# prannaykaul/lvc

Measured on AMD Instinct MI355X. Metric: img/s COCO 800x1333 R50-FPN inference (GeneralizedRCNN.forward(batched_inputs) -> Instances, 1000 proposals, 100 detections), higher is better.
Workload: dtype f32 (conv/GEMM inner products on the fp16 / bf16 matrix cores through fp32-accurate operand splits: two-way fp16 with main + cross fp32 accumulators for the 3x3 and wide 1x1 / FC layers, three-way bf16 for the rest; final boxes/scores closer to the fp64 evaluation than the reference's fp32 CPU path,; 1 GPU; COCO-detection R50-FPN inference, bs=8 synthetic 3x800x1333 per GPU, 1000 pre/post-NMS proposals per level/image, 80 classes, conditioned random-init weights; batch_per_gpu=8, global_batch=8, parallelism=dp1

## Files before the change

### include/lvc_amd.h

```cpp
#ifndef LVC_AMD_H
#define LVC_AMD_H

#ifdef __cplusplus
extern "C" {
#endif

#define LVC_OK 0
#define LVC_ERR_INVALID 1
#define LVC_ERR_HIP 2

int lvc_abi_version(void);
const char* lvc_last_error(void);
void lvc_set_error(const char* fmt, ...);

long long lvc_conv_workspace_bytes(void);
long long lvc_conv_range_words_offset(void);
void lvc_set_range_slot(int slot);
int lvc_range_slot(void);
int lvc_range_slots(void);
int lvc_conv2d_nhwc_f32(const float* x, const float* w_packed, const float* scale, const float* shift,
                        const float* residual, float* y, int N, int H, int W, int C, int K, int R, int S,
                        int stride, int pad, int Kg, int relu, int res_mode, int ldy, int ldr, int mode,
                        void* workspace, void* stream);

int lvc_conv2d_nhwc_bf16x3(const float* x, const unsigned short* w_split, const float* scale, const float* shift,
                           const float* residual, float* y, int N, int H, int W, int C, int K, int R, int S,
                           int stride, int pad, int Kg, int relu, int res_mode, int ldy, int ldr, void* workspace,
                           void* stream);

int lvc_conv3x3_nhwc_bf16x3(const float* x, const unsigned short* w_split, const float* scale, const float* shift,
                            const float* residual, float* y, int N, int H, int W, int C, int K, int Kg, int relu,
                            int res_mode, int ldy, int ldr, void* workspace, void* stream);

int lvc_conv3x3_nhwc_f16x2(const float* x, const unsigned short* w_split, const float* scale, const float* shift,
                           const float* residual, float* y, int N, int H, int W, int C, int K, int Kg, int relu,
                           int res_mode, int ldy, int ldr, void* workspace, void* stream);
int lvc_conv3x3_nhwc_f16s1(const float* x, const unsigned short* w_split, const float* scale, const float* shift,
                           const float* residual, float* y, int N, int H, int W, int C, int K, int Kg, int relu,
                           int res_mode, int ldy, int ldr, void* workspace, void* stream);
int lvc_conv3x3_nhwc_f16x2_pipe(const float* x, const unsigned short* w_split, const float* scale, const float* shift,
                                const float* residual, float* y, int N, int H, int W, int C, int K, int Kg, int relu,
                                int res_mode, int ldy, int ldr, void* workspace, void* stream);
int lvc_conv3x3_nhwc_f16_levels(int oneacc, const float* const* xs, float* const* ys, const int* Hs, const int* Ws, int L,
                                const unsigned short* w_split, const float* scale, const float* shift, int N, int C, int K, int Kg,
                                int relu, void* workspace, void* stream);
int lvc_conv3x3_nhwc_f16_levels_pred(int oneacc, const float* const* xs, float* const* ys, const int* Hs, const int* Ws, int L,
                                     const unsigned short* w_split, const float* scale, const float* shift, int N, int C, int K, int Kg,
                                     int relu, const unsigned short* pred_w, const float* pred_scale, const float* pred_shift, int pred_K,
                                     int pred_rows, int pred_ld, int pred_slot, void* workspace, void* stream);
int lvc_conv3x3_nhwc_f16_layers(int oneacc, const float* const* xs, float* const* ys, const int* Hs, const int* Ws, int L,
                                const unsigned short* const* ws, const float* const* scales, const float* const* shifts, int N, int C,
                                int K, int Kg, int relu, void* workspace, void* stream);
void lvc_set_wino_streamk(int mode);
void lvc_set_patch_plan(int mode);
int lvc_patch_plan(void);
void lvc_set_nms_reduce_global(int on);
void lvc_set_select_onelaunch(int mode);
int lvc_select_onelaunch(void);
void lvc_set_halo_test_hooks(int ph, int pw, int force);
int lvc_conv3x3_nhwc_wino(const float* x, const unsigned short* u, const float* scale, const float* shift, float* y, int N, int H, int W,
                          int C, int K, int Kpad, int relu, int ldy, void* workspace, void* stream);
int lvc_conv3x3_nhwc_wino_pred(const float* x, const unsigned short* u, const float* scale, const float* shift, float* y, int N, int H,
                               int W, int C, int K, int Kpad, int relu, int ldy, const unsigned short* pred_w, const float* pred_scale,
                               const float* pred_shift, int pred_K, int pred_rows, int pred_slot, void* workspace, void* stream);
int lvc_conv1x1_nhwc_f16x2_pipe(const float* x, const unsigned short* w_split, const float* scale, const float* shift,
                                const float* residual, float* y, int N, int H, int W, int C, int K, int stride, int relu,
                                int res_mode, int ldy, int ldr, void* workspace, void* stream);
int lvc_conv1x1_nhwc_f16s1(const float* x, const unsigned short* w_split, const float* scale, const float* shift,
                           const float* residual, float* y, int N, int H, int W, int C, int K, int stride, int relu,
                           int res_mode, int ldy, int ldr, void* workspace, void* stream);
int lvc_conv3x3_nhwc_f16s1_presplit(const float* x, const unsigned short* w_split, const float* scale, const float* shift, void* y,
                                    int N, int H, int W, int C, int K, int Kg, int next_slot, void* workspace, void* stream);
int lvc_conv1x1_nhwc_f16s1_presplit(const void* x, const unsigned short* w_split, const float* scale, const float* shift,
                                    const float* residual, float* y, int N, int H, int W, int C, int K, int relu,
                                    int res_mode, int ldy, int ldr, void* workspace, void* stream);
int lvc_conv1x1_nhwc_f16s1_w2(const float* x, const unsigned short* w_split, const float* scale, const float* shift,
                              const float* residual, float* y, int N, int H, int W, int C, int K, int Kpad, int stride, int relu,
                              int res_mode, int ldy, int ldr, void* workspace, void* stream);
int lvc_conv1x1_chain_nhwc_f16s1(const float* x, int ldx, const unsigned short* wa, int wa_rows, const float* sa, const float* ta,
                                 const float* residual, int ldr, float* y1, int ldy1, int relu1, const unsigned short* wb,
                                 int wb_rows, const float* sb, const float* tb, float* y2, int ldy2, int relu2, int M, int K1,
                                 int N1, int N2, void* workspace, void* stream);
int lvc_bottleneck_nhwc_f16s1(const float* x, int ldx, float* y, int ldy, int N, int H, int W, int cin, int proj,
                              const unsigned short* w, const float* s1, const float* t1, const float* s2, const float* t2,
                              const float* s3, const float* t3, void* workspace, void* stream);
int lvc_split_weights_rowscaled(const float* wp, int rows, int Kg, void* planes_out, float* row_factor, void* stream);

int lvc_conv2d_nhwc_f16x2(const float* x, const unsigned short* w_split, const float* scale, const float* shift,
                          const float* residual, float* y, int N, int H, int W, int C, int K, int R, int S,
                          int stride, int pad, int Kg, int relu, int res_mode, int ldy, int ldr, void* workspace,
                          void* stream);
int lvc_conv2d_nhwc_f16x2_dma(const float* x, const unsigned short* w_split, const float* scale, const float* shift,
                          const float* residual, float* y, int N, int H, int W, int C, int K, int R, int S,
                          int stride, int pad, int Kg, int relu, int res_mode, int ldy, int ldr, void* workspace,
                          void* stream);

int lvc_stem_conv_pool_nhwc4_f16x2(const float* x, const unsigned short* w_split, const float* scale, const float* shift,
                                   float* y, int N, int H, int W, int Kpad, int relu, int* d_error_word,
                                   float* y2 , int ldy2, void* stream);

int lvc_preprocess_nhwc4(const void* image, int dtype, int h, int w, const float* mean3, const float* std3,
                         float* out, int Hp, int Wp, void* stream);
int lvc_preprocess_batch_nhwc4(const void* const* images, int dtype, const int* hs, const int* ws, int B, const float* mean3,
                               const float* std3, float* out, int Hp, int Wp, void* stream);

int lvc_resize_bilinear_u8(const unsigned char* image, int H, int W, int new_h, int new_w, const int* xb, const int* xk,
                           int kxs, const int* yb, const int* yk, int kys, unsigned char* tmp, unsigned char* out_u8,
                           float* out_nhwc4, int Hp, int Wp, const float* mean3, const float* std3, void* stream);
int lvc_tta_resize_u8(const unsigned char* image, int H, int W, long long sy, long long sx, long long sc, const long long* hjobs,
                      int n_h, const long long* vjobs, int n_v, const float* mean3, const float* std3, void* stream);
long long lvc_tta_merge_workspace_bytes(int B, int Nmax);
int lvc_tta_merge(const float* boxes, const float* scores, const int* classes, const int* counts, int topk_in, const float* params,
                  const int* tab, int B, int Nmax, float score_thresh, double nms_thresh, int topk_out, float* ob, float* osc, int* ocl,
                  int* ocount, void* workspace, long long workspace_bytes, void* stream);
int lvc_train_input_u8(const void* h_blob, const void* d_blob, long long blob_bytes, int B, unsigned char* tmp, long long tmp_bytes,
                       float* out, int n_slots, int Hp, int Wp, const float* mean3, const float* std3, int* launches, void* stream);
int lvc_train_input_tiles_u8(const void* h_blob, const void* d_blob, long long blob_bytes, int B, unsigned char* tmp,
                             long long tmp_bytes, float* out, int n_slots, int Hp, int Wp, const float* mean3, const float* std3,
                             int* launches, void* stream);
int lvc_train_input_lsj_u8(const void* h_blob, const void* d_blob, long long blob_bytes, int B, unsigned char* tmp,
                           long long tmp_bytes, float* out, int n_slots, int Hp, int Wp, const float* mean3, const float* std3,
                           int* launches, void* stream);
int lvc_color_jitter_tiles_u8(const void* h_blob, void* d_blob, long long blob_bytes, int B, unsigned char* out, long long out_bytes,
                              int* launches, void* stream);
int lvc_maxpool2d_nhwc(const float* x, float* y, int N, int H, int W, int C, int k, int stride, int pad,
                       void* stream);

int lvc_crop_resize_nearest(const float* image_chw, int C, int H, int W, const int* d_windows, int K, int out_size,
                            float* out, void* stream);

int lvc_rownorm(const float* x, const float* mu, float* y, int M, int D, int ldx, int ldy, float eps, int mode,
                void* stream);
int lvc_rownorm_backward(const float* x, const float* dy, float* dx, int M, int D, float eps, int accumulate, void* stream);

int lvc_roi_align_forward_nchw(const float* input, const float* rois, float* output, int B, int C, int H, int W,
                               int K, int pooled_h, int pooled_w, float spatial_scale, int sampling_ratio,
                               int aligned, int* d_status, void* stream);
int lvc_roi_align_fpn_nhwc(const float* const* feats, const int* Hs, const int* Ws, const float* scales, int L,
                           int B, int C, const float* rois, const int* levels, const int* d_num_valid, int K,
                           int pooled_h, int pooled_w, int sampling_ratio, int aligned, float* output,
                           int* d_status, void* stream);
int lvc_roi_work_order(const float* rois, const int* levels, const float* scales, int L, int K, int pooled_h, int* d_order,
                       void* stream);
int lvc_roi_work_order_xcd(const float* rois, const int* levels, int K, int B, int* d_order, void* stream);
int lvc_roi_align_fpn_nhwc_ordered(const float* const* feats, const int* Hs, const int* Ws, const float* scales, int L,
                                   int B, int C, const float* rois, const int* levels, const int* d_num_valid, int K,
                                   int pooled_h, int pooled_w, int sampling_ratio, int aligned, float* output,
                                   int* d_status, const int* d_order, void* stream);

int lvc_roi_align_backward_nchw(const float* grad, const float* rois, float* grad_input, int B, int C, int H, int W,
                                int K, int pooled_h, int pooled_w, float spatial_scale, int sampling_ratio,
                                int aligned, int* d_status, void* stream);
int lvc_roi_align_fpn_backward_nhwc(const float* grad, float* const* grad_feats, const int* Hs, const int* Ws,
                                    const float* scales, int L, int B, int C, const float* rois, const int* levels,
                                    const int* d_num_valid, int K, int pooled_h, int pooled_w, int sampling_ratio,
                                    int aligned, int* d_status, void* stream);

long long lvc_batched_nms_workspace_bytes(int B, int Nmax);
int lvc_batched_nms(const float* boxes, const float* scores, const int* idxs, const int* d_counts, int B,
                    int Nmax, double iou_threshold, int max_keep, int* keep, int* d_num_keep, void* workspace,
                    long long workspace_bytes, void* stream);

long long lvc_rpn_proposals_workspace_bytes(int B, int L, int A, const int* Hs, const int* Ws, int pre_nms_topk);
int lvc_rpn_proposals(const float* const* logits, const int* ld_logit, const float* const* deltas,
                      const int* ld_delta, const float* const* cell_anchors, const int* Hs, const int* Ws,
                      const int* strides, int L, int A, int B, const int* d_image_sizes, int pre_nms_topk,
                      int post_nms_topk, double nms_thresh, float min_box_size, float scale_clamp,
                      float* out_boxes, float* out_logits, int* d_out_count, void* workspace,
                      long long workspace_bytes, void* stream);

long long lvc_retinanet_select_workspace_bytes(int B, int L, int A, int K, const int* Hs, const int* Ws, int topk,
                                               int max_survivors);
int lvc_retinanet_select(const float* const* logits, const int* ld_logit, const float* const* deltas, const int* ld_delta,
                         const float* const* cell_anchors, const int* Hs, const int* Ws, const int* strides,
                         float anchor_offset, int L, int A, int K, int B, int topk, float score_thresh, float wx, float wy,
                         float ww, float wh, float scale_clamp, int max_survivors, float* out_boxes, float* out_scores,
                         int* out_classes, int* out_index, int* d_count, int* d_status, void* workspace,
                         long long workspace_bytes, void* stream);

int lvc_gather_detections(const float* boxes, const float* scores, const int* classes, const int* rows, const int* keep,
                          const int* d_num_keep, int B, int Nmax, int topk, const float* d_post, float* out_boxes,
                          float* out_scores, int* out_classes, int* out_rows, int* d_out_count, void* stream);

long long lvc_retinanet_loss_workspace_bytes(int B, int L, int A, int K, const int* Hs, const int* Ws);
int lvc_retinanet_loss(const float* const* logits, const int* ld_logit, const float* const* deltas, const int* ld_delta,
                       const int* Hs, const int* Ws, int L, int A, int K, int B, const float* anchors, const int* matches,
                       const signed char* labels, const float* gt, const long long* gt_classes, const int* gt_off, double alpha,
                       double gamma, double beta, double wx, double wy, double ww, double wh, double momentum,
                       double one_minus_momentum, const double* normalizer_in, double* normalizer_out, float* out_losses,
                       double* out_sums , int* num_pos, void* workspace, long long workspace_bytes, void* stream);
int lvc_retinanet_loss_grad(const float* const* logits, const int* ld_logit, const float* const* deltas, const int* ld_delta,
                            const int* Hs, const int* Ws, int L, int A, int K, int B, const float* anchors, const int* matches,
                            const signed char* labels, const float* gt, const long long* gt_classes, const int* gt_off, double alpha,
                            double gamma, double beta, double wx, double wy, double ww, double wh, const double* normalizer,
                            const float* g_cls, const float* g_box, float* const* dlogits, const int* ld_dlogit,
                            float* const* ddeltas, const int* ld_ddelta, void* stream);

int lvc_assign_levels_rois(const float* boxes, int B, int R, int min_level, int max_level, int canonical_box_size,
                           int canonical_level, int* levels, float* rois, void* stream);

long long lvc_fast_rcnn_inference_workspace_bytes(int B, int max_candidates);
int lvc_fast_rcnn_inference(const float* cls_logits, int ld_cls, const float* deltas, int ld_delta, int K,
                            int cls_agnostic, const float* proposals, const int* d_prop_count, int B, int R,
                            const int* d_image_sizes, float wx, float wy, float ww, float wh, float scale_clamp,
                            float score_thresh, double nms_thresh, int topk, int max_candidates,
                            const float* d_post, float* out_boxes, float* out_scores, int* out_classes,
                            int* out_rows, int* d_out_count, int* d_status, void* workspace,
                            long long workspace_bytes, void* stream);

int lvc_decode_boxes(const float* deltas, int ld, const float* boxes, int M, int R, const int* d_image_sizes,
                     float wx, float wy, float ww, float wh, float scale_clamp, float* out, void* stream);

int lvc_match_boxes(const float* gt, int G, const float* boxes, int N, float t0, float t1, int nthr, int l0, int l1,
                    int l2, int allow_low_quality, long long* matches, signed char* labels, float* matched_vals,
                    unsigned int* d_gt_best, void* stream);
int lvc_match_boxes_batched(const float* gt, const int* gt_off, int Gtot, int B, const float* boxes, long long box_img_stride,
                            const int* nbox, int N, float t0, float t1, int nthr, int l0, int l1, int l2, int allow_low_quality,
                            int* matches, signed char* labels, float* vals, unsigned int* gt_best, void* stream);
long long lvc_subsample_workspace_bytes(int B);
int lvc_subsample_batched(const signed char* labels, const long long* keys , unsigned long long seed,
                          int B, int N, int nbits, int cap_pos, int bs, int* sel, int* counts, void* workspace, void* stream);
int lvc_rpn_gather_sampled(const void* const* fused, const int* ld, const void* const* cell_anchors, const int* H, const int* W,
                           const int* strides, int L, int A, int B, int bs, const int* sel, const int* counts, const int* matches,
                           const float* gt, const int* gt_off, float* logits, float* deltas, float* anchors, float* gt_boxes,
                           signed char* labels, void* stream);
int lvc_roi_build_table(const float* pboxes, const float* plogits, const int* pcount, int B, int P, const float* gt, const int* gt_off,
                        float gt_logit, int Wt, float* boxes, float* logits, int* nrow, void* stream);
int lvc_roi_gather_sampled(const float* boxes, const float* logits, const int* matches, const int* sel, const int* counts,
                           const long long* gt_classes, const int* gt_off, int B, int Wt, int bs, int K, float* s_boxes, float* s_logits,
                           long long* s_cls, long long* s_match, void* stream);
int lvc_fast_rcnn_losses(const float* logits, int ld_cls, const float* deltas, int ld_delta, int K, int cls_agnostic,
                         const float* proposals, const float* gt_boxes, const long long* gt_classes, int R, float wx,
                         float wy, float ww, float wh, float smooth_l1_beta, float* out_losses, float* dlogits,
                         float* ddeltas, double* row_terms , void* stream);
int lvc_rpn_losses(const float* logits, const float* deltas, const float* anchors, const float* gt_boxes,
                   const signed char* labels, int S, float smooth_l1_beta, float normalizer, float* out_losses,
                   void* stream);
int lvc_rpn_losses_grad(const float* logits, const float* deltas, const float* anchors, const float* gt_boxes,
                        const signed char* labels, int S, float smooth_l1_beta, float normalizer, float* out_losses,
                        float* dlogits, float* ddeltas, void* stream);

int lvc_giou_box_loss(const float* deltas, int ld_delta, const float* proposals, const float* gt_boxes,
                      const long long* gt_classes, int R, int K, float wx, float wy, float ww, float wh,
                      float scale_clamp, int iterate, float lambda, float* out_loss, float* ddeltas, void* stream);
int lvc_relu_backward(const float* dy, const float* y, long long n, float* out, void* stream);
int lvc_colsum(const float* x, int M, int N, int ldx, float* out, void* stream);

int lvc_pack_conv_weights(const float* w, const float* scale, float* wp, int K, int C, int R, int S, int rows_pad,
                          int cin_pad, int mode, void* stream);
int lvc_split_weights(const float* wp, long long n, int planes, void* out, int* err_word, void* stream);
int lvc_pack_split_conv_weights(const float* w, const float* scale, float* wp, void* planes_out, int planes, int* err_word,
                                int K, int C, int R, int S, int rows_pad, int cin_pad, int mode, void* stream);
int lvc_pack_group(int njobs, const void* const* ptrs, const int* shapes, int* err_word, void* stream);
int lvc_conv_wgrad_nhwc(const float* x, const float* dy, const float* scale, float* dw, int N, int H, int W, int C,
                        int K, int R, int S, int stride, int pad, int lddy, void* stream);
int lvc_conv_wgrad_nhwc_bf16x3(const float* x, const float* dy, const float* scale, float* dw, int N, int H, int W, int C,
                               int K, int R, int S, int stride, int pad, int lddy, void* stream);
int lvc_conv_wgrad_nhwc_f16x2(const float* x, const float* dy, const float* scale, float* dw, int N, int H, int W, int C,
                              int K, int R, int S, int stride, int pad, int lddy, int* err_word, void* stream);
int lvc_conv_wgrad_group_bf16x3(int njobs, const float* const* x, const float* const* dy, const float* const* scale,
                                float* const* dw, const int* shapes, void* stream);
int lvc_wgrad_finalize_group(int njobs, const float* const* src, float* const* dst, const int* shapes, void* stream);
int lvc_scatter_stride2_nhwc(const float* x, float* y, int N, int H, int W, int C, void* stream);
int lvc_conv3x3_grouped_nhwc(const float* x, const float* wp, const float* scale, const float* shift, const float* residual,
                             float* y, int N, int H, int W, int C, int K, int groups, int stride, int relu, int res_mode, int ldy,
                             int ldr, void* workspace, void* stream);
long long lvc_conv3x3_grouped_packed_floats(int K, int groups);
int lvc_pack_conv3x3_grouped(const float* w, const float* scale, float* wp, int K, int groups, int mode, void* stream);
long long lvc_conv3x3_grouped_wgrad_workspace_bytes(int N, int H, int W, int K, int groups, int stride);
int lvc_conv3x3_grouped_wgrad_nhwc(const float* x, const float* dy, const float* scale, float* dw, int N, int H, int W, int C,
                                   int groups, int stride, int lddy, void* scratch, void* stream);
int lvc_subsample2_nhwc(const float* x, float* y, int N, int H, int W, int C, int ldy, void* stream);
int lvc_downsum2x2_nhwc(const float* x, float* y, int N, int Hs, int Ws, int C, void* stream);
int lvc_avgpool2_nhwc(const float* x, float* y, int N, int H, int W, int C, int ldo, void* stream);
int lvc_avgpool2_bwd_nhwc(const float* dy, float* dx, int N, int H, int W, int C, int ldi, void* stream);
int lvc_colsum_atomic(const float* x, int M, int N, int ldx, float* out, void* stream);

int lvc_colmean(const float* x, float* mu, int M, int D, int ld, void* stream);
int lvc_knn_topk_candidates(const float* sims, int ld, int Q, int S, int idx_base, float* cand_val, int* cand_idx, void* stream);
int lvc_knn_merge_vote(const float* cand_val, const int* cand_idx, int nlists, int Q, const long long* shot_classes,
                       const long long* det_classes, int kvote, long long* top_classes, long long* keep, void* stream);
int lvc_max_f32(const float* x, long long n, float* out, void* stream);
int lvc_knn_topk_vote(const float* sims, int ld, int Q, int S, const long long* shot_classes,
                      const long long* det_classes, int kvote, long long* top_classes, long long* keep,
                      void* stream);
int lvc_rownorm_h(const float* x, const float* mu, float* y, unsigned short* yh, float* den, float* resid, int M, int D, int ldx,
                  float eps, int mode, void* stream);
int lvc_gemm_f16(const unsigned short* a, const unsigned short* b, int ldb, float* y, int M, int N, int C, int ldy,
                 void* stream);
int lvc_knn_verify_topk_vote(const float* approx, int ld, int Q, int S, const float* q, int ldq, const float* mu,
                             const float* den, const float* sn, int D, float margin, const float* margins,
                             const long long* shot_classes, const long long* det_classes, int kvote, long long* top_classes,
                             long long* keep, void* stream);
int lvc_knn_margins(const float* qres, const float* d_sres_max, float acc, float extra, int Q, float* margins, void* stream);
int lvc_gemm_f16_q15(const unsigned short* a, const unsigned short* b, int ldb, short* y, int M, int N, int C, int ldy, void* stream);
int lvc_knn_verify_topk_vote_q15(const short* approx, int ld, int Q, int S, const float* q, int ldq, const float* mu,
                             const float* den, const float* sn, int D, float margin, const float* margins,
// ... 81 lines not shown
```

### lvc_amd/csrc/conv_pw_s1.hip

```cpp
#include "conv_common.h"
#include <type_traits>
#include <stdlib.h>

#define PM 256
#define AROW 64
#define NJ 4
#define NT 512

struct PwArgsS {
  const float* x;
  const unsigned short* w;
  const float* scale;
  const float* shift;
  const float* res;
  float* y;
  float* partials;
  int* flags;
  int H, W, C, K, stride, Ho, Wo, M, relu, res_mode, ldy, ldr;
  int tiles_n, nk, total_units, units_per_worker, nworkers, err_index, ngroup;
  int x_bytes;
  long long w_plane_elems;
  unsigned short* planes;
  int* pl_err;
  long long pl_PS;
  int pl_N, pl_Npad, pl_H;
  float pl_qscale;
};

template <int NI, bool ONEACC, bool PLANES = false, bool PRE = false>
__global__ __launch_bounds__(NT, 2) void conv_pw_s1_kernel(PwArgsS p) {
  constexpr int HN = 64 * NI;
  constexpr int PLANE_A = PM * AROW;
  constexpr int A_BUF = 2 * PLANE_A;
  constexpr int A_BYTES = 3 * A_BUF;
  constexpr int PLANE_B = HN * 64;
  constexpr int B_BUF = 2 * PLANE_B;
  constexpr int RING_BYTES = A_BYTES + 3 * B_BUF;
  constexpr int CS_STRIDE = HN + 4;
  constexpr int CS_BYTES = PM * CS_STRIDE * 4;
  constexpr int SMEM_BYTES = RING_BYTES > CS_BYTES ? RING_BYTES : CS_BYTES;
  constexpr int RBLK = HN / 16;
  __shared__ __attribute__((aligned(1024))) unsigned char smem_raw[SMEM_BYTES];
  unsigned char* sA = smem_raw;
  unsigned char* sB = smem_raw + A_BYTES;

  const int tid = threadIdx.x;
  const int lane = tid & 63;
  const int wave = __builtin_amdgcn_readfirstlane(tid >> 6);
  const int wm = wave >> 1, wn = wave & 1;
  const int fi = lane & 31, fh = lane >> 5;
  const int q = PRE ? ((tid >> 4) & 1) * 4 + (tid & 3) : tid & 7;
  const int arid = PRE ? (tid >> 5) * 4 + ((tid >> 2) & 3) : tid >> 3;
  const int hrow = arid;

  const int lw = lvc_xcd_remap(blockIdx.x, p.nworkers);
  const int wq = p.ngroup > 1 ? lw / p.ngroup : lw;
  const int wsel = p.ngroup > 1 ? lw - wq * p.ngroup : 0;
  int u = wq * p.units_per_worker;
  const int u_end = min(u + p.units_per_worker, p.total_units);

  const unsigned long long xbase = (unsigned long long)p.x;
  const u32x4 xres = {(unsigned)__builtin_amdgcn_readfirstlane((unsigned)xbase), (unsigned)__builtin_amdgcn_readfirstlane((unsigned)(xbase >> 32) & 0xffffu),
                      (unsigned)p.x_bytes, 0x00020000u};
  const int fx3 = (fi >> 2) & 3;
  const int a_row[2] = {(wm * 64 + fi) * AROW, (wm * 64 + 32 + fi) * AROW};
  const int b_row = (wn * 32 * NI + fi) * 64;
  const int b_g[2] = {((0 + fh) ^ fx3) * 16, ((2 + fh) ^ fx3) * 16};
  int a_lds[NJ];
#pragma unroll
  for (int j = 0; j < NJ; ++j) {
    const int row = hrow + 64 * j;
    a_lds[j] = row * AROW + (((q >> 1) ^ ((row >> 2) & 3)) << 4) + (q & 1) * 8;
  }
  float big = 0.f;
  int a_pre[NJ];
#pragma unroll
  for (int j = 0; j < NJ; ++j) {
    const int row = hrow + 64 * j;
    a_pre[j] = (q >> 2) * (PM * AROW) + row * AROW + (((q & 3) ^ ((row >> 2) & 3)) << 4);
  }
#ifdef PW_TIMELINE
  unsigned long long tl_pro = 0, tl_loop = 0, tl_hand = 0, tl_cs = 0, tl_rows = 0, tl_t0 = __builtin_readcyclecounter();
  unsigned long long tl_wa = 0, tl_wv = 0, tl_wb = 0;
  unsigned tl_tiles = 0, tl_chunks = 0;
#endif

  while (u < u_end) {
#ifdef PW_TIMELINE
    const unsigned long long tl_a = __builtin_readcyclecounter();
#endif
    const int tile = u / p.nk;
    const int cc0 = u - tile * p.nk;
    const int cc1 = min(p.nk, cc0 + (u_end - u));
    const int tile_n = p.ngroup > 1 ? wsel : tile % p.tiles_n;
    const int tile_m = p.ngroup > 1 ? tile : tile / p.tiles_n;
    const int m0 = tile_m * PM;
    const int n0 = tile_n * HN;

    unsigned a_off[NJ];
#pragma unroll
    for (int j = 0; j < NJ; ++j) {
      const int m = m0 + hrow + 64 * j;
      const int n = m / (p.Ho * p.Wo);
      const int rem = m - n * (p.Ho * p.Wo);
      const int ho = rem / p.Wo, wo = rem - ho * p.Wo;
      a_off[j] = m < p.M ? (unsigned)(((n * p.H + ho * p.stride) * p.W + wo * p.stride) * p.C + q * 4) * 4u : 0x80000000u;
    }
    const unsigned short* bsrc[NI];
    int bdst[NI];
#pragma unroll
    for (int j = 0; j < NI; ++j) {
      const int idx = wave * NI + j;
      const int pl = idx / RBLK, rb = idx - pl * RBLK;
      const int row = rb * 16 + (lane >> 2);
      const int G = (lane & 3) ^ ((row >> 2) & 3);
      bsrc[j] = p.w + (size_t)pl * p.w_plane_elems + (size_t)(n0 + row) * p.C + G * 8;
      bdst[j] = pl * PLANE_B + rb * 16 * 64;
    }
    auto dma_B = [&](int cc, int buf) {
#pragma unroll
      for (int j = 0; j < NI; ++j) glds16(bsrc[j] + cc * 32, sB + buf * B_BUF + bdst[j]);
    };
    f32x4 ar[3][NJ];
    auto load_A = [&](int set, int cc) {
#pragma unroll
      for (int j = 0; j < NJ; ++j) ar[set][j] = load_untracked(xres, a_off[j], (unsigned)cc * 128u);
    };
    auto store_A = [&](int set, unsigned char* dstA) {
      if (PRE) {
#pragma unroll
        for (int j = 0; j < NJ; ++j) {
          *reinterpret_cast<f32x4*>(dstA + a_pre[j]) = ar[set][j];
        }
        return;
      }
#pragma unroll
      for (int j = 0; j < NJ; ++j) {
        f16x4 h, m;
#pragma unroll
        for (int e = 0; e < 4; ++e) {
          const float a = ONEACC ? ar[set][j][e] * LVC_ACT_SCALE : ar[set][j][e];
          const f16 hh = (f16)a;
          h[e] = hh;
          m[e] = ONEACC ? (f16)(a - (float)hh) : (f16)((a - (float)hh) * 2048.f);
          big = fmaxf(big, fabsf(ar[set][j][e]));
        }
        *reinterpret_cast<f16x4*>(dstA + a_lds[j]) = h;
        *reinterpret_cast<f16x4*>(dstA + PLANE_A + a_lds[j]) = m;
      }
    };

    f32x16 acc[2][NI], accx[ONEACC ? 1 : 2][ONEACC ? 1 : NI];
#pragma unroll
    for (int a = 0; a < 2; ++a)
#pragma unroll
      for (int b = 0; b < NI; ++b)
#pragma unroll
        for (int e = 0; e < 16; ++e) {
          acc[a][b][e] = 0.f;
          if (!ONEACC) accx[ONEACC ? 0 : a][ONEACC ? 0 : b][e] = 0.f;
        }

    f16x8 ahi[2], alo[2], bhi[NI], blo[NI];
    auto rdA = [&](const unsigned char* A, int pl, int mi, int s2) {
      return *reinterpret_cast<const f16x8*>(A + pl * PLANE_A + a_row[mi] + b_g[s2]);
    };
    auto rdB = [&](const unsigned char* B, int pl, int ni, int s2) {
      return *reinterpret_cast<const f16x8*>(B + pl * PLANE_B + b_row + ni * 32 * 64 + b_g[s2]);
    };
    auto step_body = [&](const unsigned char* A, int s2, const unsigned char* B, const unsigned char* An, int s2n, const unsigned char* Bn) {
#ifndef PW_DIAG_SKIP_LATE_READS
      alo[0] = rdA(A, 1, 0, s2);
      bhi[0] = rdB(B, 0, 0, s2);
      alo[1] = rdA(A, 1, 1, s2);
      if (NI == 2) bhi[NI - 1] = rdB(B, 0, NI - 1, s2);
#endif
#pragma unroll
      for (int mi = 0; mi < 2; ++mi)
#pragma unroll
        for (int ni = 0; ni < NI; ++ni) {
          f32x16& c = ONEACC ? acc[mi][ni] : accx[ONEACC ? 0 : mi][ONEACC ? 0 : ni];
          c = __builtin_amdgcn_mfma_f32_32x32x16_f16(ahi[mi], blo[ni], c, 0, 0, 0);
        }
      f16x8 blo_n[NI], ahi_n[2];
#pragma unroll
      for (int ni = 0; ni < NI; ++ni) blo_n[ni] = rdB(Bn, 1, ni, s2n);
#pragma unroll
      for (int ni = 0; ni < NI; ++ni)
#pragma unroll
        for (int mi = 0; mi < 2; ++mi) {
          f32x16& c = ONEACC ? acc[mi][ni] : accx[ONEACC ? 0 : mi][ONEACC ? 0 : ni];
#ifndef PW_DIAG_DROP_CROSS
          c = __builtin_amdgcn_mfma_f32_32x32x16_f16(alo[mi], bhi[ni], c, 0, 0, 0);
#endif
        }
#pragma unroll
      for (int mi = 0; mi < 2; ++mi) ahi_n[mi] = rdA(An, 0, mi, s2n);
#pragma unroll
      for (int mi = 0; mi < 2; ++mi)
#pragma unroll
        for (int ni = 0; ni < NI; ++ni)
          acc[mi][ni] = __builtin_amdgcn_mfma_f32_32x32x16_f16(ahi[mi], bhi[ni], acc[mi][ni], 0, 0, 0);
#pragma unroll
      for (int mi = 0; mi < 2; ++mi) ahi[mi] = ahi_n[mi];
#pragma unroll
      for (int ni = 0; ni < NI; ++ni) blo[ni] = blo_n[ni];
    };

    const int last = cc1 - 1;
    load_A(0, cc0);
    load_A(1, min(cc0 + 1, last));
    load_A(2, min(cc0 + 2, last));
    dma_B(cc0, 0);
    dma_B(min(cc0 + 1, last), 1);
    wait_tied<2 * NJ + 2 * NI>(ar[0][0], ar[0][1], ar[0][2], ar[0][3]);
    store_A(0, sA);
    wait_vm<0>();
    __syncthreads();
#pragma unroll
    for (int mi = 0; mi < 2; ++mi) ahi[mi] = rdA(sA, 0, mi, 0);
#pragma unroll
    for (int ni = 0; ni < NI; ++ni) blo[ni] = rdB(sB, 1, ni, 0);
#ifdef PW_DIAG_SKIP_LATE_READS
#pragma unroll
    for (int mi = 0; mi < 2; ++mi) alo[mi] = rdA(sA, 1, mi, 0);
#pragma unroll
    for (int ni = 0; ni < NI; ++ni) bhi[ni] = rdB(sB, 0, ni, 0);
#endif
#ifdef PW_TIMELINE
    const unsigned long long tl_b = __builtin_readcyclecounter();
    tl_pro += tl_b - tl_a;
#endif
    auto chunk = [&](int i, int k) {
      const int cc = cc0 + i;
      const int kn = (k + 1) % 3;
      const unsigned char* Acur = sA + k * A_BUF;
      unsigned char* Anext = sA + kn * A_BUF;
      const unsigned char* Bcur = sB + k * B_BUF;
      const unsigned char* Bnext = sB + kn * B_BUF;
#ifdef PW_TIMELINE
      const unsigned long long tl_1 = __builtin_readcyclecounter();
#endif
      wait_tied<NJ + NI>(ar[kn][0], ar[kn][1], ar[kn][2], ar[kn][3]);
#ifdef PW_TIMELINE
      tl_wa += __builtin_readcyclecounter() - tl_1;
#endif
      step_body(Acur, 0, Bcur, Acur, 1, Bcur);
      store_A(kn, Anext);
      __builtin_amdgcn_sched_barrier(0);
#ifdef PW_TIMELINE
      const unsigned long long tl_2 = __builtin_readcyclecounter();
      wait_vm<NJ>();
      const unsigned long long tl_3 = __builtin_readcyclecounter();
      __builtin_amdgcn_s_barrier();
      tl_wv += tl_3 - tl_2; tl_wb += __builtin_readcyclecounter() - tl_3;
#else
      wait_vm<NJ>();
      __builtin_amdgcn_s_barrier();
#endif
      __builtin_amdgcn_sched_barrier(0);
      dma_B(min(cc + 2, last), (k + 2) % 3);
      load_A(k, min(cc + 3, last));
      step_body(Acur, 1, Bcur, Anext, 0, Bnext);
      __builtin_amdgcn_sched_barrier(0);
    };
    const int nchunks = cc1 - cc0;
#pragma unroll 1
    for (int i = 0; i < nchunks; i += 3) {
      chunk(i, 0);
      if (i + 1 < nchunks) chunk(i + 1, 1);
      if (i + 2 < nchunks) chunk(i + 2, 2);
    }
    wait_vm<0>();
    __syncthreads();
#ifdef PW_TIMELINE
    const unsigned long long tl_c = __builtin_readcyclecounter();
    tl_loop += tl_c - tl_b; tl_chunks += nchunks; ++tl_tiles;
#endif
    u += nchunks;
// ... 152 lines not shown
        using A0 = std::integral_constant<int, 0>; using A1 = std::integral_constant<int, 1>; using A2 = std::integral_constant<int, 2>;
        if constexpr (PLANES) {
          const int hd = p.pl_H * 64;
          const int which = col / hd, hh = (col - which * hd) >> 6, d = col & 63;
          const float f = which == 0 ? p.pl_qscale : 1.f;
          unsigned short* const ph = p.planes + (size_t)(2 * which) * p.pl_PS + d;
          float bigp = 0.f;
#pragma unroll 1
          for (int g = 0; g < NIT; ++g) {
            const int m = m0 + g * RPI + rsub;
            if (m < p.M) {
              const f32x4 v = *reinterpret_cast<const f32x4*>(cs + g * RPI * CS_STRIDE);
              f32x4 o = v * sc + sh;
              o *= f;
              const int b = m / p.pl_N, n = m - b * p.pl_N;
              f16x4 hi, lo;
#pragma unroll
              for (int e = 0; e < 4; ++e) {
                float a = o[e];
                asm volatile("" : "+v"(a));
                bigp = fmaxf(bigp, fabsf(a));
                if (a != a) bigp = INFINITY;
                hi[e] = (f16)a;
                lo[e] = (f16)(a - (float)hi[e]);
              }
              unsigned short* dst = ph + ((size_t)(b * p.pl_H + hh) * p.pl_Npad + n) * 64;
              *reinterpret_cast<f16x4*>(dst) = hi;
              *reinterpret_cast<f16x4*>(dst + p.pl_PS) = lo;
            }
          }
          if (p.pl_err && !(bigp <= LVC_F16_MAX)) atomicOr(p.pl_err, 2);
        } else if (has_res) {
          if (p.relu == 1) rows(std::true_type{}, A1{}); else if (p.relu == 2) rows(std::true_type{}, A2{}); else rows(std::true_type{}, A0{});
        } else {
          if (p.relu == 1) rows(std::false_type{}, A1{}); else if (p.relu == 2) rows(std::false_type{}, A2{}); else rows(std::false_type{}, A0{});
        }
      }
    } else {
      constexpr int C4 = HN / 4;
      constexpr int RPI = NT / C4;
      constexpr int NIT = PM / RPI;
      constexpr int NG = 4;
      const int c4 = tid % C4, rsub = tid / C4;
      const int col = n0 + c4 * 4;
      const bool col_ok = col < p.K;
      const bool has_res = p.res_mode != 0 && col_ok;
      auto res_load = [&](int it) {
        const int m = m0 + it * RPI + rsub;
        f32x4 v = {0.f, 0.f, 0.f, 0.f};
        if (m < p.M) {
          size_t ro = (size_t)m;
          if (p.res_mode == 2) {
            const int n = m / (p.Ho * p.Wo);
            const int rem = m - n * (p.Ho * p.Wo);
            const int ho = rem / p.Wo, wo = rem - ho * p.Wo;
            ro = ((size_t)(n * (p.Ho >> 1) + (ho >> 1)) * (p.Wo >> 1) + (wo >> 1));
          }
          v = *reinterpret_cast<const f32x4*>(p.res + ro * p.ldr + col);
        }
        return v;
      };
      f32x4 rv[NG];
#pragma unroll
      for (int i = 0; i < NG; ++i) rv[i] = f32x4{0.f, 0.f, 0.f, 0.f};
      if (has_res) {
#pragma unroll
        for (int i = 0; i < NG; ++i) rv[i] = res_load(i);
      }
      float* Cs = reinterpret_cast<float*>(smem_raw);
#pragma unroll
      for (int mi = 0; mi < 2; ++mi)
#pragma unroll
        for (int ni = 0; ni < NI; ++ni)
#pragma unroll
          for (int e = 0; e < 16; ++e) {
            const int row = wm * 64 + mi * 32 + (e & 3) + 8 * (e >> 2) + 4 * fh;
            const int colc = wn * 32 * NI + ni * 32 + fi;
            Cs[row * CS_STRIDE + colc] = acc[mi][ni][e];
          }
      __syncthreads();
#ifdef PW_TIMELINE
      tl_e = __builtin_readcyclecounter();
      tl_cs += tl_e - tl_d;
#endif
      if (col_ok) {
        f32x4 sc = {1.f, 1.f, 1.f, 1.f}, sh = {0.f, 0.f, 0.f, 0.f};
        if (p.scale) sc = *reinterpret_cast<const f32x4*>(p.scale + col);
        if (p.shift) sh = *reinterpret_cast<const f32x4*>(p.shift + col);
        const float* cs = Cs + rsub * CS_STRIDE + c4 * 4;
        float* const yb = p.y + (size_t)(m0 + rsub) * p.ldy + col;
        auto rows = [&](auto res_tag, auto act_tag) {
          constexpr bool RES = decltype(res_tag)::value;
          constexpr int ACT = decltype(act_tag)::value;
#pragma unroll 1
          for (int g = 0; g < NIT; g += NG) {
            f32x4 rn[NG];
            if (RES) {
#pragma unroll
              for (int i = 0; i < NG; ++i) rn[i] = f32x4{0.f, 0.f, 0.f, 0.f};
              if (g + NG < NIT) {
#pragma unroll
                for (int i = 0; i < NG; ++i) rn[i] = res_load(g + NG + i);
              }
            }
            f32x4 v[NG];
#pragma unroll
            for (int i = 0; i < NG; ++i) v[i] = *reinterpret_cast<const f32x4*>(cs + (g + i) * RPI * CS_STRIDE);
#pragma unroll
            for (int i = 0; i < NG; ++i) {
              const int m = m0 + (g + i) * RPI + rsub;
              if (m < p.M) {
                f32x4 o = v[i] * sc + sh;
                if (RES) o += rv[i];
                if (ACT == 1) {
                  o[0] = o[0] > 0.f ? o[0] : 0.f; o[1] = o[1] > 0.f ? o[1] : 0.f;
                  o[2] = o[2] > 0.f ? o[2] : 0.f; o[3] = o[3] > 0.f ? o[3] : 0.f;
                } else if (ACT == 2) {
#pragma unroll
                  for (int e = 0; e < 4; ++e) o[e] = o[e] * 0.5f * (1.f + erff(o[e] * 0.70710678118654752440f));
                }
                *reinterpret_cast<f32x4*>(yb + (size_t)((g + i) * RPI) * p.ldy) = o;
              }
            }
            if (RES) {
#pragma unroll
              for (int i = 0; i < NG; ++i) rv[i] = rn[i];
            }
          }
        };
        using A0 = std::integral_constant<int, 0>; using A1 = std::integral_constant<int, 1>; using A2 = std::integral_constant<int, 2>;
        if (has_res) {
          if (p.relu == 1) rows(std::true_type{}, A1{}); else if (p.relu == 2) rows(std::true_type{}, A2{}); else rows(std::true_type{}, A0{});
        } else {
          if (p.relu == 1) rows(std::false_type{}, A1{}); else if (p.relu == 2) rows(std::false_type{}, A2{}); else rows(std::false_type{}, A0{});
        }
      }
    }
    __syncthreads();
#ifdef PW_TIMELINE
    tl_rows += __builtin_readcyclecounter() - tl_e;
#endif
  }
#ifdef PW_TIMELINE
  if (lane == 0 && (blockIdx.x & 15) == 0) {
    unsigned long long* d = reinterpret_cast<unsigned long long*>(reinterpret_cast<char*>(p.partials) + LVC_WS_DIAG_OFFSET) + ((blockIdx.x >> 4) * 8 + wave) * 16;
    d[0] = tl_pro; d[1] = tl_loop; d[2] = tl_hand; d[3] = tl_cs; d[4] = tl_rows; d[5] = tl_tiles; d[6] = tl_chunks; d[7] = __builtin_readcyclecounter() - tl_t0; d[8] = 1; d[9] = tl_wa; d[10] = tl_wv; d[11] = tl_wb;
  }
#endif
  if (PRE) return;
  lvc_report_range(p.flags, p.err_index, big, ONEACC ? LVC_ACT_MAX : LVC_F16_MAX);
}

struct PwPlanes { unsigned short* planes; int* err; long long PS; int N, Npad, H; float qscale; };

static int pw_s1_launch(bool oneacc, const float* x, const unsigned short* w_split, const float* scale, const float* shift,
                        const float* residual, float* y, int N, int H, int W, int C, int K, int stride, int relu, int res_mode,
                        int ldy, int ldr, void* workspace, void* stream, const PwPlanes* pl = nullptr, bool pre = false) {
  LVC_CHECK_ARG(x && w_split && y && workspace, "null pointer");
  LVC_CHECK_ARG(!oneacc || scale, "the single-accumulator form needs the row factors in `scale`");
  LVC_CHECK_ARG(N > 0 && H > 0 && W > 0 && C > 0 && K > 0 && stride >= 1, "non-positive dimension");
  LVC_CHECK_ARG(C % 32 == 0, "needs C % 32 == 0");
  LVC_CHECK_ARG(relu >= 0 && relu <= 2, "relu: 0 none, 1 ReLU, 2 GELU");
  LVC_CHECK_ARG(res_mode >= 0 && res_mode <= 2 && (res_mode == 0 || residual), "bad residual");
  const int Ho = (H - 1) / stride + 1, Wo = (W - 1) / stride + 1;
  if (res_mode == 2) LVC_CHECK_ARG(Ho % 2 == 0 && Wo % 2 == 0, "upsample-add needs even output size");
  PwArgsS a;
  a.x = x; a.w = w_split; a.scale = scale; a.shift = shift; a.res = residual; a.y = y;
  a.H = H; a.W = W; a.C = C; a.K = K; a.stride = stride; a.Ho = Ho; a.Wo = Wo;
  const long long Mll = (long long)N * Ho * Wo;
  LVC_CHECK_ARG(Mll < (1ll << 31), "too many output pixels");
  a.M = (int)Mll; a.relu = relu; a.res_mode = res_mode;
  a.ldy = ldy > 0 ? ldy : K; a.ldr = ldr > 0 ? ldr : K;
  LVC_CHECK_ARG((K & 3) == 0 && (a.ldy & 3) == 0 && (res_mode == 0 || (a.ldr & 3) == 0), "K, ldy, ldr must be multiples of 4");
  LVC_CHECK_ARG(((uintptr_t)x & 15) == 0 && ((uintptr_t)w_split & 15) == 0 && ((uintptr_t)y & 15) == 0 && ((uintptr_t)workspace & 15) == 0 &&
                    ((uintptr_t)scale & 15) == 0 && ((uintptr_t)shift & 15) == 0 && ((uintptr_t)residual & 15) == 0,
                "pointers must be 16-byte aligned");
  const long long xb = (long long)N * H * W * C * 4;
  LVC_CHECK_ARG(xb < (1ll << 31), "input tensor must be smaller than 2 GiB");
  a.x_bytes = (int)xb;
  const int ni = K <= 64 ? 1 : 2;
  const int HN = 64 * ni;
  a.tiles_n = lvc_cdiv(K, HN);
  a.nk = C / 32;
  const int tiles_m = lvc_cdiv(a.M, PM);
  long long units = (long long)tiles_m * a.tiles_n * a.nk;
  LVC_CHECK_ARG(units < (1ll << 31), "iteration space too large");
  a.total_units = (int)units;
  a.w_plane_elems = (long long)(lvc_cdiv(K, 128) * 128) * C;
  int cap = lvc_cu_count();
  if (cap > LVC_MAX_WORKERS) cap = LVC_MAX_WORKERS;
  a.ngroup = 1;
  if ((a.tiles_n == 2 || a.tiles_n == 4 || a.tiles_n == 8 || a.tiles_n == 16) && cap % a.tiles_n == 0 && units / a.tiles_n >= (long long)(cap / a.tiles_n) * 4) {
    a.ngroup = a.tiles_n;
    units /= a.tiles_n;
    cap /= a.tiles_n;
    a.total_units = (int)units;
  }
  const int min_units = 4;
  lvc_plan_workers(units, cap, min_units, &a.units_per_worker, &a.nworkers);
  a.nworkers *= a.ngroup;
  a.partials = (float*)workspace;
  a.flags = lvc_ws_flags(workspace);
  a.err_index = lvc_ws_range_index(lvc_range_slot());
  hipStream_t st = (hipStream_t)stream;
  a.planes = nullptr; a.pl_err = nullptr; a.pl_PS = 0; a.pl_N = a.pl_Npad = a.pl_H = 0; a.pl_qscale = 1.f;
  if (pl) {
    LVC_CHECK_ARG(oneacc && ni == 2 && res_mode == 0 && relu == 0, "the planes epilogue exists for the single-accumulator 128-column tile");
    a.planes = pl->planes; a.pl_err = pl->err; a.pl_PS = pl->PS; a.pl_N = pl->N; a.pl_Npad = pl->Npad; a.pl_H = pl->H; a.pl_qscale = pl->qscale;
    hipLaunchKernelGGL((conv_pw_s1_kernel<2, true, true>), dim3(a.nworkers), dim3(NT), 0, st, a);
    LVC_CHECK_LAUNCH();
    return LVC_OK;
  }
  if (pre) {
    LVC_CHECK_ARG(oneacc && ni == 2 && stride == 1, "pre-split input: the single-accumulator 128-column tile, stride 1");
    hipLaunchKernelGGL((conv_pw_s1_kernel<2, true, false, true>), dim3(a.nworkers), dim3(NT), 0, st, a);
    LVC_CHECK_LAUNCH();
    return LVC_OK;
  }
  if (oneacc) {
    if (ni == 1) hipLaunchKernelGGL((conv_pw_s1_kernel<1, true>), dim3(a.nworkers), dim3(NT), 0, st, a);
    else hipLaunchKernelGGL((conv_pw_s1_kernel<2, true>), dim3(a.nworkers), dim3(NT), 0, st, a);
  } else {
    if (ni == 1) hipLaunchKernelGGL((conv_pw_s1_kernel<1, false>), dim3(a.nworkers), dim3(NT), 0, st, a);
    else hipLaunchKernelGGL((conv_pw_s1_kernel<2, false>), dim3(a.nworkers), dim3(NT), 0, st, a);
  }
  LVC_CHECK_LAUNCH();
  return LVC_OK;
}

extern "C" int lvc_conv1x1_nhwc_f16x2_pipe(const float* x, const unsigned short* w_split, const float* scale, const float* shift,
                                            const float* residual, float* y, int N, int H, int W, int C, int K, int stride, int relu,
                                            int res_mode, int ldy, int ldr, void* workspace, void* stream) {
  return pw_s1_launch(false, x, w_split, scale, shift, residual, y, N, H, W, C, K, stride, relu, res_mode, ldy, ldr, workspace, stream);
}

extern "C" int lvc_conv1x1_nhwc_f16s1(const float* x, const unsigned short* w_split, const float* scale, const float* shift,
                                       const float* residual, float* y, int N, int H, int W, int C, int K, int stride, int relu,
                                       int res_mode, int ldy, int ldr, void* workspace, void* stream) {
  return pw_s1_launch(true, x, w_split, scale, shift, residual, y, N, H, W, C, K, stride, relu, res_mode, ldy, ldr, workspace, stream);
}

extern "C" int lvc_conv1x1_nhwc_f16s1_presplit(const void* x, const unsigned short* w_split, const float* scale, const float* shift,
                                                const float* residual, float* y, int N, int H, int W, int C, int K, int relu,
                                                int res_mode, int ldy, int ldr, void* workspace, void* stream) {
  return pw_s1_launch(true, (const float*)x, w_split, scale, shift, residual, y, N, H, W, C, K, 1, relu, res_mode, ldy, ldr, workspace, stream, nullptr, true);
}

extern "C" int lvc_conv1x1_qkv_planes_f16s1(const float* x, const unsigned short* w_split, const float* scale, const float* shift, void* planes,
                                            int B, int N, int C, int H, float softmax_scale, int* err_word, void* workspace, void* stream) {
  LVC_CHECK_ARG(planes && B > 0 && N > 0 && H > 0, "bad arguments");
  const int Npad = (N + 127) / 128 * 128;
  PwPlanes pl;
  pl.planes = (unsigned short*)planes; pl.err = err_word; pl.N = N; pl.Npad = Npad; pl.H = H; pl.qscale = softmax_scale * 1.44269504088896340736f;
  pl.PS = (long long)B * H * Npad * 64;
  return pw_s1_launch(true, x, w_split, scale, shift, nullptr, (float*)planes, B * N, 1, 1, C, 3 * H * 64, 1, 0, 0, 0, 0, workspace, stream, &pl);
}
```

### lvc_amd/csrc/roi_align.hip

```cpp
#include "common.h"
#include <stdlib.h>
#include <type_traits>

#define LVC_MAX_LEVELS 8

struct RoiAlignArgs {
  const float* feat[LVC_MAX_LEVELS];
  int H[LVC_MAX_LEVELS], W[LVC_MAX_LEVELS];
  float scale[LVC_MAX_LEVELS];
  long long sb[LVC_MAX_LEVELS];
  long long sc, sh_mul_w;
  int nhwc;
  int C;
  const float* rois;
  const int* levels;
  const int* num_valid;
  int K, ph, pw, sampling_ratio, aligned;
  float* out;
  long long so_k, so_c, so_h, so_w;
  int* status;
  const int* order;
};

__global__ __launch_bounds__(256) void roi_align_fwd_kernel(RoiAlignArgs p) {
// ... 532 lines not shown
        for (int ix = 0; ix < gw; ++ix) {
          const float xx = roi_start_w + pw * bin_w + (float)(ix + .5f) * bin_w / (float)gw;
          float x = xx, y = yy;
          if (y < -1.0f || y > (float)H || x < -1.0f || x > (float)W) continue;
          if (y <= 0) y = 0;
          if (x <= 0) x = 0;
          int y_low = (int)y, x_low = (int)x, y_high, x_high;
          if (y_low >= H - 1) { y_high = y_low = H - 1; y = (float)y_low; } else y_high = y_low + 1;
          if (x_low >= W - 1) { x_high = x_low = W - 1; x = (float)x_low; } else x_high = x_low + 1;
          const float ly = y - y_low, lx = x - x_low;
          const float hy = 1.f - ly, hx = 1.f - lx;
          if (c_ok) {
            unsafeAtomicAdd(gin + (long long)(y_low * W + x_low) * p.C, g * (hy * hx) / count);
            unsafeAtomicAdd(gin + (long long)(y_low * W + x_high) * p.C, g * (hy * lx) / count);
            unsafeAtomicAdd(gin + (long long)(y_high * W + x_low) * p.C, g * (ly * hx) / count);
            unsafeAtomicAdd(gin + (long long)(y_high * W + x_high) * p.C, g * (ly * lx) / count);
          }
        }
      }
    }
  }
}

extern "C" int lvc_roi_align_backward_nchw(const float* grad, const float* rois, float* grad_input, int B, int C,
                                           int H, int W, int K, int pooled_h, int pooled_w, float spatial_scale,
                                           int sampling_ratio, int aligned, int* d_status, void* stream) {
  LVC_CHECK_ARG(grad_input && (K == 0 || (grad && rois)), "null pointer");
  LVC_CHECK_ARG(B > 0 && C > 0 && H > 0 && W > 0 && pooled_h > 0 && pooled_w > 0 && K >= 0, "bad shape");
  if (hipMemsetAsync(grad_input, 0, (size_t)B * C * H * W * sizeof(float), (hipStream_t)stream) != hipSuccess) {
    lvc_set_error("%s: hipMemsetAsync failed", __func__);
    return LVC_ERR_HIP;
  }
  if (K == 0) return LVC_OK;
  RoiAlignArgs a;
  memset(&a, 0, sizeof a);
  a.feat[0] = grad_input; a.H[0] = H; a.W[0] = W; a.scale[0] = spatial_scale;
  a.sb[0] = (long long)C * H * W;
  a.nhwc = 0; a.C = C; a.rois = rois; a.levels = nullptr; a.num_valid = nullptr;
  a.K = K; a.ph = pooled_h; a.pw = pooled_w; a.sampling_ratio = sampling_ratio; a.aligned = aligned;
  a.out = const_cast<float*>(grad);
  a.so_k = (long long)C * pooled_h * pooled_w; a.so_c = (long long)pooled_h * pooled_w;
  a.so_h = pooled_w; a.so_w = 1;
  a.status = d_status;
  hipLaunchKernelGGL(roi_align_bwd_kernel, dim3(K, lvc_cdiv(C, 256)), dim3(256), 0, (hipStream_t)stream, a);
  LVC_CHECK_LAUNCH();
  return LVC_OK;
}

extern "C" int lvc_roi_align_fpn_backward_nhwc(const float* grad, float* const* grad_feats, const int* Hs,
                                               const int* Ws, const float* scales, int L, int B, int C,
                                               const float* rois, const int* levels, const int* d_num_valid, int K,
                                               int pooled_h, int pooled_w, int sampling_ratio, int aligned,
                                               int* d_status, void* stream) {
  LVC_CHECK_ARG(L >= 1 && L <= LVC_MAX_LEVELS, "1..8 levels");
  LVC_CHECK_ARG(grad_feats && Hs && Ws && scales && (K == 0 || (grad && rois)), "null pointer");
  LVC_CHECK_ARG(B > 0 && C > 0 && pooled_h > 0 && pooled_w > 0 && K >= 0, "bad shape");
  LVC_CHECK_ARG(L == 1 || levels, "levels required when L > 1");
  RoiAlignArgs a;
  memset(&a, 0, sizeof a);
  for (int l = 0; l < L; ++l) {
    LVC_CHECK_ARG(grad_feats[l] && Hs[l] > 0 && Ws[l] > 0, "bad level");
    if (hipMemsetAsync(grad_feats[l], 0, (size_t)B * Hs[l] * Ws[l] * C * sizeof(float), (hipStream_t)stream) != hipSuccess) {
      lvc_set_error("%s: hipMemsetAsync failed", __func__);
      return LVC_ERR_HIP;
    }
    a.feat[l] = grad_feats[l]; a.H[l] = Hs[l]; a.W[l] = Ws[l]; a.scale[l] = scales[l];
    a.sb[l] = (long long)C * Hs[l] * Ws[l];
  }
  if (K == 0) return LVC_OK;
  a.nhwc = 1; a.C = C; a.rois = rois; a.levels = levels; a.num_valid = d_num_valid;
  a.K = K; a.ph = pooled_h; a.pw = pooled_w; a.sampling_ratio = sampling_ratio; a.aligned = aligned;
  a.out = const_cast<float*>(grad);
  a.so_k = (long long)C * pooled_h * pooled_w; a.so_c = 1;
  a.so_h = (long long)pooled_w * C; a.so_w = C;
  a.status = d_status;
  if (pooled_h == 7 && pooled_w == 7)
    hipLaunchKernelGGL((roi_align_bwd_rows_kernel<7, 7>), dim3(K, lvc_cdiv(C, 256)), dim3(256), 0, (hipStream_t)stream, a);
  else
    hipLaunchKernelGGL(roi_align_bwd_kernel, dim3(K, lvc_cdiv(C, 256)), dim3(256), 0, (hipStream_t)stream, a);
  LVC_CHECK_LAUNCH();
  return LVC_OK;
}

extern "C" int lvc_roi_align_forward_nchw(const float* input, const float* rois, float* output, int B,
                                          int C, int H, int W, int K, int pooled_h, int pooled_w,
                                          float spatial_scale, int sampling_ratio, int aligned,
                                          int* d_status, void* stream) {
  LVC_CHECK_ARG(K == 0 || (input && rois && output), "null pointer");
  LVC_CHECK_ARG(B > 0 && C > 0 && H > 0 && W > 0 && pooled_h > 0 && pooled_w > 0 && K >= 0, "bad shape");
  RoiAlignArgs a;
  memset(&a, 0, sizeof a);
  a.feat[0] = input; a.H[0] = H; a.W[0] = W; a.scale[0] = spatial_scale;
  a.sb[0] = (long long)C * H * W;
  a.nhwc = 0; a.C = C; a.rois = rois; a.levels = nullptr; a.num_valid = nullptr;
  a.K = K; a.ph = pooled_h; a.pw = pooled_w; a.sampling_ratio = sampling_ratio; a.aligned = aligned;
  a.out = output;
  a.so_k = (long long)C * pooled_h * pooled_w; a.so_c = (long long)pooled_h * pooled_w;
  a.so_h = pooled_w; a.so_w = 1;
  a.status = d_status;
  return launch(a, stream);
}

struct RoiOrderArgs {
  const float* rois;
  const int* levels;
  float scale[LVC_MAX_LEVELS];
  int K, ph;
  int* order;
};
__global__ __launch_bounds__(1024) void roi_work_order_kernel(RoiOrderArgs p) {
  __shared__ int hist[64];
  const int tid = threadIdx.x;
  if (tid < 64) hist[tid] = 0;
  __syncthreads();
  auto bucket = [&](int k) {
    const float* r = p.rois + (long long)k * 5;
    const float sc = p.scale[p.levels ? p.levels[k] : 0];
    const float w = fmaxf((r[3] - r[1]) * sc, 0.f) + 2.f, h = fmaxf((r[4] - r[2]) * sc, 0.f) + 2.f * (float)p.ph;
    const float a = w * h;
    int b = a == a ? (int)(2.f * log2f(fminf(fmaxf(a, 1.f), 1e9f))) : 0;
    b = b < 0 ? 0 : b > 63 ? 63 : b;
    return 63 - b;
  };
  for (int k = tid; k < p.K; k += 1024) atomicAdd(&hist[bucket(k)], 1);
  __syncthreads();
  if (tid == 0) {
    int run = 0;
    for (int i = 0; i < 64; ++i) { const int n = hist[i]; hist[i] = run; run += n; }
  }
  __syncthreads();
  for (int k = tid; k < p.K; k += 1024) p.order[atomicAdd(&hist[bucket(k)], 1)] = k;
}

extern "C" int lvc_roi_work_order(const float* rois, const int* levels, const float* scales, int L, int K, int pooled_h,
                                  int* d_order, void* stream) {
  LVC_CHECK_ARG(L >= 1 && L <= LVC_MAX_LEVELS && K >= 0 && pooled_h > 0, "bad shape");
  if (K == 0) return LVC_OK;
  LVC_CHECK_ARG(rois && scales && d_order && (L == 1 || levels), "null pointer");
  RoiOrderArgs a;
  memset(&a, 0, sizeof a);
  a.rois = rois; a.levels = levels; a.K = K; a.ph = pooled_h; a.order = d_order;
  for (int l = 0; l < L; ++l) a.scale[l] = scales[l];
  hipLaunchKernelGGL(roi_work_order_kernel, dim3(1), dim3(1024), 0, (hipStream_t)stream, a);
  LVC_CHECK_LAUNCH();
  return LVC_OK;
}

#define ROI_XCD_MAX_B 16
struct RoiOrderXcdArgs {
  const float* rois;
  const int* levels;
  int K, B;
  int* order;
};
__global__ __launch_bounds__(1024) void roi_work_order_xcd_kernel(RoiOrderXcdArgs p) {
  __shared__ int hist[ROI_XCD_MAX_B][256];
  __shared__ int cnt[ROI_XCD_MAX_B], tail0[ROI_XCD_MAX_B], s_min;
  const int tid = threadIdx.x;
  for (int i = tid; i < ROI_XCD_MAX_B * 256; i += 1024) (&hist[0][0])[i] = 0;
  __syncthreads();
  auto key = [&](int k, int& b) {
    const float* r = p.rois + (long long)k * 5;
    const float bf = r[0];
    b = bf >= 0.f && bf < (float)p.B ? (int)bf : 0;
    const int lv = p.levels ? (p.levels[k] & 3) : 0;
    const float yc = (r[2] + r[4]) * 0.5f;
    int band = yc == yc ? (int)(fminf(fmaxf(yc, 0.f), 1e6f) * (1.f / 16.f)) : 0;
    band = band > 63 ? 63 : band;
    return lv * 64 + band;
  };
  for (int k = tid; k < p.K; k += 1024) { int b; const int ky = key(k, b); atomicAdd(&hist[b][ky], 1); }
  __syncthreads();
  if (tid < p.B) {
    int run = 0;
    for (int i = 0; i < 256; ++i) { const int n = hist[tid][i]; hist[tid][i] = run; run += n; }
    cnt[tid] = run;
  }
  __syncthreads();
  if (tid == 0) {
    int m = cnt[0];
    for (int b = 1; b < p.B; ++b) m = cnt[b] < m ? cnt[b] : m;
    s_min = m;
    int run = 0;
    for (int b = 0; b < p.B; ++b) { tail0[b] = run; run += cnt[b] - m; }
  }
  __syncthreads();
  const int m = s_min;
  for (int k = tid; k < p.K; k += 1024) {
    int b;
    const int ky = key(k, b);
    const int r = atomicAdd(&hist[b][ky], 1);
    p.order[r < m ? r * p.B + b : m * p.B + tail0[b] + (r - m)] = k;
  }
}

extern "C" int lvc_roi_work_order_xcd(const float* rois, const int* levels, int K, int B, int* d_order, void* stream) {
  LVC_CHECK_ARG(K >= 0 && B >= 1 && B <= ROI_XCD_MAX_B, "1..16 images");
  if (K == 0) return LVC_OK;
  LVC_CHECK_ARG(rois && d_order, "null pointer");
  RoiOrderXcdArgs a;
  a.rois = rois; a.levels = levels; a.K = K; a.B = B; a.order = d_order;
  hipLaunchKernelGGL(roi_work_order_xcd_kernel, dim3(1), dim3(1024), 0, (hipStream_t)stream, a);
  LVC_CHECK_LAUNCH();
  return LVC_OK;
}

static int roi_align_fpn_nhwc_impl(const float* const* feats, const int* Hs, const int* Ws,
                                      const float* scales, int L, int B, int C, const float* rois,
                                      const int* levels, const int* d_num_valid, int K, int pooled_h,
                                      int pooled_w, int sampling_ratio, int aligned, float* output,
                                      int* d_status, const int* d_order, void* stream) {
  LVC_CHECK_ARG(L >= 1 && L <= LVC_MAX_LEVELS, "1..8 levels");
  LVC_CHECK_ARG(K == 0 || (feats && Hs && Ws && scales && rois && output), "null pointer");
  LVC_CHECK_ARG(B > 0 && C > 0 && pooled_h > 0 && pooled_w > 0 && K >= 0, "bad shape");
  LVC_CHECK_ARG(L == 1 || levels, "levels required when L > 1");
  RoiAlignArgs a;
  memset(&a, 0, sizeof a);
  for (int l = 0; l < L; ++l) {
    a.feat[l] = feats[l]; a.H[l] = Hs[l]; a.W[l] = Ws[l]; a.scale[l] = scales[l];
    a.sb[l] = (long long)C * Hs[l] * Ws[l];
  }
  a.nhwc = 1; a.C = C; a.rois = rois; a.levels = levels; a.num_valid = d_num_valid;
  a.K = K; a.ph = pooled_h; a.pw = pooled_w; a.sampling_ratio = sampling_ratio; a.aligned = aligned;
  a.out = output;
  a.so_k = (long long)C * pooled_h * pooled_w; a.so_c = 1;
  a.so_h = (long long)pooled_w * C; a.so_w = C;
  a.status = d_status;
  a.order = d_order;
  return launch(a, stream);
}

extern "C" int lvc_roi_align_fpn_nhwc(const float* const* feats, const int* Hs, const int* Ws,
                                      const float* scales, int L, int B, int C, const float* rois,
                                      const int* levels, const int* d_num_valid, int K, int pooled_h,
                                      int pooled_w, int sampling_ratio, int aligned, float* output,
                                      int* d_status, void* stream) {
  return roi_align_fpn_nhwc_impl(feats, Hs, Ws, scales, L, B, C, rois, levels, d_num_valid, K, pooled_h, pooled_w, sampling_ratio, aligned,
                                 output, d_status, nullptr, stream);
}

extern "C" int lvc_roi_align_fpn_nhwc_ordered(const float* const* feats, const int* Hs, const int* Ws,
                                      const float* scales, int L, int B, int C, const float* rois,
                                      const int* levels, const int* d_num_valid, int K, int pooled_h,
                                      int pooled_w, int sampling_ratio, int aligned, float* output,
                                      int* d_status, const int* d_order, void* stream) {
  return roi_align_fpn_nhwc_impl(feats, Hs, Ws, scales, L, B, C, rois, levels, d_num_valid, K, pooled_h, pooled_w, sampling_ratio, aligned,
                                 output, d_status, d_order, stream);
}
```

### lvc_amd/csrc/stem_pool_h2.hip

```cpp
#include "conv_common.h"
#include <stdlib.h>

#define SP_PH 3
#define SP_PW 17
#define SP_CH (2 * SP_PH + 1)
#define SP_CW (2 * SP_PW + 1)
#define SP_M (SP_CH * SP_CW)
#define SP_IH (2 * SP_CH + 5)
#define SP_IW (2 * SP_CW + 6)
#define SP_IROW (SP_IW * 4)
#define SP_PLANE_IN (SP_IH * SP_IROW)
#define SP_LROW 40
#define SP_PLANE_B (64 * SP_LROW)
#define SP_CS 68
#define SP_NT 512
#define SP_NLD 3

struct StemArgsH {
  const float* x;
  const unsigned short* w;
  int* err;
  const float* scale;
  const float* shift;
  float* y;
  float* y2;
  int ldy2;
  int N, H, W, Ho, Wo, Hp, Wp, relu;
  int tiles_x, tiles_y, ntiles, nworkers;
  int x_bytes, w_plane_bytes;
};

__device__ __forceinline__ void split2s(float a, f16& h, f16& m) {
  h = (f16)a;
  m = (f16)((a - (float)h) * 2048.f);
}

__global__ __launch_bounds__(SP_NT, 4) void stem_pool_h2_kernel(StemArgsH p) {
  constexpr int IN_ELEMS = 2 * SP_PLANE_IN;
  constexpr int B_ELEMS = 2 * SP_PLANE_B;
  constexpr int CS_OFF = 0;
  constexpr int RING_BYTES = (IN_ELEMS + 2 * B_ELEMS) * 2;
  constexpr int CS_BYTES = SP_M * SP_CS * 4;
  constexpr int SMEM_BYTES = RING_BYTES > CS_BYTES ? RING_BYTES : CS_BYTES;
  __shared__ __attribute__((aligned(16))) unsigned char smem_raw[SMEM_BYTES];
  f16* sIn = reinterpret_cast<f16*>(smem_raw);
  f16* sB = sIn + IN_ELEMS;
  float* Cs = reinterpret_cast<float*>(smem_raw + CS_OFF);

  const int tid = threadIdx.x;
  const int lane = tid & 63;
  const int wave = tid >> 6;
  const int wm = wave >> 1, wn = wave & 1;
  const int fi = lane & 31, fh = lane >> 5;
  const int brid = (tid & 255) >> 2;
  const int b_row = (brid & 1) * 4 + ((brid >> 1) & 3) + (brid >> 3) * 8;
  const int b_q4 = tid & 3;
  const int b_pl0 = tid >> 8;
  const unsigned b_off = (unsigned)(b_row * 224 + b_q4 * 8) * 2u;

  const __amdgpu_buffer_rsrc_t xres = __builtin_amdgcn_make_buffer_rsrc((void*)p.x, 0, p.x_bytes, 0x00020000);
  const __amdgpu_buffer_rsrc_t wres = __builtin_amdgcn_make_buffer_rsrc((void*)p.w, 0, 2 * p.w_plane_bytes, 0x00020000);

  int a_frag[2];
#pragma unroll
  for (int mi = 0; mi < 2; ++mi) {
    const int m = wm * 64 + mi * 32 + fi;
    const int mm = m < SP_M ? m : 0;
    const int cyl = mm / SP_CW, cxl = mm - cyl * SP_CW;
    a_frag[mi] = 2 * cyl * SP_IROW + 8 * cxl + fh * 8;
  }
  const int b_frag = (wn * 32 + fi) * SP_LROW + fh * 8;

  const int ocol = wn * 32 + fi;
  const float sc = p.scale ? p.scale[ocol] : 1.f;
  const float sh = p.shift ? p.shift[ocol] : 0.f;

  int range_err = 0;
  f32x4 wreg[SP_NLD];
  u32x4 breg[1], breg2;
  auto window_offsets = [&](int tile, unsigned* off) {
    const int tx = tile % p.tiles_x;
    const int t2 = tile / p.tiles_x;
    const int ty = t2 % p.tiles_y;
    const int img = t2 / p.tiles_y;
    const int iy0 = 2 * (2 * ty * SP_PH - 1) - 3, ix0 = 2 * (2 * tx * SP_PW - 1) - 3;
#pragma unroll
    for (int j = 0; j < SP_NLD; ++j) {
      const int idx = tid + SP_NT * j;
      const int iy = idx / SP_IW, ix = idx - iy * SP_IW;
      const int yy = iy0 + iy, xx = ix0 + ix;
      const bool ok = idx < SP_IH * SP_IW && yy >= 0 && yy < p.H && xx >= 0 && xx < p.W;
      off[j] = ok ? (unsigned)(((img * p.H + yy) * p.W + xx) * 4) * 4u : 0x80000000u;
    }
  };
  auto load_window = [&](int tile) {
    unsigned off[SP_NLD];
    window_offsets(tile, off);
#pragma unroll
    for (int j = 0; j < SP_NLD; ++j)
      wreg[j] = __builtin_bit_cast(f32x4, __builtin_amdgcn_raw_buffer_load_b128(xres, off[j], 0, 0));
  };
  auto store_window = [&]() {
#pragma unroll
    for (int j = 0; j < SP_NLD; ++j) {
      const int idx = tid + SP_NT * j;
      if (idx < SP_IH * SP_IW) {
        f16x4 h, m;
        float big = 0.f;
#pragma unroll
        for (int e = 0; e < 4; ++e) {
          f16 hh, mm;
          split2s(wreg[j][e], hh, mm);
          h[e] = hh; m[e] = mm;
          big = fmaxf(big, fabsf(wreg[j][e]));
        }
        if (!(big <= LVC_F16_MAX)) range_err = 1;
        const int o = idx * 4;
        *reinterpret_cast<f16x4*>(sIn + o) = h;
        *reinterpret_cast<f16x4*>(sIn + SP_PLANE_IN + o) = m;
      }
    }
  };
  int ld_r = 0;
  auto load_B = [&]() {
    breg[0] = __builtin_bit_cast(u32x4, __builtin_amdgcn_raw_buffer_load_b128(
                                            wres, b_off + (unsigned)(b_pl0 * p.w_plane_bytes), ld_r * 64, 0));
    ld_r = ld_r == 6 ? 0 : ld_r + 1;
  };
  auto load_B2 = [&]() {
    breg2 = __builtin_bit_cast(u32x4, __builtin_amdgcn_raw_buffer_load_b128(
                                          wres, b_off + (unsigned)(b_pl0 * p.w_plane_bytes), ld_r * 64, 0));
    ld_r = ld_r == 6 ? 0 : ld_r + 1;
  };
  auto store_B = [&](int buf) {
    f16* sb = sB + buf * B_ELEMS;
    *reinterpret_cast<u32x4*>(sb + b_pl0 * SP_PLANE_B + b_row * SP_LROW + b_q4 * 8) = breg[0];
  };

  int tile = lvc_xcd_remap(blockIdx.x, p.nworkers);
  if (tile >= p.ntiles) return;
  load_window(tile);
  load_B();
  store_window();
  store_B(0);
  load_B();
  if (tile + p.nworkers < p.ntiles) load_window(tile + p.nworkers);
  __syncthreads();
  int cur = 0;

  for (; tile < p.ntiles; tile += p.nworkers) {
    f32x16 acc[2], accx[2];
#pragma unroll
    for (int a = 0; a < 2; ++a)
#pragma unroll
      for (int e = 0; e < 16; ++e) { acc[a][e] = 0.f; accx[a][e] = 0.f; }

    f16x8 fa[2][2], fb[2];
    auto read_frags = [&](int row_off, const f16* sb, int s2) {
#pragma unroll
      for (int mi = 0; mi < 2; ++mi)
#pragma unroll
        for (int pl = 0; pl < 2; ++pl)
          fa[mi][pl] = *reinterpret_cast<const f16x8*>(sIn + pl * SP_PLANE_IN + a_frag[mi] + row_off + s2 * 16);
#pragma unroll
      for (int pl = 0; pl < 2; ++pl)
        fb[pl] = *reinterpret_cast<const f16x8*>(sb + pl * SP_PLANE_B + b_frag + s2 * 16);
    };
    auto mfma_group = [&]() {
#pragma unroll
      for (int mi = 0; mi < 2; ++mi) accx[mi] = __builtin_amdgcn_mfma_f32_32x32x16_f16(fa[mi][0], fb[1], accx[mi], 0, 0, 0);
#pragma unroll
      for (int mi = 0; mi < 2; ++mi) acc[mi] = __builtin_amdgcn_mfma_f32_32x32x16_f16(fa[mi][0], fb[0], acc[mi], 0, 0, 0);
#pragma unroll
      for (int mi = 0; mi < 2; ++mi) accx[mi] = __builtin_amdgcn_mfma_f32_32x32x16_f16(fa[mi][1], fb[0], accx[mi], 0, 0, 0);
    };
    for (int r = 0; r < 7; ++r) {
      const f16* sb = sB + cur * B_ELEMS;
      read_frags(r * SP_IROW, sb, 0);
      if (r < 6) store_B(cur ^ 1);
      mfma_group();
      __builtin_amdgcn_sched_barrier(0);
      read_frags(r * SP_IROW, sb, 1);
      if (r < 6) load_B(); else load_B2();
      mfma_group();
      __builtin_amdgcn_sched_barrier(0);
      __syncthreads();
      cur ^= 1;
    }

    const int tx = tile % p.tiles_x;
    const int t2 = tile / p.tiles_x;
    const int ty = t2 % p.tiles_y;
    const int img = t2 / p.tiles_y;
#pragma unroll
    for (int mi = 0; mi < 2; ++mi)
#pragma unroll
      for (int e = 0; e < 16; ++e) {
        const int row = wm * 64 + mi * 32 + (e & 3) + 8 * (e >> 2) + 4 * fh;
        if (row < SP_M) {
          float v = (acc[mi][e] + accx[mi][e] * (1.f / 2048.f)) * sc + sh;
          if (p.relu) v = v > 0.f ? v : 0.f;
          Cs[row * SP_CS + ocol] = v;
        }
      }
    const bool more = tile + p.nworkers < p.ntiles;
    __syncthreads();
    const int cy0 = 2 * ty * SP_PH - 1, cx0 = 2 * tx * SP_PW - 1;
    for (int o = tid; o < SP_PH * SP_PW * 16; o += SP_NT) {
      const int c4 = o & 15, pp = o >> 4;
      const int pi = pp / SP_PW, pj = pp - pi * SP_PW;
      const int py = ty * SP_PH + pi, px = tx * SP_PW + pj;
      if (py < p.Hp && px < p.Wp) {
        f32x4 best = {-INFINITY, -INFINITY, -INFINITY, -INFINITY};
#pragma unroll
        for (int dy = 0; dy < 3; ++dy) {
          const int cyl = 2 * pi + dy;
          const int cy = cy0 + cyl;
          if (cy < 0 || cy >= p.Ho) continue;
#pragma unroll
          for (int dx = 0; dx < 3; ++dx) {
            const int cxl = 2 * pj + dx;
            const int cx = cx0 + cxl;
            if (cx < 0 || cx >= p.Wo) continue;
            const f32x4 v = *reinterpret_cast<const f32x4*>(Cs + (cyl * SP_CW + cxl) * SP_CS + c4 * 4);
            best[0] = v[0] > best[0] ? v[0] : best[0];
            best[1] = v[1] > best[1] ? v[1] : best[1];
            best[2] = v[2] > best[2] ? v[2] : best[2];
            best[3] = v[3] > best[3] ? v[3] : best[3];
          }
        }
        *reinterpret_cast<f32x4*>(p.y + ((size_t)(img * p.Hp + py) * p.Wp + px) * 64 + c4 * 4) = best;
        if (p.y2) *reinterpret_cast<f32x4*>(p.y2 + ((size_t)(img * p.Hp + py) * p.Wp + px) * p.ldy2 + c4 * 4) = best;
      }
    }
    __syncthreads();
    if (more) store_window();
    store_B(cur);
    breg[0] = breg2;
    if (tile + 2 * p.nworkers < p.ntiles) load_window(tile + 2 * p.nworkers);
    __syncthreads();
  }
  if (range_err && p.err) atomicOr(p.err, 2);
}

extern "C" int lvc_stem_conv_pool_nhwc4_f16x2(const float* x, const unsigned short* w_split, const float* scale,
                                              const float* shift, float* y, int N, int H, int W, int Kpad, int relu,
                                              int* d_error_word, float* y2, int ldy2, void* stream) {
  LVC_CHECK_ARG(x && w_split && y, "null pointer");
  LVC_CHECK_ARG(!y2 || (ldy2 >= 64 && ldy2 % 4 == 0 && ((uintptr_t)y2 & 15) == 0), "bad second output");
  LVC_CHECK_ARG(N > 0 && H > 0 && W > 0 && Kpad >= 64, "bad shape");
  LVC_CHECK_ARG(((uintptr_t)x & 15) == 0 && ((uintptr_t)w_split & 15) == 0 && ((uintptr_t)y & 15) == 0,
                "pointers must be 16-byte aligned");
  StemArgsH a;
  a.x = x; a.w = w_split; a.scale = scale; a.shift = shift; a.y = y; a.y2 = y2; a.ldy2 = ldy2;
  a.N = N; a.H = H; a.W = W; a.relu = relu; a.err = d_error_word;
  a.Ho = (H + 6 - 7) / 2 + 1; a.Wo = (W + 6 - 7) / 2 + 1;
  a.Hp = (a.Ho + 2 - 3) / 2 + 1; a.Wp = (a.Wo + 2 - 3) / 2 + 1;
  a.tiles_x = lvc_cdiv(a.Wp, SP_PW); a.tiles_y = lvc_cdiv(a.Hp, SP_PH);
  const long long nt = (long long)N * a.tiles_x * a.tiles_y;
  const long long xb = (long long)N * H * W * 16, wb = (long long)Kpad * 224 * 2;
  LVC_CHECK_ARG(nt < (1ll << 31) && xb < (1ll << 31), "input too large");
  a.ntiles = (int)nt; a.x_bytes = (int)xb; a.w_plane_bytes = (int)wb;
  a.nworkers = a.ntiles < 2 * lvc_cu_count() ? a.ntiles : 2 * lvc_cu_count();
  hipLaunchKernelGGL(stem_pool_h2_kernel, dim3(a.nworkers), dim3(SP_NT), 0, (hipStream_t)stream, a);
  LVC_CHECK_LAUNCH();
  return LVC_OK;
}
```

### lvc_amd/kernels.py

```python
import collections
import ctypes

import torch

from . import _lib
from ._lib import LvcNativeError, c_double, c_float, c_int, c_longlong, c_void_p, check, ptr

BK = 32
BN = 128


def _stream(t):
    return c_void_p(torch.cuda.current_stream(t.device).cuda_stream)


def _req_cuda(*ts):
    for t in ts:
        if t is not None and not t.is_cuda:
            raise RuntimeError("lvc_amd kernels need device tensors (got a CPU tensor); there is no CPU path")


def _float3(v):
    return (c_float * 3)(*[float(x) for x in v])

# ... 518 lines not shown
            and pc.K % 4 == 0 and ldo % 4 == 0 and (ldr or 0) % 4 == 0):
        return ConvRoute("f32", "lvc_conv2d_nhwc_f32", False, False)
    if halo:
        if not (f16 and halo_tiles(N, H * W, pc.K) >= _HALO_H2_MIN_TILES):
            return ConvRoute("bf16x3_halo", "lvc_conv3x3_nhwc_bf16x3", False, False)
        if configured and HALO_S1 == 2:
            if (tier == 0 and (not pc.two_acc or WINO_RPN) and not has_res and out_contiguous and ldo == pc.K
                    and wino_sized(N, H, W, pc.K)):
                return ConvRoute("f16x2_wino", "lvc_conv3x3_nhwc_wino", True, True)
            if not two_acc:
                return ConvRoute("f16x2_halo", "lvc_conv3x3_nhwc_f16s1", True, True)
        if configured and HALO_S1 >= 1:
            return ConvRoute("f16x2_halo", "lvc_conv3x3_nhwc_f16x2_pipe", False, True)
        return ConvRoute("f16x2_halo", "lvc_conv3x3_nhwc_f16x2", False, configured)
    if f16 and pw and pc.C >= _H2_PW_MIN_C and rows >= 2048:
        if configured and PW_S1 and pc.C >= _PW_S1_MIN_C and pc.K >= 64 and (not has_res or _PW_S1_RES) and out_numel < (1 << 29):
            one = PW_S1 == 2 and not two_acc and pc.C >= _PW_S1_ONE_MIN_C
            if one and PW_W2 and pc.C >= _PW_W2_MIN_C and pc.K >= 256 and pc.K % 256 == 0 and rows >= _PW_W2_MIN_ROWS:
                return ConvRoute("f16x2_pws1", "lvc_conv1x1_nhwc_f16s1_w2", True, True)
            return ConvRoute("f16x2_pws1", "lvc_conv1x1_nhwc_f16s1" if one else "lvc_conv1x1_nhwc_f16x2_pipe", one, True)
        dma_ok = out_numel < (1 << 29) and (not has_res or (res_numel < (1 << 29) and pc.K % 32 == 0))
        return ConvRoute("f16x2_pw", "lvc_conv2d_nhwc_f16x2_dma" if dma_ok else "lvc_conv2d_nhwc_f16x2", False, configured)
    return ConvRoute("bf16x3", "lvc_conv2d_nhwc_bf16x3", False, False)


_TAIL_GENERIC = lambda pc, wts: (pc.R, pc.S, pc.stride, pc.pad, pc.Kg)
_TAIL_3X3 = lambda pc, wts: (pc.Kg,)
_TAIL_1X1 = lambda pc, wts: (pc.stride,)
_NO_LAST = lambda pc: ()
_CONV_ARGS = {
    "lvc_conv2d_nhwc_f32": ("w", _TAIL_GENERIC, lambda pc: (pc.mode,)),
    "lvc_conv2d_nhwc_bf16x3": ("3", _TAIL_GENERIC, _NO_LAST),
    "lvc_conv2d_nhwc_f16x2": ("h", _TAIL_GENERIC, _NO_LAST),
    "lvc_conv2d_nhwc_f16x2_dma": ("h", _TAIL_GENERIC, _NO_LAST),
    "lvc_conv3x3_nhwc_bf16x3": ("3", _TAIL_3X3, _NO_LAST),
    "lvc_conv3x3_nhwc_f16x2": ("h", _TAIL_3X3, _NO_LAST),
    "lvc_conv3x3_nhwc_f16x2_pipe": ("h", _TAIL_3X3, _NO_LAST),
    "lvc_conv3x3_nhwc_f16s1": ("s", _TAIL_3X3, _NO_LAST),
    "lvc_conv1x1_nhwc_f16x2_pipe": ("h", _TAIL_1X1, _NO_LAST),
    "lvc_conv1x1_nhwc_f16s1": ("s", _TAIL_1X1, _NO_LAST),
    "lvc_conv1x1_nhwc_f16s1_w2": ("s", lambda pc, wts: (wts.shape[1], pc.stride), _NO_LAST),
    "lvc_conv3x3_grouped_nhwc": ("w", lambda pc, wts: (pc.groups, pc.stride), _NO_LAST),
}
_GELU_EPILOGUE = ("lvc_conv1x1_nhwc_f16x2_pipe", "lvc_conv1x1_nhwc_f16s1", "lvc_conv1x1_nhwc_f16s1_w2", "lvc_conv2d_nhwc_f16x2_dma")


def presplit_pair_ok(x, pc2, pc3, residual=None):
    if not (PRESPLIT and pc3.C == pc2.K and pc2.K % 32 == 0):
        return False
    N, H, W, C = x.shape
    rows = N * H * W
    if not (C == pc2.C and 2048 <= rows and max(x.numel(), rows * pc2.K, rows * pc3.K) < (1 << 29) and pc3.K > 64
            and _out_hw(pc3, H, W) == (H, W)):
        return False
    r2 = conv_route(pc2, N, H, W)
    r3 = conv_route(pc3, N, H, W, ldr=None if residual is None else residual.shape[-1],
                    res_numel=0 if residual is None else residual.numel())
    return r2.entry == "lvc_conv3x3_nhwc_f16s1" and r3.entry == "lvc_conv1x1_nhwc_f16s1"


def conv3x3_conv1x1_presplit(x, pc2, pc3, residual=None, relu=True):
    _req_cuda(x, residual)
    assert x.dim() == 4 and x.is_contiguous() and x.dtype == torch.float32
    N, H, W, C = x.shape
    mid = torch.empty(N, H, W, pc2.K, device=x.device, dtype=torch.float32)
    out = torch.empty(N, H, W, pc3.K, device=x.device, dtype=torch.float32)
    if residual is not None:
        assert residual.is_contiguous() and residual.dtype == torch.float32 and residual.shape[:3] == out.shape[:3]
    ldr = residual.shape[-1] if residual is not None else 0
    ws = ptr(conv_workspace(x.device))
    planes2, scale2 = pc2.split2s()
    planes3, scale3 = pc3.split2s()
    rows = N * H * W
    pc2.last_one = True
    pc3.last_one = True
    _launch("f16x2_halo", 2.0 * rows * pc2.K * C * 9, 4.0 * (rows * C + rows * pc2.K + pc2.K * C * 9), pc2.slot,
            "lvc_conv3x3_nhwc_f16s1_presplit", lambda: _lib.lib().lvc_conv3x3_nhwc_f16s1_presplit(
                ptr(x), ptr(planes2), ptr(scale2), ptr(pc2.shift), ptr(mid), c_int(N), c_int(H), c_int(W), c_int(C), c_int(pc2.K),
                c_int(pc2.Kg), c_int(pc3.slot), ws, _stream(x)))
    _launch("f16x2_pws1", 2.0 * rows * pc3.K * pc3.C,
            4.0 * (rows * pc3.C + rows * pc3.K + (residual.numel() if residual is not None else 0) + pc3.K * pc3.C), pc3.slot,
            "lvc_conv1x1_nhwc_f16s1_presplit", lambda: _lib.lib().lvc_conv1x1_nhwc_f16s1_presplit(
                ptr(mid), ptr(planes3), ptr(scale3), ptr(pc3.shift), ptr(residual), ptr(out), c_int(N), c_int(H), c_int(W), c_int(pc3.C),
                c_int(pc3.K), c_int(1 if relu else 0), c_int(1 if residual is not None else 0), c_int(pc3.K), c_int(ldr), ws, _stream(x)))
    return out


def conv2d_nhwc(x, pc, relu=False, residual=None, res_mode=0, out=None, split=None, act=None):
    _req_cuda(x, residual)
    assert x.dim() == 4 and x.is_contiguous() and x.dtype == torch.float32
    N, H, W, C = x.shape
    assert C == pc.C, "channel mismatch: tensor {} vs packed {}".format(C, pc.C)
    Ho, Wo = _out_hw(pc, H, W)
    if out is None:
        out = torch.empty(N, Ho, Wo, pc.K, device=x.device, dtype=torch.float32)
    grouped = getattr(pc, "groups", 1) != 1
    if grouped and out.numel() == 0:
        return out
    if residual is not None:
        assert residual.is_contiguous() and residual.dtype == torch.float32
        if res_mode == 0:
            res_mode = 1
    res_numel = residual.numel() if residual is not None else 0
    big = max(x.numel(), out.numel(), res_numel)
    if big >= (1 << 29) and N > 1 and out.is_contiguous() and out.shape[-1] == pc.K:
        per_image = (big + N - 1) // N
        nb = max(1, ((1 << 29) - 1) // per_image)
        _log_once("conv_batch_split", "conv/GEMM layer with %d elements in one tensor (batch %d): run in groups of %d images to stay "
                  "inside the kernels' 2 GiB buffer descriptors", big, N, nb)
        for n0 in range(0, N, nb):
            n1 = min(N, n0 + nb)
            conv2d_nhwc(x[n0:n1], pc, relu=relu, residual=residual[n0:n1] if residual is not None else None, res_mode=res_mode,
                        out=out[n0:n1], split=split, act=act)
        return out
    ldo = out.shape[-1]
    ldr = residual.shape[-1] if residual is not None else 0
    route = conv_route(pc, N, H, W, ldo, out.is_contiguous(), out.numel(), None if residual is None else ldr, res_numel, split)
    entry = route.entry
    if route.slotted:
        pc.last_one = route.one
    if entry == "lvc_conv3x3_nhwc_wino":
        def call():
            return _wino_launch(x, pc, relu, out)
    else:
        if entry == "lvc_conv2d_nhwc_f16x2" and route.engine == "f16x2_pw":
            _log_once("pw_dma_fallback", "pointwise layer %dx%d->%d (%d output elements, residual %s) is outside the LDS-DMA "
                      "kernel's range; it runs on the register-staged fp16x2 kernel", N * H * W, C, pc.K, out.numel(),
                      "yes" if residual is not None else "no")
        code = 1 if relu else 0
        if act == "gelu" and not relu and entry in _GELU_EPILOGUE:
            code, act = 2, None
        operand, tail, last = _CONV_ARGS[entry]

        def call():
            wts, scale = (pc.split2s() if operand == "s" else
                          ((pc.split2h() if operand == "h" else pc.split3() if operand == "3" else pc.w), pc.scale))
            ints = (N, H, W, C, pc.K) + tail(pc, wts) + (code, res_mode, ldo, ldr) + last(pc)
            return getattr(_lib.lib(), entry)(ptr(x), ptr(wts), ptr(scale), ptr(pc.shift), ptr(residual), ptr(out),
                                              *[c_int(v) for v in ints], ptr(conv_workspace(x.device)), _stream(x))
    c_real = 3 if pc.mode == 1 else C
    nbytes = 4.0 * (N * (Ho * Wo if (pc.R == 1 and pc.S == 1) else H * W) * c_real + N * Ho * Wo * pc.K + res_numel
                    + pc.K * c_real * pc.R * pc.S)
    if grouped:
        c_real = C // pc.groups
        nbytes = 4.0 * (N * H * W * C + N * Ho * Wo * pc.K + res_numel + pc.K * c_real * 9)
    _launch(route.engine, 2.0 * N * Ho * Wo * pc.K * c_real * pc.R * pc.S, nbytes, pc.slot if route.slotted else None, entry, call)
    if act == "gelu":
        check(_lib.lib().lvc_gelu(ptr(out), ptr(out), c_longlong(out.numel()), _stream(out)), "lvc_gelu")
    elif act is not None:
        raise ValueError("unknown activation {!r}".format(act))
    return out


class PackedChain:

    __slots__ = ("wa", "sa", "ta", "wb", "sb", "tb", "K1", "N1", "N2", "slot", "state", "__weakref__")


_PERM16 = (0, 1, 2, 3, 8, 9, 10, 11, 4, 5, 6, 7, 12, 13, 14, 15)
CHAIN_SHAPES = {(64, 256, 64), (128, 256, 64), (128, 512, 128)}


def _chain_planes(pc):
    assert pc.R == 1 and pc.S == 1 and pc.mode == 0 and pc.stride == 1 and pc.pad == 0
    rows, Kg = pc.w.shape
    idx = torch.arange(Kg, device=pc.w.device).view(-1, 16)[:, list(_PERM16)].reshape(-1)
    wperm = pc.w[:, idx].contiguous()
    planes = torch.empty((2, rows, Kg), device=pc.w.device, dtype=torch.float16)
    fac = torch.empty(rows, device=pc.w.device, dtype=torch.float32)
    check(_lib.lib().lvc_split_weights_rowscaled(ptr(wperm), c_int(rows), c_int(Kg), ptr(planes), ptr(fac), _stream(pc.w)),
          "lvc_split_weights_rowscaled")
    fac = fac[: pc.K]
    return planes, (fac * pc.scale if pc.scale is not None else fac).contiguous()


CONV_WINO = _os.environ.get("LVC_CONV_WINO", "1") != "0"
WINO_STREAMK = int(_os.environ.get("LVC_WINO_STREAMK", "0"))


def set_wino_streamk(mode):
    global WINO_STREAMK
    WINO_STREAMK = int(mode)
    _lib.lib().lvc_set_wino_streamk(c_int(int(mode)))
WINO_RPN = False
_WINO_MIN_TILES = 512


def pack_wino(pc):
    cached = pc.state.get("_wino")
    if cached is not None and cached[0] is pc.w:
        return cached[1], cached[2]
    assert pc.R == 3 and pc.S == 3 and pc.mode == 0 and pc.C % 32 == 0
    K, C = pc.K, pc.C
    w = pc.w[:K].view(K, C // 32, 3, 3, 32).permute(0, 1, 4, 2, 3).reshape(K, C, 3, 3).double()
    g0, g1, g2 = w[..., 0], w[..., 1], w[..., 2]
    U = torch.stack([g0, (g0 + g1 + g2) / 2, (g0 - g1 + g2) / 2, g2], dim=-1).float()
    Kpad = (K + 127) // 128 * 128
    flat = torch.zeros(Kpad, C * 12, device=pc.w.device)
    flat[:K] = U.reshape(K, C * 12)
    planes = torch.empty(2, Kpad, C * 12, dtype=torch.int16, device=pc.w.device)
    fac = torch.empty(Kpad, device=pc.w.device)
    check(_lib.lib().lvc_split_weights_rowscaled(ptr(flat), c_int(Kpad), c_int(C * 12), ptr(planes), ptr(fac), _stream(flat)), "lvc_split_weights_rowscaled")
    u = planes.view(2, Kpad, C // 16, 16, 3, 4).permute(4, 2, 5, 0, 1, 3).contiguous()
    scale = (fac[:K] * pc.scale if pc.scale is not None else fac[:K]).contiguous()
    pc.state["_wino"] = (pc.w, u, scale)
    return u, scale


def _wino_launch(x, pc, relu, out):
    _req_cuda(x)
    N, H, W, C = x.shape
    u, scale = pack_wino(pc)
    return _lib.lib().lvc_conv3x3_nhwc_wino(ptr(x), ptr(u), ptr(scale), ptr(pc.shift), ptr(out), c_int(N), c_int(H), c_int(W), c_int(C), c_int(pc.K),
                                            c_int(u.shape[4]), c_int(1 if relu else 0), c_int(out.stride(2)), ptr(conv_workspace(x.device)), _stream(x))


def conv3x3_wino(x, pc, relu=False, out=None):
    if out is None:
        out = torch.empty(x.shape[0], x.shape[1], x.shape[2], pc.K, device=x.device, dtype=torch.float32)
    check(_wino_launch(x, pc, relu, out), "lvc_conv3x3_nhwc_wino")
    return out


def wino_tiles(N, H, W, K):
    return N * ((H + 7) // 8) * ((W + 31) // 32) * ((K + 127) // 128)


def _direct_f16_3x3(pc, C):
    return (CONV_ENGINE == "bf16x3" and CONV_SPLIT == "f16x2" and CONV_HALO and HALO_S1 >= 1 and pc.state["tier"] < 2 and pc.mode == 0
            and pc.R == 3 and pc.S == 3 and pc.stride == 1 and pc.pad == 1 and pc.C == C and C % 32 == 0)


def _level_maps_ok(xs, N, C, K):
    return (all(x.dim() == 4 and x.is_contiguous() and x.dtype == torch.float32 and x.shape[0] == N and x.shape[3] == C
                and x.numel() < (1 << 29) for x in xs)
            and halo_tiles(N, max(x.shape[1] * x.shape[2] for x in xs), K) >= _HALO_H2_MIN_TILES)


def _wino_levels(xs, K):
    big = [i for i, x in enumerate(xs) if wino_sized(x.shape[0], x.shape[1], x.shape[2], K)]
    return big, [i for i in range(len(xs)) if i not in big]


_GROUP_SLOTS = {}


def _group_slot(pcs):
    key = tuple(id(pc.state) for pc in pcs)
    ent = _GROUP_SLOTS.get(key)
    if ent is None or any(r() is None for r in ent[1]):
        import weakref

        slot = _new_range_slot(pcs[0])
        for pc in pcs[1:]:
            _SLOT_OWNERS[slot].append(weakref.ref(pc))
        if len(_GROUP_SLOTS) > 64:
            _GROUP_SLOTS.clear()
        ent = _GROUP_SLOTS[key] = (slot, [weakref.ref(pc) for pc in pcs])
    else:
        import weakref

        live = [r for r in _SLOT_OWNERS.get(ent[0], []) if r() is not None and all(r() is not pc for pc in pcs)]
        _SLOT_OWNERS[ent[0]] = live + [weakref.ref(pc) for pc in pcs]
    return ent[0]


def conv3x3_levels(xs, pc, relu=False, outs=None):
    _req_cuda(*xs)
    pcs = list(pc) if isinstance(pc, (list, tuple)) else [pc] * len(xs)
    shared = not isinstance(pc, (list, tuple))
    p0 = pcs[0]
    N, C = xs[0].shape[0], xs[0].shape[3]
    if outs is None:
        outs = [torch.empty(x.shape[0], x.shape[1], x.shape[2], q.K, device=x.device, dtype=torch.float32) for x, q in zip(xs, pcs)]
    forms = {(q.two_acc or q.state["tier"] >= 1) for q in pcs}
    ok = (len(xs) > 1 and len(xs) <= 6 and len(pcs) == len(xs) and len(forms) == 1
          and all(_direct_f16_3x3(q, C) and q.K == p0.K and q.Kg == p0.Kg for q in pcs) and p0.K >= 64 and p0.K % 4 == 0
          and _level_maps_ok(xs, N, C, p0.K)
          and all(o.is_contiguous() and o.shape == (x.shape[0], x.shape[1], x.shape[2], p0.K) for o, x in zip(outs, xs)))
    if not ok:
        for x, q, o in zip(xs, pcs, outs):
            conv2d_nhwc(x, q, relu=relu, out=o)
        return outs
    one = HALO_S1 == 2 and not (True in forms)
    if CONV_WINO and HALO_S1 == 2 and all(q.state["tier"] == 0 and (not q.two_acc or WINO_RPN) for q in pcs):
        big, rest = _wino_levels(xs, p0.K)
        if big:
            for i in big:
                conv2d_nhwc(xs[i], pcs[i], relu=relu, out=outs[i])
            if rest:
                conv3x3_levels([xs[i] for i in rest], pc if shared else [pcs[i] for i in rest], relu=relu, outs=[outs[i] for i in rest])
            return outs
    L = len(xs)
    XP, IP = c_void_p * L, c_int * L
    xp, yp = XP(*[x.data_ptr() for x in xs]), XP(*[o.data_ptr() for o in outs])
    hs, ws = IP(*[x.shape[1] for x in xs]), IP(*[x.shape[2] for x in xs])
    for q in pcs:
        q.last_one = one
    ops = [q.split2s() if one else (q.split2h(), q.scale) for q in (pcs[:1] if shared else pcs)]
    if shared:
        weights = (ptr(ops[0][0]), ptr(ops[0][1]), ptr(p0.shift))
    else:
        weights = [XP(*[0 if t is None else t.data_ptr() for t in ts]) for ts in ([o[0] for o in ops], [o[1] for o in ops], [q.shift for q in pcs])]
    entry = "lvc_conv3x3_nhwc_f16_levels" if shared else "lvc_conv3x3_nhwc_f16_layers"
    px = sum(x.shape[0] * x.shape[1] * x.shape[2] for x in xs)
    _launch("f16x2_halo", 2.0 * px * p0.K * C * 9, 4.0 * (px * C + px * p0.K + (1 if shared else L) * p0.K * C * 9),
# ... 56 lines not shown
                c_int(0), xp, yp, hs, ws, c_int(L), ptr(planes), ptr(pc.scale), ptr(pc.shift), c_int(N),
                c_int(C), c_int(pc.K), c_int(pc.Kg), c_int(1 if relu else 0), ptr(pplanes),
                ptr(pred.scale), ptr(pred.shift), c_int(pred.K), c_int(pred.w.shape[0]),
                c_int(pred.K), c_int(pred.slot), ptr(conv_workspace(xs[0].device)), _stream(xs[0])))
    return outs


def pack_chain(pc_a, pc_b, state=None):
    assert pc_b.C == pc_a.K
    ch = PackedChain()
    ch.slot = _new_range_slot(ch)
    ch.state = state if state is not None else {"off": False}
    ch.wa, ch.sa = _chain_planes(pc_a)
    ch.wb, ch.sb = _chain_planes(pc_b)
    ch.ta, ch.tb = pc_a.shift, pc_b.shift
    ch.K1, ch.N1, ch.N2 = pc_a.C, pc_a.K, pc_b.K
    return ch


def conv1x1_chain(x, ch, residual=None, relu1=True, relu2=True, out1=None, out2=None):
    _req_cuda(x, residual)
    assert x.dtype == torch.float32 and x.is_contiguous() and x.shape[-1] >= ch.K1
    M = x.numel() // x.shape[-1]
    lead = tuple(x.shape[:-1])
    if out1 is None:
        out1 = torch.empty(lead + (ch.N1,), device=x.device, dtype=torch.float32)
    if out2 is None:
        out2 = torch.empty(lead + (ch.N2,), device=x.device, dtype=torch.float32)
    if residual is not None:
        assert residual.is_contiguous() and residual.dtype == torch.float32 and residual.numel() // residual.shape[-1] == M
    nbytes = 4.0 * (M * (ch.K1 + ch.N1 + ch.N2 + (ch.N1 if residual is not None else 0)) + ch.K1 * ch.N1 + ch.N1 * ch.N2)
    _launch("f16s1_chain", 2.0 * M * (ch.K1 * ch.N1 + ch.N1 * ch.N2), nbytes, ch.slot, "lvc_conv1x1_chain_nhwc_f16s1",
            lambda: _lib.lib().lvc_conv1x1_chain_nhwc_f16s1(
                ptr(x), c_int(x.shape[-1]), ptr(ch.wa), c_int(ch.wa.shape[1]), ptr(ch.sa), ptr(ch.ta), ptr(residual),
                c_int(residual.shape[-1] if residual is not None else 0), ptr(out1), c_int(out1.shape[-1]), c_int(1 if relu1 else 0),
                ptr(ch.wb), c_int(ch.wb.shape[1]), ptr(ch.sb), ptr(ch.tb), ptr(out2), c_int(out2.shape[-1]), c_int(1 if relu2 else 0),
                c_int(M), c_int(ch.K1), c_int(ch.N1), c_int(ch.N2), ptr(conv_workspace(x.device)), _stream(x)))
    return out1, out2


class PackedBneck:

    __slots__ = ("w", "s1", "t1", "s2", "t2", "s3", "t3", "cin", "proj", "slot", "state", "__weakref__")


BNECK = _os.environ.get("LVC_BNECK", "1") != "0"
BNECK_SHAPES = {(256, 64, 256, False), (64, 64, 256, True)}
_BNECK_IDX = {}


def _bneck_index(cin, proj, device):
    key = (cin, proj, str(device))
    if key in _BNECK_IDX:
        return _BNECK_IDX[key]
    import numpy as np

    lane = np.arange(64)
    rowl = (lane % 32)[:, None].repeat(8, 1)
    kpos = np.asarray(_PERM16)[(lane // 32)[:, None] * 8 + np.arange(8)[None]]

    def frags(specs):
        pl = np.stack([np.full((64, 8), s[0]) for s in specs])
        rows = np.stack([s[1] + rowl for s in specs])
        cols = np.stack([np.asarray(s[2])[kpos] for s in specs])
        return pl, rows, cols

    a16 = np.arange(16)
    p1 = [(pl, 32 * cb, 32 * c + 16 * sp + a16) for c in range(cin // 32) for sp in range(2) for cb in range(2) for pl in range(2)]

    def col2(ch, r, s_):
        return (ch // 32) * 288 + (r * 3 + s_) * 32 + ch % 32

    p2 = [(pl, 32 * cb, col2(16 * (u // 9) + a16, (u % 9) // 3, (u % 9) % 3)) for u in range(36) for cb in range(2) for pl in range(2)]
    p3 = [(pl, 32 * j, 64 * half + 16 * s + a16) for j in range(8) for half in range(2 if proj else 1) for s in range(4)
          for pl in range(2)]
    out = tuple(tuple(torch.from_numpy(np.ascontiguousarray(a)).to(device) for a in frags(sp)) for sp in (p1, p2, p3))
    _BNECK_IDX[key] = out
    return out


def pack_bottleneck(pc1, pc2, pc3, proj, state=None):
    assert pc1.R == 1 and pc2.R == 3 and pc2.S == 3 and pc2.pad == 1 and pc2.stride == 1 and pc3.R == 1 and pc1.stride == 1
    cin = pc1.C
    assert (cin, pc1.K, pc3.K, bool(proj)) in BNECK_SHAPES and pc2.C == 64 and pc2.K == 64 and pc3.C == (128 if proj else 64)
    dev = pc1.w.device
    bk = PackedBneck()
    bk.slot = _new_range_slot(bk)
    bk.state = state if state is not None else {"off": False}
    bk.cin, bk.proj = cin, bool(proj)
    parts = []
    affine = []
    for pc, (pl, rows, cols) in zip((pc1, pc2, pc3), _bneck_index(cin, bool(proj), dev)):
        nrows, Kg = pc.w.shape
        planes = torch.empty((2, nrows, Kg), device=dev, dtype=torch.float16)
        fac = torch.empty(nrows, device=dev, dtype=torch.float32)
        check(_lib.lib().lvc_split_weights_rowscaled(ptr(pc.w), c_int(nrows), c_int(Kg), ptr(planes), ptr(fac), _stream(pc.w)),
              "lvc_split_weights_rowscaled")
        parts.append(planes[pl, rows, cols].reshape(-1))
        fac = fac[: pc.K]
        affine.append(((fac * pc.scale) if pc.scale is not None else fac).contiguous())
        affine.append(pc.shift.contiguous() if pc.shift is not None else torch.zeros(pc.K, device=dev, dtype=torch.float32))
    bk.w = torch.cat(parts).contiguous()
    bk.s1, bk.t1, bk.s2, bk.t2, bk.s3, bk.t3 = affine
    return bk


def bottleneck_fused(x, bk, out=None):
    _req_cuda(x)
    assert x.dtype == torch.float32 and x.is_contiguous() and x.dim() == 4 and x.shape[-1] >= bk.cin
    N, H, W, ldx = x.shape
    if out is None:
        out = torch.empty(N, H, W, 256, device=x.device, dtype=torch.float32)
    M = N * H * W
    kk = bk.cin * 64 + 64 * 64 * 9 + 64 * 256 + (bk.cin * 256 if bk.proj else 0)
    _launch("f16s1_bneck", 2.0 * M * kk, 4.0 * (M * (bk.cin + 256) + kk), bk.slot, "lvc_bottleneck_nhwc_f16s1",
            lambda: _lib.lib().lvc_bottleneck_nhwc_f16s1(
                ptr(x), c_int(ldx), ptr(out), c_int(out.shape[-1]), c_int(N), c_int(H), c_int(W),
                c_int(bk.cin), c_int(1 if bk.proj else 0), ptr(bk.w), ptr(bk.s1), ptr(bk.t1), ptr(bk.s2),
                ptr(bk.t2), ptr(bk.s3), ptr(bk.t3), ptr(conv_workspace(x.device)), _stream(x)))
    return out


def split_planes_f16x2(w):
    _req_cuda(w)
    w = w.detach().float().contiguous()
    out = torch.empty((2,) + tuple(w.shape), device=w.device, dtype=torch.float16)
    check(_lib.lib().lvc_split_weights(ptr(w), c_longlong(w.numel()), c_int(2), ptr(out), ptr(_conv_error_view(w.device)), _stream(w)),
          "lvc_split_weights")
    return out


def stem_conv_pool(x4, pc, relu=True, second=None):
    _req_cuda(x4)
    assert x4.dim() == 4 and x4.shape[3] == 4 and x4.is_contiguous() and x4.dtype == torch.float32
    assert pc.mode == 1 and pc.K == 64 and pc.R == 7 and pc.stride == 2 and pc.pad == 3
    N, H, W, _ = x4.shape
    Ho, Wo = (H - 1) // 2 + 1, (W - 1) // 2 + 1
    Hp, Wp = (Ho - 1) // 2 + 1, (Wo - 1) // 2 + 1
    out = torch.empty(N, Hp, Wp, 64, device=x4.device, dtype=torch.float32)
    y2 = second(out.shape) if second is not None else None
    if y2 is not None:
        assert y2.shape == out.shape and y2.stride(3) == 1 and y2.stride(1) == Wp * y2.stride(2) and y2.stride(0) == Hp * y2.stride(1)
    if CONV_SPLIT == "f16x2":
        err = _conv_error_view(x4.device)
        st = _lib.lib().lvc_stem_conv_pool_nhwc4_f16x2(ptr(x4), ptr(pc.split2h()), ptr(pc.scale), ptr(pc.shift), ptr(out),
                                                       c_int(N), c_int(H), c_int(W), c_int(pc.w.shape[0]),
                                                       c_int(1 if relu else 0), ptr(err), ptr(y2),
                                                       c_int(y2.stride(2) if y2 is not None else 0), _stream(x4))
        check(st, "lvc_stem_conv_pool_nhwc4_f16x2")
        return out
    raise RuntimeError("the fused stem exists for the fp16 split only; BasicStem runs conv + max-pool as two launches otherwise")


def linear(x, pc, relu=False, split=None):
    M, Kin = x.shape
    y = conv2d_nhwc(x.view(M, 1, 1, Kin), pc, relu=relu, split=split)
    return y.view(M, pc.K)


def new_status(device):
    return torch.zeros(1, dtype=torch.int32, device=device)


ROI_NEGATIVE_SIZE = 1
DET_OVERFLOW = 2
RETINA_OVERFLOW = 4
MASK_BAD_CLASS = 8
KEYPOINT_BAD_TARGET = 16


def roi_align_forward(input, rois, spatial_scale, pooled_h, pooled_w, sampling_ratio, aligned, status=None):
    _req_cuda(input, rois)
    input = input.contiguous().float()
    rois = rois.contiguous().float()
    B, C, H, W = input.shape
    K = rois.shape[0]
    out = torch.empty(K, C, pooled_h, pooled_w, device=input.device, dtype=torch.float32)
    st = _lib.lib().lvc_roi_align_forward_nchw(
        ptr(input), ptr(rois), ptr(out), c_int(B), c_int(C), c_int(H), c_int(W), c_int(K),
        c_int(pooled_h), c_int(pooled_w), c_float(spatial_scale), c_int(sampling_ratio),
        c_int(1 if aligned else 0), ptr(status), _stream(input))
    check(st, "lvc_roi_align_forward_nchw")
    return out


ROI_ORDER_MIN = 1024


def roi_align_fpn_nhwc(feats, scales, rois, levels, pooled_h, pooled_w, sampling_ratio, aligned,
                       num_valid=None, status=None, order=None):
    _req_cuda(rois, *feats)
    L = len(feats)
    B, _, _, C = feats[0].shape
    K = rois.shape[0]
    rois = rois.contiguous().float()
    out = torch.empty(K, pooled_h, pooled_w, C, device=rois.device, dtype=torch.float32)
    FP = c_void_p * L
    IP = c_int * L
    FL = c_float * L
    fp = FP(*[f.data_ptr() for f in feats])
    hs = IP(*[f.shape[1] for f in feats])
    ws = IP(*[f.shape[2] for f in feats])
    sc = FL(*[float(s) for s in scales])
    for f in feats:
        assert f.is_contiguous() and f.dtype == torch.float32 and f.shape[0] == B and f.shape[3] == C
    if levels is not None:
        assert levels.dtype == torch.int32 and levels.is_contiguous()
    if order is not None:
        assert order.dtype == torch.int32 and order.is_contiguous() and order.numel() == K
    elif K >= ROI_ORDER_MIN:
        order = torch.empty(K, device=rois.device, dtype=torch.int32)
        if B <= 16:
            check(_lib.lib().lvc_roi_work_order_xcd(ptr(rois), ptr(levels), c_int(K), c_int(B), ptr(order), _stream(rois)), "lvc_roi_work_order_xcd")
        else:
            check(_lib.lib().lvc_roi_work_order(ptr(rois), ptr(levels), sc, c_int(L), c_int(K), c_int(pooled_h), ptr(order), _stream(rois)),
                  "lvc_roi_work_order")
    st = _lib.lib().lvc_roi_align_fpn_nhwc_ordered(
        fp, hs, ws, sc, c_int(L), c_int(B), c_int(C), ptr(rois), ptr(levels), ptr(num_valid), c_int(K),
        c_int(pooled_h), c_int(pooled_w), c_int(sampling_ratio), c_int(1 if aligned else 0), ptr(out),
        ptr(status), ptr(order), _stream(rois))
    check(st, "lvc_roi_align_fpn_nhwc")
    return out


def roi_align_backward(grad, rois, spatial_scale, pooled_h, pooled_w, batch_size, channels, height, width,
                       sampling_ratio, aligned, status=None):
    _req_cuda(grad, rois)
    grad = grad.contiguous().float()
    rois = rois.contiguous().float()
    K = rois.shape[0]
    assert grad.shape == (K, channels, pooled_h, pooled_w)
    gin = torch.empty(batch_size, channels, height, width, device=grad.device, dtype=torch.float32)
    st = _lib.lib().lvc_roi_align_backward_nchw(
        ptr(grad), ptr(rois), ptr(gin), c_int(batch_size), c_int(channels), c_int(height), c_int(width), c_int(K),
        c_int(pooled_h), c_int(pooled_w), c_float(spatial_scale), c_int(sampling_ratio),
        c_int(1 if aligned else 0), ptr(status), _stream(grad))
    check(st, "lvc_roi_align_backward_nchw")
    return gin


def roi_align_fpn_backward_nhwc(grad, shapes, scales, rois, levels, sampling_ratio, aligned, num_valid=None,
                                status=None):
    _req_cuda(grad, rois)
    grad = grad.contiguous().float()
    rois = rois.contiguous().float()
    K, ph, pw, C = grad.shape
    L = len(shapes)
    B = shapes[0][0]
    outs = [torch.empty(*sh, device=grad.device, dtype=torch.float32) for sh in shapes]
    FP = c_void_p * L
    IP = c_int * L
    FL = c_float * L
    if levels is not None:
        assert levels.dtype == torch.int32 and levels.is_contiguous()
    st = _lib.lib().lvc_roi_align_fpn_backward_nhwc(
        ptr(grad), FP(*[o.data_ptr() for o in outs]), IP(*[sh[1] for sh in shapes]), IP(*[sh[2] for sh in shapes]),
        FL(*[float(s) for s in scales]), c_int(L), c_int(B), c_int(C), ptr(rois), ptr(levels), ptr(num_valid),
        c_int(K), c_int(ph), c_int(pw), c_int(sampling_ratio), c_int(1 if aligned else 0), ptr(status),
        _stream(grad))
    check(st, "lvc_roi_align_fpn_backward_nhwc")
    return outs


SELECT_ONELAUNCH = int(_os.environ.get("LVC_SELECT_ONELAUNCH", "3"))


def set_select_onelaunch(mode):
    global SELECT_ONELAUNCH
    SELECT_ONELAUNCH = int(mode)
    _lib.lib().lvc_set_select_onelaunch(c_int(int(mode)))


def batched_nms_batch(boxes, scores, idxs, counts, iou_threshold, max_keep=0):
    _req_cuda(boxes, scores, idxs, counts)
    B, Nmax = scores.shape
    boxes = boxes.contiguous().float()
    scores = scores.contiguous().float()
    if idxs is not None:
        idxs = idxs.contiguous()
        assert idxs.dtype == torch.int32
    keep = torch.empty(B, Nmax, dtype=torch.int32, device=boxes.device)
    num_keep = torch.empty(B, dtype=torch.int32, device=boxes.device)
    wsb = _lib.size_query("lvc_batched_nms_workspace_bytes", c_int(B), c_int(Nmax))
    ws = torch.empty(wsb, dtype=torch.uint8, device=boxes.device)
    st = _lib.lib().lvc_batched_nms(
        ptr(boxes), ptr(scores), ptr(idxs), ptr(counts), c_int(B), c_int(Nmax), c_double(iou_threshold),
        c_int(max_keep), ptr(keep), ptr(num_keep), ptr(ws), c_longlong(wsb), _stream(boxes))
    check(st, "lvc_batched_nms")
    return keep, num_keep


def batched_nms(boxes, scores, idxs, iou_threshold):
    n = boxes.shape[0]
    if n == 0:
        return torch.empty(0, dtype=torch.int64, device=boxes.device)
    idx32 = idxs.to(torch.int32)[None] if idxs is not None else None
    keep, nk = batched_nms_batch(boxes[None], scores[None], idx32, None, iou_threshold)
    return keep[0, : int(nk.item())].to(torch.int64)


def nms(boxes, scores, iou_threshold):
    return batched_nms(boxes, scores, None, iou_threshold)


SCALE_CLAMP = 4.135166556742356


def _arr(ctype, vals):
    return (ctype * len(vals))(*vals)


def rpn_proposals(logits, deltas, cell_anchors, strides, image_sizes, pre_nms_topk, post_nms_topk,
                  nms_thresh, min_box_size=0.0):
    L = len(logits)
    B, A = logits[0].shape[0], cell_anchors[0].shape[0]
    dev = logits[0].device
    _req_cuda(*logits, *deltas, *cell_anchors, image_sizes)
    for t in list(logits) + list(deltas):
        assert t.dtype == torch.float32 and t.stride(-1) == 1 and t.dim() == 4
        assert t.stride(2) == t.stride(3) * 0 + t.stride(2)
    Hs = [t.shape[1] for t in logits]
    Ws = [t.shape[2] for t in logits]
    for t, h, w in zip(list(logits) + list(deltas), Hs * 2, Ws * 2):
        assert t.stride(1) == w * t.stride(2) and t.stride(0) == h * w * t.stride(2), "need an NHWC channel slice"
    VP, IP = c_void_p * L, c_int * L
    lp = VP(*[t.data_ptr() for t in logits])
    dp = VP(*[t.data_ptr() for t in deltas])
    ap = VP(*[t.contiguous().data_ptr() for t in cell_anchors])
    ldl = IP(*[t.stride(2) for t in logits])
    ldd = IP(*[t.stride(2) for t in deltas])
    hs, ws_, st = IP(*Hs), IP(*Ws), IP(*strides)
    lib = _lib.lib()
    nbytes = _lib.size_query("lvc_rpn_proposals_workspace_bytes", c_int(B), c_int(L), c_int(A), hs, ws_, c_int(pre_nms_topk))
    ws = torch.empty(nbytes, dtype=torch.uint8, device=dev)
    boxes = torch.empty(B, post_nms_topk, 4, device=dev, dtype=torch.float32)
    olog = torch.empty(B, post_nms_topk, device=dev, dtype=torch.float32)
    count = torch.empty(B, dtype=torch.int32, device=dev)
    assert image_sizes.dtype == torch.int32 and image_sizes.is_contiguous()
    rc = lib.lvc_rpn_proposals(lp, ldl, dp, ldd, ap, hs, ws_, st, c_int(L), c_int(A), c_int(B), ptr(image_sizes),
                               c_int(pre_nms_topk), c_int(post_nms_topk), c_double(nms_thresh),
                               c_float(min_box_size), c_float(SCALE_CLAMP), ptr(boxes), ptr(olog), ptr(count),
                               ptr(ws), c_longlong(nbytes), _stream(boxes))
    check(rc, "lvc_rpn_proposals")
    return boxes, olog, count


def assign_levels_rois(boxes, min_level, max_level, canonical_box_size=224, canonical_level=4):
    _req_cuda(boxes)
    B, R, _ = boxes.shape
    boxes = boxes.contiguous()
    levels = torch.empty(B * R, dtype=torch.int32, device=boxes.device)
    rois = torch.empty(B * R, 5, dtype=torch.float32, device=boxes.device)
    rc = _lib.lib().lvc_assign_levels_rois(ptr(boxes), c_int(B), c_int(R), c_int(min_level), c_int(max_level),
                                           c_int(canonical_box_size), c_int(canonical_level), ptr(levels), ptr(rois),
                                           _stream(boxes))
    check(rc, "lvc_assign_levels_rois")
    return levels, rois


def fast_rcnn_inference(cls_logits, deltas, proposals, prop_count, image_sizes, num_classes, box_weights,
                        score_thresh, nms_thresh, topk, post=None, status=None, max_candidates=16384):
    _req_cuda(cls_logits, deltas, proposals, prop_count, image_sizes, post)
    B, R, _ = proposals.shape
    K = num_classes
    dev = proposals.device
    assert cls_logits.stride(1) == 1 and deltas.stride(1) == 1
    cls_agnostic = 1 if deltas.shape[1] == 4 else 0
    if status is None:
        status = new_status(dev)
    lib = _lib.lib()
    max_candidates = max(1, R * K) if max_candidates is None else min(max_candidates, max(1, R * K))
    nbytes = _lib.size_query("lvc_fast_rcnn_inference_workspace_bytes", c_int(B), c_int(max_candidates))
    ws = torch.empty(nbytes, dtype=torch.uint8, device=dev)
    ob = torch.empty(B, topk, 4, device=dev, dtype=torch.float32)
    osc = torch.empty(B, topk, device=dev, dtype=torch.float32)
    ocl = torch.empty(B, topk, device=dev, dtype=torch.int32)
    orow = torch.empty(B, topk, device=dev, dtype=torch.int32)
    cnt = torch.empty(B, device=dev, dtype=torch.int32)
    wx, wy, ww, wh = box_weights
    rc = lib.lvc_fast_rcnn_inference(
        ptr(cls_logits), c_int(cls_logits.stride(0)), ptr(deltas), c_int(deltas.stride(0)), c_int(K),
        c_int(cls_agnostic), ptr(proposals.contiguous()), ptr(prop_count), c_int(B), c_int(R), ptr(image_sizes),
        c_float(wx), c_float(wy), c_float(ww), c_float(wh), c_float(SCALE_CLAMP), c_float(score_thresh),
        c_double(nms_thresh), c_int(topk), c_int(max_candidates), ptr(post), ptr(ob), ptr(osc), ptr(ocl), ptr(orow),
        ptr(cnt), ptr(status), ptr(ws), c_longlong(nbytes), _stream(proposals))
    check(rc, "lvc_fast_rcnn_inference")
    return ob, osc, ocl, orow, cnt


RETINANET_MAX_SURVIVORS = 1 << 16
RETINANET_OVERFLOW = 4


def retinanet_select(logits, deltas, cell_anchors, strides, anchor_offset, num_classes, topk, score_thresh,
                     box_weights=(1.0, 1.0, 1.0, 1.0), max_survivors=RETINANET_MAX_SURVIVORS, status=None):
    L = len(logits)
    if not (L == len(deltas) == len(cell_anchors) == len(strides) and 1 <= L <= 8):
        raise ValueError("retinanet_select: 1..8 levels with logits, deltas, cell anchors and a stride each")
    _req_cuda(*logits, *deltas, *cell_anchors, status)
    B, A, K = logits[0].shape[0], cell_anchors[0].shape[0], int(num_classes)
    dev = logits[0].device
    if not (0 < topk <= 2048):
        raise ValueError("retinanet_select: topk must be in 1..2048 (got {})".format(topk))
    if any(c.shape != (A, 4) for c in cell_anchors):
        raise NotImplementedError("retinanet_select: a different number of anchors per level is not built")
    Hs = [t.shape[1] for t in logits]
    Ws = [t.shape[2] for t in logits]
    for t, d, h, w in zip(logits, deltas, Hs, Ws):
        for u, need in ((t, A * K), (d, 4 * A)):
            if not (u.dtype == torch.float32 and u.dim() == 4 and u.shape[:3] == (B, h, w) and u.shape[3] >= need and u.stride(3) == 1
                    and u.stride(1) == w * u.stride(2) and u.stride(0) == h * w * u.stride(2)):
                raise ValueError("retinanet_select: need fp32 NHWC channel slices [B,H,W,>=A*K] / [B,H,W,>=4A] of dense pixel rows")
        if h * w * A * K >= (1 << 31) or h * w * t.stride(2) >= (1 << 31):
            raise ValueError("retinanet_select: a level with 2^31 entries per image")
    full = max(h * w * A * K for h, w in zip(Hs, Ws))
    max_survivors = full if max_survivors is None else max(1, min(int(max_survivors), full))
    if status is None:
        status = new_status(dev)
    VP, IP = c_void_p * L, c_int * L
    lp = VP(*[t.data_ptr() for t in logits])
    dp = VP(*[t.data_ptr() for t in deltas])
    anchors = [t.contiguous().float() for t in cell_anchors]
    ap = VP(*[t.data_ptr() for t in anchors])
    ldl = IP(*[t.stride(2) for t in logits])
    ldd = IP(*[t.stride(2) for t in deltas])
    hs, ws_, st = IP(*Hs), IP(*Ws), IP(*[int(s) for s in strides])
    lib = _lib.lib()
    try:
        nbytes = _lib.size_query("lvc_retinanet_select_workspace_bytes", c_int(B), c_int(L), c_int(A), c_int(K), hs, ws_, c_int(topk), c_int(max_survivors))
    except _lib.LvcNativeError:
        raise ValueError("retinanet_select: shapes outside the kernel's range") from None
    ws = torch.empty(nbytes, dtype=torch.uint8, device=dev)
    rows = L * topk
    boxes = torch.empty(B, rows, 4, device=dev, dtype=torch.float32)
    scores = torch.empty(B, rows, device=dev, dtype=torch.float32)
    classes = torch.empty(B, rows, device=dev, dtype=torch.int32)
    index = torch.empty(B, rows, device=dev, dtype=torch.int32)
    count = torch.empty(B, device=dev, dtype=torch.int32)
    wx, wy, ww, wh = [float(v) for v in box_weights]
    rc = lib.lvc_retinanet_select(lp, ldl, dp, ldd, ap, hs, ws_, st, c_float(anchor_offset), c_int(L), c_int(A), c_int(K), c_int(B),
                                  c_int(topk), c_float(score_thresh), c_float(wx), c_float(wy), c_float(ww), c_float(wh),
                                  c_float(SCALE_CLAMP), c_int(max_survivors), ptr(boxes), ptr(scores), ptr(classes), ptr(index),
                                  ptr(count), ptr(status), ptr(ws), c_longlong(nbytes), _stream(boxes))
    check(rc, "lvc_retinanet_select")
    return boxes, scores, classes, index, count, status


def retinanet_select_checked(*args, max_survivors=RETINANET_MAX_SURVIVORS, **kw):
    out = retinanet_select(*args, max_survivors=max_survivors, **kw)
    if max_survivors is not None and int(out[5].item()) & RETINANET_OVERFLOW:
        _log_once("retinanet_overflow", "more than %d entries above the score threshold on one (image, level): the selection is "
                  "repeated with the list sized for H*W*A*K", max_survivors)
        kw.pop("status", None)
        out = retinanet_select(*args, max_survivors=None, **kw)
    return out


class RetinaNetLossArgs:

    def __init__(self, logits, deltas, num_anchors, num_classes, anchors, matches, labels, gt, gt_classes, gt_off,
                 alpha=0.25, gamma=2.0, beta=0.1, box_weights=(1.0, 1.0, 1.0, 1.0)):
        L = len(logits)
        if not (L == len(deltas) and 1 <= L <= 8):
            raise ValueError("retinanet_loss: 1..8 levels with logits and deltas each")
        if 0.0 < float(gamma) < 1.0 or float(gamma) < 0.0:
            raise NotImplementedError("MODEL.RETINANET.FOCAL_LOSS_GAMMA = {}: an exponent in (0, 1) has an unbounded derivative at "
                                      "saturation (and a negative one is no focal loss); 0 or >= 1 are built".format(gamma))
        _req_cuda(*logits, *deltas, anchors, matches, labels, gt_off, gt_classes)
        A, Kc = int(num_anchors), int(num_classes)
        B = logits[0].shape[0]
        self.Hs = [t.shape[1] for t in logits]
        self.Ws = [t.shape[2] for t in logits]
        for t, d, h, w in zip(logits, deltas, self.Hs, self.Ws):
            for u, need in ((t, A * Kc), (d, 4 * A)):
                if not (u.dtype == torch.float32 and u.dim() == 4 and u.shape[:3] == (B, h, w) and u.shape[3] >= need and u.stride(3) == 1
                        and u.stride(1) == w * u.stride(2) and u.stride(0) == h * w * u.stride(2)):
                    raise ValueError("retinanet_loss: need fp32 NHWC channel slices [B,H,W,>=A*K] / [B,H,W,>=4A] of dense pixel rows")
        R = sum(h * w for h, w in zip(self.Hs, self.Ws)) * A
        G = gt.shape[0]
        if not (anchors.shape == (R, 4) and anchors.dtype == torch.float32 and anchors.is_contiguous()):
            raise ValueError("retinanet_loss: anchors must be a contiguous fp32 [R,4], R = sum_l H_l W_l A = {}".format(R))
        if not (matches.shape == (B, R) and matches.dtype == torch.int32 and matches.is_contiguous()
                and labels.shape == (B, R) and labels.dtype == torch.int8 and labels.is_contiguous()):
            raise ValueError("retinanet_loss: matches int32 [B,R] and labels int8 [B,R] (match_boxes_batched)")
        if not (gt_off.dtype == torch.int32 and gt_off.numel() == B + 1 and gt.dtype == torch.float32 and gt.shape == (G, 4)
                and gt.is_contiguous() and gt_classes.dtype == torch.int64 and gt_classes.numel() == G and gt_classes.is_contiguous()):
            raise ValueError("retinanet_loss: gt fp32 [G,4], gt_classes int64 [G], gt_off int32 [B+1]")
        self.logits, self.deltas = list(logits), list(deltas)
        self.L, self.A, self.K, self.B, self.R = L, A, Kc, B, R
        self.tensors = (anchors, matches, labels, gt, gt_classes, gt_off)
        self.scalars = (float(alpha), float(gamma), float(beta)) + tuple(float(v) for v in box_weights)
        self.dev = logits[0].device

    def _levels(self, ts):
        VP, IP = c_void_p * self.L, c_int * self.L
        return VP(*[t.data_ptr() for t in ts]), IP(*[t.stride(2) for t in ts])

    def common(self):
        lp, ldl = self._levels(self.logits)
        dp, ldd = self._levels(self.deltas)
        IP = c_int * self.L
        return ([lp, ldl, dp, ldd, IP(*self.Hs), IP(*self.Ws), c_int(self.L), c_int(self.A), c_int(self.K), c_int(self.B)]
                + [ptr(t) for t in self.tensors] + [c_double(v) for v in self.scalars])


def retinanet_loss(args, normalizer_in, normalizer_out, momentum=0.9, one_minus_momentum=1 - 0.9, return_sums=False):
    _req_cuda(normalizer_in, normalizer_out)
    if not (normalizer_in.dtype == normalizer_out.dtype == torch.float64 and normalizer_in.numel() == normalizer_out.numel() == 1
            and normalizer_in.data_ptr() != normalizer_out.data_ptr()):
        raise ValueError("retinanet_loss: normalizer_in / normalizer_out must be two different float64 [1] device tensors")
# ... 1861 lines not shown
```

### lvc_amd/modeling/backbone/resnet.py

```python
import torch
import torch.nn.functional as F
from torch import nn

from ... import kernels as K
from ...layers import Conv2d, ShapeSpec, get_norm
from ...layers.layout import require_device, to_nchw_view, to_nhwc
from ...utils import weight_init
from .backbone import BACKBONE_REGISTRY, Backbone


class CNNBlockBase(nn.Module):

    def __init__(self, in_channels, out_channels, stride):
        super().__init__()
        self.in_channels, self.out_channels, self.stride = in_channels, out_channels, stride

    def freeze(self):
        for p in self.parameters():
            p.requires_grad = False
        return self


FUSE_STRIDED_PROJECTION = True


class BottleneckBlock(CNNBlockBase):
    def __init__(self, in_channels, out_channels, *, bottleneck_channels, stride=1, num_groups=1, norm="BN",
                 stride_in_1x1=False, dilation=1):
        super().__init__(in_channels, out_channels, stride)
        if dilation != 1:
            raise NotImplementedError("dilated bottlenecks (MODEL.RESNETS.RES5_DILATION != 1) are not built")
        if in_channels != out_channels:
            self.shortcut = Conv2d(in_channels, out_channels, kernel_size=1, stride=stride, bias=False,
                                   norm=get_norm(norm, out_channels))
        else:
            self.shortcut = None
        stride_1x1, stride_3x3 = (stride, 1) if stride_in_1x1 else (1, stride)
        self.conv1 = Conv2d(in_channels, bottleneck_channels, kernel_size=1, stride=stride_1x1, bias=False,
                            norm=get_norm(norm, bottleneck_channels), activation=F.relu_)
        self.conv2 = Conv2d(bottleneck_channels, bottleneck_channels, kernel_size=3, stride=stride_3x3, padding=1,
                            bias=False, norm=get_norm(norm, bottleneck_channels), activation=F.relu_, groups=num_groups)
        self.conv3 = Conv2d(bottleneck_channels, out_channels, kernel_size=1, bias=False,
                            norm=get_norm(norm, out_channels))
        for layer in [self.conv1, self.conv2, self.conv3, self.shortcut]:
            if layer is not None:
                weight_init.c2_msra_fill(layer)

    def can_fuse_projection(self, *inputs):
        grad_free = self._grad_free(*inputs)
        strided = self.shortcut is not None and self.shortcut.stride == 2 and self.conv1.stride == 2
        return (K.FUSE_PROJECTION and K.CONV_ENGINE == "bf16x3" and grad_free and self.shortcut is not None
                and (self.shortcut.stride == 1 or (strided and FUSE_STRIDED_PROJECTION)) and self.conv2.stride == 1
                and (self.conv2.out_channels + self.in_channels) % 32 == 0 and self.conv2.out_channels % 4 == 0)

    def _fused_projection(self):
        a3, asc = self.conv3._affine(), self.shortcut._affine()

        def build():
            w3, ws = self.conv3.weight.detach().float(), self.shortcut.weight.detach().float()
            if a3[0] is not None:
                w3 = w3 * a3[0].view(-1, 1, 1, 1)
            if asc[0] is not None:
                ws = ws * asc[0].view(-1, 1, 1, 1)
            shifts = [t for t in (a3[1], asc[1]) if t is not None]
            shift = None if not shifts else shifts[0] if len(shifts) == 1 else shifts[0] + shifts[1]
            return K.pack_conv(torch.cat([w3, ws], 1).contiguous(), affine=(None, shift))

        if not hasattr(self, "_cache_fused"):
            from ...layers.wrappers import _PackedCache
            self._cache_fused = _PackedCache()
        return self._cache_fused.get([self.conv3.weight, self.shortcut.weight, a3[0], a3[1], asc[0], asc[1]], build)

    def _grad_free(self, *inputs):
        if not torch.is_grad_enabled():
            return True
        if any(t is not None and t.requires_grad for t in inputs):
            return False
        return not any(p.requires_grad for p in self.parameters())

    def chain_to(self, nxt, fused_projection, *inputs):
        if nxt is not None and nxt.fused_eligible():
            return None
        if not (K.CHAIN and K.CONV_ENGINE == "bf16x3" and K.CONV_SPLIT == "f16x2" and K.PW_S1 == 2 and nxt is not None
                and self._grad_free(*inputs) and nxt._grad_free() and nxt.conv1.stride == 1 and self.conv2.stride == 1
                and not getattr(self.conv3, "two_acc", False) and not getattr(nxt.conv1, "two_acc", False)):
            return None
        k1 = self.conv2.out_channels + (self.in_channels if fused_projection else 0)
        if (k1, self.out_channels, nxt.conv1.out_channels) not in K.CHAIN_SHAPES:
            return None
        if not hasattr(self, "_cache_chain"):
            from ...layers.wrappers import _PackedCache
            self._cache_chain = _PackedCache()
            self._chain_state = {"off": False}
        if self._chain_state["off"] or self.conv3._range_state["tier"] or nxt.conv1._range_state["tier"]:
            return None
        pa = self._fused_projection() if fused_projection else self.conv3.packed()
        pb = nxt.conv1.packed()
        return self._cache_chain.get([pa.w, pa.scale, pa.shift, pb.w, pb.scale, pb.shift], lambda: K.pack_chain(pa, pb, self._chain_state))

    def fused_eligible(self, *inputs):
        if not (K.BNECK and K.CONV_ENGINE == "bf16x3" and K.CONV_SPLIT == "f16x2" and self.conv1.stride == 1 and self.conv2.stride == 1
                and self.conv2.out_channels == 64 and self.conv2.groups == 1):
            return False
        proj = self.shortcut is not None
        if (self.in_channels, self.conv2.in_channels, self.out_channels, proj) not in K.BNECK_SHAPES:
            return False
        if getattr(self, "_bneck_state", None) is not None and self._bneck_state["off"]:
            return False
        if not self._grad_free(*inputs):
            return False
        if proj and (self.shortcut.stride != 1 or not self.can_fuse_projection(*inputs)):
            return False
        layers = (self.conv1, self.conv2, self.conv3, self.shortcut) if proj else (self.conv1, self.conv2, self.conv3)
        return not any(not l._folds_norm() or getattr(l, "two_acc", False) or l._range_state["tier"] for l in layers)

    def fused(self, *inputs):
        if not self.fused_eligible(*inputs):
            return None
        proj = self.shortcut is not None
        if not hasattr(self, "_cache_bneck"):
            from ...layers.wrappers import _PackedCache
            self._cache_bneck = _PackedCache()
            self._bneck_state = {"off": False}
        p1, p2 = self.conv1.packed(), self.conv2.packed()
        p3 = self._fused_projection() if proj else self.conv3.packed()
        return self._cache_bneck.get([p1.w, p1.scale, p1.shift, p2.w, p2.scale, p2.shift, p3.w, p3.scale, p3.shift],
                                     lambda: K.pack_bottleneck(p1, p2, p3, proj, self._bneck_state))

    def forward_chained(self, x, t, nxt, concat=None):
        if t is None and concat is None:
            bk = self.fused(x)
            if bk is not None and x.shape[0] * x.shape[1] * x.shape[2] * max(x.shape[3], 256) * 4 < 0xFFF00000:
                return K.bottleneck_fused(x, bk), None
        if t is None:
            t = self.conv1.forward_nhwc(x)
        if (concat is None and self.shortcut is not None and self.shortcut.stride == 2 and self.can_fuse_projection(x, t)
                and self.chain_to(nxt, False, x, t) is None):
            cb = self.conv2.out_channels
            concat = torch.empty(t.shape[0], t.shape[1], t.shape[2], cb + self.in_channels, device=t.device, dtype=torch.float32)
            K.subsample2_into(x, concat[..., cb:])
        if concat is not None:
            K.conv2d_nhwc(t, self.conv2.packed(), relu=True, out=concat)
            ch = self.chain_to(nxt, True, x, t)
            if ch is not None and concat.numel() < (1 << 29):
                return K.conv1x1_chain(concat, ch)
            return K.conv2d_nhwc(concat, self._fused_projection(), relu=True), None
        ch = self.chain_to(nxt, False, x, t)
        if ch is None and self.conv2.activation is not None and self._grad_free(x, t):
            p2, p3 = self.conv2.packed(), self.conv3.packed()
            shortcut = self.shortcut.forward_nhwc(x) if self.shortcut is not None else x
            if K.presplit_pair_ok(t, p2, p3, shortcut):
                return K.conv3x3_conv1x1_presplit(t, p2, p3, residual=shortcut, relu=True), None
            z = self.conv2.forward_nhwc(t)
            return self.conv3.forward_nhwc(z, residual=shortcut, res_mode=1, relu=True), None
        z = self.conv2.forward_nhwc(t)
        shortcut = self.shortcut.forward_nhwc(x) if self.shortcut is not None else x
        if ch is not None and shortcut.numel() < (1 << 29):
            return K.conv1x1_chain(z, ch, residual=shortcut)
        return self.conv3.forward_nhwc(z, residual=shortcut, res_mode=1, relu=True), None

    def forward_nhwc(self, x, concat=None):
        return self.forward_chained(x, None, None, concat=concat)[0]

    def forward(self, x):
        return to_nchw_view(self.forward_nhwc(to_nhwc(x)))


FUSE_POOLED_PROJECTION = True


class BottleneckBlockCLIP(CNNBlockBase):

    def __init__(self, in_channels, out_channels, *, bottleneck_channels, stride=1, num_groups=1, norm="BN",
                 stride_in_1x1=False, dilation=1):
        super().__init__(in_channels, out_channels, stride)
        if dilation != 1:
            raise NotImplementedError("dilated bottlenecks (MODEL.RESNETS.RES5_DILATION != 1) are not built")
        if num_groups != 1:
            raise NotImplementedError("MODEL.RESNETS.D with MODEL.RESNETS.NUM_GROUPS > 1 is not built")
        if stride not in (1, 2):
            raise NotImplementedError("BottleneckBlockCLIP: the average pool is built for stride 1 and 2 (got {})".format(stride))
        if in_channels != out_channels or stride > 1:
            self.shortcut = Conv2d(in_channels, out_channels, kernel_size=1, stride=1, bias=False, norm=get_norm(norm, out_channels))
        else:
            self.shortcut = None
        self.conv1 = Conv2d(in_channels, bottleneck_channels, kernel_size=1, bias=False,
                            norm=get_norm(norm, bottleneck_channels), activation=F.relu_)
        self.conv2 = Conv2d(bottleneck_channels, bottleneck_channels, kernel_size=3, padding=1, bias=False,
                            norm=get_norm(norm, bottleneck_channels), activation=F.relu_)
        self.conv3 = Conv2d(bottleneck_channels, out_channels, kernel_size=1, bias=False, norm=get_norm(norm, out_channels))
        for layer in [self.conv1, self.conv2, self.conv3, self.shortcut]:
            if layer is not None:
                weight_init.c2_msra_fill(layer)

    _grad_free = BottleneckBlock._grad_free
    _fused_projection = BottleneckBlock._fused_projection

    def _pool(self, x):
        return K.avgpool2_nhwc(x) if self.stride == 2 else x

    def can_fuse_projection(self, x=None):
        if x is not None and torch.is_grad_enabled() and x.requires_grad:
            return False
        return (FUSE_POOLED_PROJECTION and K.FUSE_PROJECTION and K.CONV_ENGINE == "bf16x3" and self._grad_free() and self.stride == 2
                and (self.conv2.out_channels + self.in_channels) % 32 == 0 and self.conv2.out_channels % 4 == 0 and self.in_channels % 4 == 0)

    def fused_eligible(self):
        return False

    def fused(self):
        return None

    def chain_to(self, nxt, fused_projection):
        return None

    def forward_nhwc(self, x):
        t = self.conv2.forward_nhwc(self.conv1.forward_nhwc(x))
        if self.can_fuse_projection(x):
            N, H, W, _ = x.shape
            cb = self.conv2.out_channels
            concat = torch.empty(N, H // 2, W // 2, cb + self.in_channels, device=x.device, dtype=torch.float32)
            K.avgpool2_into(t, concat[..., :cb])
            K.avgpool2_into(x, concat[..., cb:])
            return K.conv2d_nhwc(concat, self._fused_projection(), relu=True)
        shortcut = self.shortcut.forward_nhwc(self._pool(x)) if self.shortcut is not None else x
        return self.conv3.forward_nhwc(self._pool(t), residual=shortcut, res_mode=1, relu=True)

    def forward(self, x):
        return to_nchw_view(self.forward_nhwc(to_nhwc(x)))


class BasicStem(CNNBlockBase):
    def __init__(self, in_channels=3, out_channels=64, norm="BN"):
        super().__init__(in_channels, out_channels, 4)
        self.in_channels = in_channels
        self.conv1 = Conv2d(in_channels, out_channels, kernel_size=7, stride=2, padding=3, bias=False,
                            norm=get_norm(norm, out_channels), activation=F.relu_)
        weight_init.c2_msra_fill(self.conv1)

    def forward_nhwc(self, x4, second=None):
        if (K.CONV_ENGINE == "bf16x3" and K.CONV_SPLIT == "f16x2" and K.STEM_FUSED and self.conv1.out_channels == 64
                and self.conv1._folds_norm()):
            return K.stem_conv_pool(x4, self.conv1.packed(), relu=True, second=second)
        y = self.conv1.forward_nhwc(x4)
        y = K.maxpool2d_nhwc(y, 3, 2, 1)
        if second is not None:
            second(y.shape).copy_(y)
        return y

    def forward(self, x):
        return to_nchw_view(self.forward_nhwc(_as_nhwc4(x)))


class DeepStem(CNNBlockBase):

    def __init__(self, in_channels=3, out_channels=64, norm="BN"):
        super().__init__(in_channels, out_channels, 4)
        self.in_channels = in_channels
        mid = out_channels // 2
        if in_channels != 3 or mid % 32:
            raise NotImplementedError("DeepStem: 3 input channels and MODEL.RESNETS.STEM_OUT_CHANNELS a multiple of 64 (got {} -> {})".format(
                in_channels, out_channels))
        self.conv1 = Conv2d(in_channels, mid, kernel_size=3, stride=2, padding=1, bias=False, norm=get_norm(norm, mid), activation=F.relu_)
        self.conv2 = Conv2d(mid, mid, kernel_size=3, stride=1, padding=1, bias=False, norm=get_norm(norm, mid), activation=F.relu_)
        self.conv3 = Conv2d(mid, out_channels, kernel_size=3, stride=1, padding=1, bias=False, norm=get_norm(norm, out_channels),
                            activation=F.relu_)
        weight_init.c2_msra_fill(self.conv1)

    def forward_nhwc(self, x4):
        y = self.conv3.forward_nhwc(self.conv2.forward_nhwc(self.conv1.forward_nhwc(x4)))
        return K.maxpool2d_nhwc(y, 3, 2, 1)

    def forward(self, x):
        return to_nchw_view(self.forward_nhwc(_as_nhwc4(x)))


def _as_nhwc4(x):
    N, C, H, W = x.shape
    assert C == 3
    s = x.stride()
    if s == (H * W * 4, 1, W * 4, 4) and x.storage_offset() % 4 == 0:
        return x.as_strided((N, H, W, 4), (H * W * 4, W * 4, 4, 1), x.storage_offset())
    return F.pad(x.permute(0, 2, 3, 1), (0, 1)).contiguous()


class ResNet(Backbone):
    def __init__(self, stem, stages, num_classes=None, out_features=None):
        super().__init__()
        if num_classes is not None:
            raise NotImplementedError("classification head is not on the detection path")
        self.stem = stem
        current_stride = self.stem.stride
        self._out_feature_strides = {"stem": current_stride}
        self._out_feature_channels = {"stem": self.stem.out_channels}
        self.stages_and_names = []
        for i, blocks in enumerate(stages):
            assert len(blocks) > 0, len(blocks)
            for block in blocks:
                assert isinstance(block, CNNBlockBase), block
            name = "res" + str(i + 2)
            stage = nn.Sequential(*blocks)
            self.add_module(name, stage)
            self.stages_and_names.append((stage, name))
            current_stride = int(current_stride * _prod([k.stride for k in blocks]))
            self._out_feature_strides[name] = current_stride
            self._out_feature_channels[name] = blocks[-1].out_channels
        if out_features is None:
            out_features = [name]
        self._out_features = out_features
        assert len(self._out_features)
        children = [x[0] for x in self.named_children()]
        for f in self._out_features:
            assert f in children, "Available children: {}".format(", ".join(children))

    def forward_nhwc(self, x4):
        outputs = {}
        first = self.stages_and_names[0][0][0] if self.stages_and_names else None
        concat = []
        if (isinstance(first, BottleneckBlock) and first.shortcut is not None and first.shortcut.stride == 1 and first.can_fuse_projection(x4)
                and not first.fused_eligible(x4)):
            def second(shape):
                n, h, w, c = shape
                concat.append(torch.empty(n, h, w, first.conv2.out_channels + c, device=x4.device, dtype=torch.float32))
                return concat[0][..., first.conv2.out_channels:]
            x = self.stem.forward_nhwc(x4, second=second)
        else:
            x = self.stem.forward_nhwc(x4)
        if "stem" in self._out_features:
            outputs["stem"] = x
        for stage, name in self.stages_and_names:
            blocks = list(stage)
            t = None
            for i, blk in enumerate(blocks):
                nxt = blocks[i + 1] if i + 1 < len(blocks) else None
                if isinstance(blk, BottleneckBlock):
                    x, t = blk.forward_chained(x, t, nxt if isinstance(nxt, BottleneckBlock) else None,
                                               concat=concat[0] if (blk is first and concat) else None)
                else:
                    x, t = blk.forward_nhwc(x), None
            if name in self._out_features:
                outputs[name] = x
        return outputs

    def forward(self, x):
        require_device(x, "ResNet")
        return {k: to_nchw_view(v) for k, v in self.forward_nhwc(_as_nhwc4(x)).items()}

    def output_shape(self):
        return {name: ShapeSpec(channels=self._out_feature_channels[name], stride=self._out_feature_strides[name])
                for name in self._out_features}

    def freeze(self, freeze_at=0):
        if freeze_at >= 1:
            self.stem.freeze()
        for idx, (stage, _) in enumerate(self.stages_and_names, start=2):
            if freeze_at >= idx:
                for block in stage.children():
                    block.freeze()
        return self

    @staticmethod
    def make_stage(block_class, num_blocks, first_stride=None, *, in_channels, out_channels, **kwargs):
        if first_stride is not None:
            assert "stride" not in kwargs and "stride_per_block" not in kwargs
            kwargs["stride_per_block"] = [first_stride] + [1] * (num_blocks - 1)
        blocks = []
        for i in range(num_blocks):
            curr = {}
            for k, v in kwargs.items():
                if k.endswith("_per_block"):
                    assert len(v) == num_blocks
                    curr[k[: -len("_per_block")]] = v[i]
                else:
                    curr[k] = v
            blocks.append(block_class(in_channels=in_channels, out_channels=out_channels, **curr))
            in_channels = out_channels
        return blocks


def _prod(xs):
    p = 1
    for x in xs:
        p *= x
    return p


@BACKBONE_REGISTRY.register()
def build_resnet_backbone(cfg, input_shape):
    R = cfg.MODEL.RESNETS
    norm = R.NORM
    unsupported = []
    resnet_d = bool(R.get("D", False))
    if resnet_d and R.NUM_GROUPS > 1:
        unsupported.append("RESNETS.D with RESNETS.NUM_GROUPS = {} (grouped CLIP blocks)".format(R.NUM_GROUPS))
    if resnet_d and R.DEPTH in (18, 34):
        unsupported.append("RESNETS.D with RESNETS.DEPTH = {}".format(R.DEPTH))
# ... 35 lines not shown
```

### lvc_amd/modeling/meta_arch/rcnn.py

```python
import torch
from torch import nn

from ... import kernels as K
from ...structures import Boxes, ImageList, Instances
from ..backbone import build_backbone
from ..postprocessing import detector_postprocess
from ..proposal_generator import RPN, build_proposal_generator
from ..roi_heads import StandardROIHeads, build_roi_heads
from ..roi_heads.roi_heads import check_status, instances_from_batched, run_with_fallbacks
from .build import META_ARCH_REGISTRY


def _freeze(module):
    for p in module.parameters():
        p.requires_grad = False


class _RCNNBase(nn.Module):
    def _dev_const(self, values, dtype):
        cache = self.__dict__.setdefault("_const_cache", {})
        key = (dtype, tuple(tuple(v) for v in values))
        t = cache.get(key)
        if t is None or t.device.type != torch.device(self.device).type:
            if len(cache) > 256:
                cache.clear()
            t = torch.tensor([list(v) for v in values], dtype=dtype, device=self.device)
            cache[key] = t
        return t

    def _init_common(self, cfg):
        self.device = torch.device(cfg.MODEL.DEVICE)
        assert len(cfg.MODEL.PIXEL_MEAN) == len(cfg.MODEL.PIXEL_STD)
        self.pixel_mean = [float(v) for v in cfg.MODEL.PIXEL_MEAN]
        self.pixel_std = [float(v) for v in cfg.MODEL.PIXEL_STD]
        assert len(self.pixel_mean) == 3, "the stem kernel is built for 3-channel images"
        self._input_cfg = cfg

    def _prepack_trainable(self):
        if not K.PREPACK or not torch.is_grad_enabled():
            return
        lst = self.__dict__.get("_trainable_convs")
        if lst is None or lst[0] != sum(1 for p in self.parameters() if p.requires_grad):
            from ...layers import Conv2d

            convs = [m for m in self.modules() if isinstance(m, Conv2d) and m.weight.requires_grad]
            lst = self.__dict__["_trainable_convs"] = (sum(1 for p in self.parameters() if p.requires_grad), convs)
        if lst[1]:
            from ...layers import Conv2d

            Conv2d.prepack(lst[1], holder=self.__dict__.setdefault("_prepack_plan", {}))

    def _mean_std(self):
        return self.__dict__.get("_norm") or (self.pixel_mean, self.pixel_std)

    def preprocess_image(self, batched_inputs):
        if "prepared" in batched_inputs[0] and "image" not in batched_inputs[0]:
            return batched_inputs[0]["prepared"].image_list(self.device)
        if "image" not in batched_inputs[0] and "raw" in batched_inputs[0]:
            return self._preprocess_raw(batched_inputs)
        images = [x["image"].to(self.device, non_blocking=True) for x in batched_inputs]
        sizes = [(int(im.shape[-2]), int(im.shape[-1])) for im in images]
        Hp, Wp = ImageList.padded_size(sizes, self.backbone.size_divisibility)
        buf = torch.empty(len(images), Hp, Wp, 4, device=self.device, dtype=torch.float32)
        if len({im.dtype for im in images}) == 1 and images[0].dtype in (torch.float32, torch.uint8):
            K.preprocess_batch_into(images, buf, *self._mean_std())
        else:
            for i, im in enumerate(images):
                K.preprocess_into(im, buf[i], *self._mean_std())
        return ImageList(buf.permute(0, 3, 1, 2)[:, :3], sizes)

    def preprocess_nhwc(self, batched_inputs):
        images = self.preprocess_image(batched_inputs)
        N, _, Hp, Wp = images.tensor.shape
        x4 = images.tensor.as_strided((N, Hp, Wp, 4), (Hp * Wp * 4, Wp * 4, 4, 1), images.tensor.storage_offset())
        return x4, images.image_sizes

    @staticmethod
    def post_rows(batched_inputs, sizes):
        post_rows, out_sizes = [], []
        for inp, (h, w) in zip(batched_inputs, sizes):
            dh, dw = (int(inp["raw"].shape[0]), int(inp["raw"].shape[1])) if "image" not in inp else (h, w)
            oh, ow = inp.get("height", dh), inp.get("width", dw)
            post_rows.append([ow / w, oh / h, float(oh), float(ow)])
            out_sizes.append((oh, ow))
        return post_rows, out_sizes

    def _preprocess_raw(self, batched_inputs):
        from ...data import ResizeShortestEdge

        aug = self.__dict__.get("_test_resize")
        if aug is None:
            aug = self.__dict__["_test_resize"] = ResizeShortestEdge.from_config(self._input_cfg, is_train=False)
        raws = [x["raw"].to(self.device, non_blocking=True) for x in batched_inputs]
        tfms = [aug.get_transform(r) for r in raws]
        sizes = [(t.new_h, t.new_w) if t is not None else (int(r.shape[0]), int(r.shape[1])) for t, r in zip(tfms, raws)]
        Hp, Wp = ImageList.padded_size(sizes, self.backbone.size_divisibility)
        buf = torch.empty(len(raws), Hp, Wp, 4, device=self.device, dtype=torch.float32)
        for i, (r, t) in enumerate(zip(raws, tfms)):
            if t is None:
                K.preprocess_into(r.permute(2, 0, 1), buf[i], *self._mean_std())
            else:
                t.apply_image(r, out_slot=buf[i], mean=self._mean_std()[0], std=self._mean_std()[1])
        return ImageList(buf.permute(0, 3, 1, 2)[:, :3], sizes)


@META_ARCH_REGISTRY.register()
class GeneralizedRCNN(_RCNNBase):
    def __init__(self, cfg):
        super().__init__()
        self._init_common(cfg)
        self.backbone = build_backbone(cfg)
        self.proposal_generator = build_proposal_generator(cfg, self.backbone.output_shape())
        self.roi_heads = build_roi_heads(cfg, self.backbone.output_shape())
        self.to(self.device)
        M = cfg.MODEL
        if M.BACKBONE.FREEZE:
            _freeze(self.backbone)
        if M.BACKBONE.FREEZE_BOTTOM_UP:
            _freeze(self.backbone.bottom_up)
        if M.PROPOSAL_GENERATOR.FREEZE and self.proposal_generator:
            _freeze(self.proposal_generator)
        if M.ROI_HEADS.FREEZE_FEAT:
            _freeze(self.roi_heads.box_head)
            if M.ROI_BOX_HEAD.CLS_AGNOSTIC_BBOX_REG:
                for n, p in self.roi_heads.box_predictor.named_parameters():
                    if "bbox_pred" in n:
                        p.requires_grad = False
        if M.ROI_HEADS.FREEZE_BBOX_PRED:
            for n, p in self.roi_heads.box_predictor.named_parameters():
                if "bbox_pred" in n:
                    p.requires_grad = False
        if M.PROPOSAL_GENERATOR.UNFREEZE_FIN:
            for p in self.proposal_generator.rpn_head.objectness_logits.parameters():
                p.requires_grad = True
            for p in self.proposal_generator.rpn_head.anchor_deltas.parameters():
                p.requires_grad = True
        assert not M.IMAGES_ONLY
        self.roi_heads_name = M.ROI_HEADS.NAME
        self.output_layer = M.ROI_HEADS.OUTPUT_LAYER

    def forward(self, batched_inputs):
        if not self.training:
            return self.inference(batched_inputs)
        if self._mask_on() and not self.__dict__.get("_mask_train_enabled", False):
            raise NotImplementedError("training the mask branch (MODEL.MASK_ON: mask_rcnn_loss, gt_masks) is not built")
        if self._keypoint_on() and not self.__dict__.get("_keypoint_train_enabled", False):
            from ..roi_heads.keypoint_head import TRAIN_REFUSAL

            raise NotImplementedError(TRAIN_REFUSAL)

        def once():
            self.__dict__["_range_checked"] = False
            self._prepack_trainable()
            losses = self._forward_train(batched_inputs)
            if not self.__dict__["_range_checked"]:
                K.check_conv_error_word(self.device)
            return losses

        return run_with_fallbacks(self, once)

    def _forward_train(self, batched_inputs):
        images = self.preprocess_image(batched_inputs)
        if "instances" in batched_inputs[0]:
            gt_instances = [x["instances"].to(self.device) for x in batched_inputs]
        elif "targets" in batched_inputs[0]:
            gt_instances = [x["targets"].to(self.device) for x in batched_inputs]
        else:
            gt_instances = None
        with torch.set_grad_enabled(torch.is_grad_enabled() and any(p.requires_grad for p in self.backbone.parameters())):
            features = self.backbone(images.tensor)
        from ..proposal_generator.rbg import RBG

        if isinstance(self.proposal_generator, RBG):
            proposals = [x["proposals"].to(self.device) for x in batched_inputs]
            proposal_losses = {}
            from ..roi_heads.cascade_rcnn import CascadeROIHeads

            if (isinstance(self.roi_heads, CascadeROIHeads) and self.roi_heads.can_batch_train(gt_instances)
                    and self.proposal_generator.can_batch(proposals, gt_instances)):
                gt, gt_off, _n = K.cat_ground_truth(gt_instances)
                table, keep = self.proposal_generator.forward_batched(proposals, gt_instances, gt, gt_off)
                return self.roi_heads.forward_train_batched(features, table, keep, gt, gt_off, gt_instances,
                                                            [x.image_size for x in gt_instances])
            proposals, _ = self.proposal_generator(proposals, gt_instances)
        elif (self.deferred_reads and isinstance(self.proposal_generator, RPN) and isinstance(self.roi_heads, StandardROIHeads)
              and self.proposal_generator.can_batch_targets(gt_instances) and self.roi_heads.can_batch_train(gt_instances)):
            return self._forward_train_deferred(images, features, gt_instances)
        elif self.proposal_generator:
            proposals, proposal_losses = self.proposal_generator(images, features, gt_instances)
        else:
            assert "proposals" in batched_inputs[0]
            proposals = [x["proposals"].to(self.device) for x in batched_inputs]
            proposal_losses = {}
        _, detector_losses = self.roi_heads(images, features, proposals, gt_instances)
        losses = {}
        losses.update(detector_losses)
        losses.update(proposal_losses)
        return losses

    deferred_reads = True

    def _forward_train_deferred(self, images, features, gt_instances):
        from ...utils.events import get_event_storage

        rpn, heads = self.proposal_generator, self.roi_heads
        boxes, logits, count, proposal_losses, rpn_counts, gt, gt_off = rpn.forward_train_batched(images, features, gt_instances)
        detector_losses, cnt, (stats, layout) = heads.forward_train_batched(features, boxes, logits, count, gt, gt_off, gt_instances)
        B, bs = boxes.shape[0], heads.batch_size_per_image
        meta = torch.cat([count.long(), rpn_counts.view(-1).long(), cnt.view(-1).long(), stats.long(), K.range_summary(self.device).long()]).tolist()
        pc, rc, cc, st, flagged = meta[:B], meta[B:3 * B], meta[3 * B:5 * B], meta[5 * B:-1], meta[-1]
        if flagged:
            K.check_conv_error_word(self.device)
        self.__dict__["_range_checked"] = True
        storage = get_event_storage()
        storage.put_scalar("rpn/num_pos_anchors", sum(rc[0::2]) / B)
        storage.put_scalar("rpn/num_neg_anchors", sum(rc[1::2]) / B)
        counts = [(cc[2 * i], cc[2 * i + 1]) for i in range(B)]
        if all(a + b == bs for a, b in counts):
            heads.log_train_scalars(counts, st, layout, B * bs)
        else:
            proposals = []
            for i, size in enumerate(images.image_sizes):
                inst = Instances(size)
                inst.proposal_boxes = Boxes(boxes[i, : pc[i]])
                inst.objectness_logits = logits[i, : pc[i]]
                proposals.append(inst)
            _, detector_losses = heads(images, features, proposals, gt_instances)
            K.check_conv_error_word(self.device)
        losses = {}
        losses.update(detector_losses)
        losses.update(proposal_losses)
        return losses

    def inference_batched(self, batched_inputs, do_postprocess=True, status=None):
        assert isinstance(self.proposal_generator, RPN) and isinstance(self.roi_heads, StandardROIHeads)
        x4, sizes = self.preprocess_nhwc(batched_inputs)
        return self.inference_nhwc(x4, sizes, self.post_rows(batched_inputs, sizes)[0] if do_postprocess else None, status)

    def inference_nhwc(self, x4, sizes, post_rows=None, status=None):
        dev = self.device
        sizes_dev = self._dev_const(sizes, torch.int32)
        feats = self.backbone.forward_nhwc(x4)
        pboxes, _plogits, pcount = self.proposal_generator.predict_proposals_batched(feats, sizes_dev)
        post = None
        if post_rows is not None:
            post = self._dev_const(post_rows, torch.float32)
        if status is None:
            status = K.new_status(dev)
        ob, osc, ocl, _orow, cnt = self.roi_heads.forward_batched(feats, pboxes, pcount, sizes_dev, post=post, status=status)
        return ob, osc, ocl, cnt, status

    def inference(self, batched_inputs, detected_instances=None, do_postprocess=True):
        assert not self.training
        if detected_instances is not None:
            if not (self._mask_on() or self._keypoint_on()):
                raise NotImplementedError("forward_with_given_boxes (mask/keypoint heads) is not on the box-only path")
            return self._inference_given_boxes(batched_inputs, detected_instances, do_postprocess)
        if getattr(self, "output_layer", None) == "BoxOnlyLayersCascade":
            return self._inference_box_corrector(batched_inputs)
        if not (isinstance(self.proposal_generator, RPN) and isinstance(self.roi_heads, StandardROIHeads)):
            return self._inference_modular(batched_inputs, do_postprocess)
        if self._mask_on():
            return run_with_fallbacks(self, lambda: self._inference_masks(batched_inputs, do_postprocess))
        if self._keypoint_on():
            return run_with_fallbacks(self, lambda: self._inference_keypoints(batched_inputs, do_postprocess))
        return run_with_fallbacks(self, lambda: self._inference_fast(batched_inputs, do_postprocess))

    def _inference_fast(self, batched_inputs, do_postprocess):
        x4, sizes = self.preprocess_nhwc(batched_inputs)
        post_rows, out_sizes = self.post_rows(batched_inputs, sizes) if do_postprocess else (None, sizes)
        ob, osc, ocl, cnt, status = self.inference_nhwc(x4, sizes, post_rows)
        insts = instances_from_batched(ob, osc, ocl, cnt, out_sizes, status)
        return [{"instances": r} for r in insts] if do_postprocess else insts

    def _mask_on(self):
        return bool(getattr(self.roi_heads, "mask_on", False))

    def _keypoint_on(self):
        return bool(getattr(self.roi_heads, "keypoint_on", False))

    def _enable_branch_training(self, name, on):
        heads = self.roi_heads
        if type(heads) is not StandardROIHeads:
            raise NotImplementedError("MODEL.ROI_HEADS.NAME = {}: the {} branch and its training are built for StandardROIHeads"
                                      .format(type(heads).__name__, name))
        if not getattr(heads, name + "_on", False):
            raise ValueError("enable_{}_training: the model was built with MODEL.{}_ON = False".format(name, name.upper()))
        head = getattr(heads, name + "_head")
        if on and getattr(head, "vis_period", 0) > 0:
            raise NotImplementedError("VIS_PERIOD > 0: visualising the mask predictions is not built")
        for owner in (self, heads, head):
            owner.__dict__["_{}_train_enabled".format(name)] = bool(on)
        return self

    def enable_mask_training(self, on=True):
        return self._enable_branch_training("mask", on)

    def enable_keypoint_training(self, on=True):
        return self._enable_branch_training("keypoint", on)

    def _inference_given_boxes(self, batched_inputs, detected_instances, do_postprocess):
        images = self.preprocess_image(batched_inputs)
        features = self.backbone(images.tensor)
        detected = [x.to(self.device) for x in detected_instances]
        results = run_with_fallbacks(self, lambda: self._given_boxes_checked(features, detected))
        if not do_postprocess:
            return results
        return [{"instances": detector_postprocess(r, inp.get("height", size[0]), inp.get("width", size[1]))}
                for r, inp, size in zip(results, batched_inputs, images.image_sizes)]

    def _given_boxes_checked(self, features, detected):
        results = self.roi_heads.forward_with_given_boxes(features, detected)
        K.check_conv_error_word(self.device)
        return results

    mask_threshold = 0.5

    def _branch_device(self, batched_inputs, do_postprocess, branch):
        x4, sizes = self.preprocess_nhwc(batched_inputs)
        dev = self.device
        sizes_dev = self._dev_const(sizes, torch.int32)
        feats = self.backbone.forward_nhwc(x4)
        pboxes, _plogits, pcount = self.proposal_generator.predict_proposals_batched(feats, sizes_dev)
        status = K.new_status(dev)
        heads = self.roi_heads
        ob, osc, ocl, _orow, cnt = heads.forward_batched(feats, pboxes, pcount, sizes_dev, post=None, status=status)
        out, rows = branch(heads, feats, ob, ocl, cnt, status)
        out_sizes, post = [tuple(s) for s in sizes], None
        if do_postprocess:
            post_rows, out_sizes = self.post_rows(batched_inputs, sizes)
            out_sizes = [(int(oh), int(ow)) for oh, ow in out_sizes]
            B, T = osc.shape
            keep = self.__dict__.get("_identity_keep")
            if keep is None or keep.shape != (B, T) or keep.device != osc.device:
                keep = self.__dict__["_identity_keep"] = torch.arange(T, dtype=torch.int32, device=dev).repeat(B, 1).contiguous()
            post = self._dev_const(post_rows, torch.float32)
            ob, osc, ocl, rows, cnt = K.gather_detections(ob, osc, ocl, rows, keep, cnt, T, post=post)
        return ob, osc, ocl, rows, cnt, out, status, out_sizes, post

    def _masks_device(self, batched_inputs, do_postprocess):
        return self._branch_device(batched_inputs, do_postprocess, lambda heads, feats, boxes, classes, count, status:
                                   heads.forward_masks_batched(feats, boxes, classes, count, status=status))[:8]

    def _inference_masks(self, batched_inputs, do_postprocess):
        import numpy as np

        ob, osc, ocl, rows, cnt, prob, status, out_sizes = self._masks_device(batched_inputs, do_postprocess)
        B, T = osc.shape
        ocl64 = ocl.to(torch.int64)
        meta = torch.cat([cnt, status, K.range_summary(self.device).to(torch.int32), rows.reshape(-1),
                          ob.reshape(-1).view(torch.int32)]).cpu().numpy()
        counts, st, flagged = [int(c) for c in meta[:B]], int(meta[B]), int(meta[B + 1])
        check_status(st)
        if flagged:
            K.check_conv_error_word(self.device)
        rows_h = meta[B + 2: B + 2 + B * T].reshape(B, T)
        boxes_h = np.ascontiguousarray(meta[B + 2 + B * T:]).view(np.float32).reshape(B, T, 4)
        buf, bases = None, []
        if do_postprocess:
            jr, jb, js, jo, total = [], [], [], [], 0
            for i, (oh, ow) in enumerate(out_sizes):
                n = counts[i]
                bases.append(total)
                jr.append(rows_h[i, :n])
                jb.append(boxes_h[i, :n])
                js += [(oh, ow)] * n
                jo += [total + k * oh * ow for k in range(n)]
                total += n * oh * ow
            jobs = K.paste_jobs(np.concatenate(jr), np.concatenate(jb), js, jo)
            buf = K.paste_masks(prob, jobs, total, threshold=self.mask_threshold)
        out = []
        for i, size in enumerate(out_sizes):
            n = counts[i]
            inst = Instances(tuple(size))
            inst.pred_boxes = Boxes(ob[i, :n])
            inst.scores = osc[i, :n]
            inst.pred_classes = ocl64[i, :n]
            if do_postprocess:
                oh, ow = size
                inst.pred_masks = buf[bases[i]: bases[i] + n * oh * ow].view(n, oh, ow).view(torch.bool)
            else:
                r0 = int(rows_h[i, 0]) if n else 0
                inst.pred_masks = prob[r0: r0 + n][:, None]
            out.append(inst)
        return [{"instances": r} for r in out] if do_postprocess else out

    def _keypoints_device(self, batched_inputs, do_postprocess):
        ob, osc, ocl, rows, cnt, kp, status, out_sizes, post = self._branch_device(
            batched_inputs, do_postprocess, lambda heads, feats, boxes, _classes, count, status:
            heads.forward_keypoints_batched(feats, boxes, count, status=status))
        B, T = osc.shape
        own = kp.index_select(0, rows.reshape(-1).long().clamp_(0, kp.shape[0] - 1))
        kps = torch.cat([own[:, :, :2], own[:, :, 3:4]], 2).view(B, T, kp.shape[1], 3)
        if post is not None:
            kps[..., :2] *= post[:, None, None, :2]
        return ob, osc, ocl, cnt, kps, status, out_sizes

    def _inference_keypoints(self, batched_inputs, do_postprocess):
        ob, osc, ocl, cnt, kps, status, out_sizes = self._keypoints_device(batched_inputs, do_postprocess)
        insts = instances_from_batched(ob, osc, ocl, cnt, out_sizes, status)
        for i, inst in enumerate(insts):
            inst._fields["pred_keypoints"] = kps[i, : len(inst)]
        return [{"instances": r} for r in insts] if do_postprocess else insts

    def _inference_box_corrector(self, batched_inputs):
        from ...structures import pairwise_iou

        images = self.preprocess_image(batched_inputs)
        with torch.no_grad():
            features = self.backbone(images.tensor)
        gt_instances = [x["instances"].to(self.device) for x in batched_inputs]
        proposals = [x["proposals"].to(self.device) for x in batched_inputs]
        out_results, in_proposals = self.roi_heads(images, features, proposals, gt_instances)
        input_ious, output_ious, gt_classes = [], [], []
        for out, inp in zip(out_results, in_proposals):
            gt = inp.gt_boxes
            input_ious.append(torch.diag(pairwise_iou(inp.proposal_boxes, gt)))
            output_ious.append(torch.diag(pairwise_iou(out.pred_boxes, gt)))
            gt_classes.append(inp.gt_classes)
        return {"input_ious": torch.cat(input_ious), "output_ious": torch.cat(output_ious), "gt_classes": torch.cat(gt_classes)}

    def _inference_modular(self, batched_inputs, do_postprocess):
        from ..proposal_generator.rbg import RBG

        images = self.preprocess_image(batched_inputs)
        features = self.backbone(images.tensor)
        if isinstance(self.proposal_generator, RBG):
            if "instances" not in batched_inputs[0] or "proposals" not in batched_inputs[0]:
                raise KeyError("PROPOSAL_GENERATOR.NAME = 'RBG' evaluates loaded `proposals` against `instances` (reference "
                               "rcnn.py:278-284); both keys are required in every input dict")
            gt_instances = [x["instances"].to(self.device) for x in batched_inputs]
            proposals = [x["proposals"].to(self.device) for x in batched_inputs]
            proposals, _ = self.proposal_generator(proposals, gt_instances)
            results, _ = self.roi_heads(images, features, proposals, gt_instances)
            if getattr(self, "roi_heads_name", None) != "UBBRROIHeads":
                return results
            return [{"instances": detector_postprocess(r, inp.get("height", size[0]), inp.get("width", size[1]))}
                    for r, inp, size in zip(results, batched_inputs, images.image_sizes)]
        if self.proposal_generator:
            proposals, _ = self.proposal_generator(images, features, None)
        else:
            assert "proposals" in batched_inputs[0]
            proposals = [x["proposals"].to(self.device) for x in batched_inputs]
        results, _ = self.roi_heads(images, features, proposals, None)
        if not do_postprocess:
            return results
        processed = []
        for r, inp, size in zip(results, batched_inputs, images.image_sizes):
            processed.append({"instances": detector_postprocess(r, inp.get("height", size[0]), inp.get("width", size[1]))})
        return processed


@META_ARCH_REGISTRY.register()
class ProposalNetwork(_RCNNBase):

    def __init__(self, cfg):
        super().__init__()
        self._init_common(cfg)
        self.backbone = build_backbone(cfg)
        self.proposal_generator = build_proposal_generator(cfg, self.backbone.output_shape())
        self.to(self.device)

    def forward(self, batched_inputs, no_post=False):
        images = self.preprocess_image(batched_inputs)
        with torch.set_grad_enabled(self.training and torch.is_grad_enabled()
                                    and any(p.requires_grad for p in self.backbone.parameters())):
            features = self.backbone(images.tensor)
        if "instances" in batched_inputs[0]:
            gt_instances = [x["instances"].to(self.device) for x in batched_inputs]
        elif "targets" in batched_inputs[0]:
            gt_instances = [x["targets"].to(self.device) for x in batched_inputs]
        else:
# ... 34 lines not shown
```

### lvc_amd/modeling/poolers.py

```python
import math

import torch
from torch import nn

from .. import kernels as K
from ..layers.layout import to_nchw_view, to_nhwc


class _PoolAllLevels(torch.autograd.Function):

    @staticmethod
    def forward(ctx, pooler, boxes, status, *feats):
        levels, rois = K.assign_levels_rois(boxes, pooler.min_level, pooler.max_level, pooler.canonical_box_size,
                                            pooler.canonical_level)
        if len(feats) == 1:
            levels = None
        ctx.pooler, ctx.rois, ctx.levels = pooler, rois, levels
        ctx.shapes = [tuple(f.shape) for f in feats]
        return K.roi_align_fpn_nhwc(list(feats), pooler.scales, rois, levels, pooler.output_size[0], pooler.output_size[1],
                                    pooler.sampling_ratio, pooler.aligned, status=status)

    @staticmethod
    @torch.autograd.function.once_differentiable
    def backward(ctx, grad):
        pl = ctx.pooler
        grads = K.roi_align_fpn_backward_nhwc(grad, ctx.shapes, pl.scales, ctx.rois, ctx.levels, pl.sampling_ratio, pl.aligned)
        return (None, None, None) + tuple(grads)


class _PoolRois(torch.autograd.Function):

    @staticmethod
    def forward(ctx, pooler, rois, levels, num_valid, status, *feats):
        ctx.pooler, ctx.rois, ctx.levels, ctx.num_valid = pooler, rois, levels, num_valid
        ctx.shapes = [tuple(f.shape) for f in feats]
        return K.roi_align_fpn_nhwc(list(feats), pooler.scales, rois, levels, pooler.output_size[0], pooler.output_size[1],
                                    pooler.sampling_ratio, pooler.aligned, status=status)

    @staticmethod
    @torch.autograd.function.once_differentiable
    def backward(ctx, grad):
        pl = ctx.pooler
        grads = K.roi_align_fpn_backward_nhwc(grad, ctx.shapes, pl.scales, ctx.rois, ctx.levels, pl.sampling_ratio, pl.aligned,
                                              num_valid=ctx.num_valid)
        return (None, None, None, None, None) + tuple(grads)


class ROIPooler(nn.Module):
    def __init__(self, output_size, scales, sampling_ratio, pooler_type, canonical_box_size=224, canonical_level=4):
        super().__init__()
        if isinstance(output_size, int):
            output_size = (output_size, output_size)
        assert len(output_size) == 2 and isinstance(output_size[0], int) and isinstance(output_size[1], int)
        self.output_size = output_size
        if pooler_type == "ROIAlign":
            self.aligned = False
        elif pooler_type == "ROIAlignV2":
            self.aligned = True
        else:
            raise NotImplementedError("pooler type '{}' is not used by the shipped configs".format(pooler_type))
        self.scales = tuple(scales)
        self.sampling_ratio = sampling_ratio
        min_level = -(math.log2(scales[0]))
        max_level = -(math.log2(scales[-1]))
        assert math.isclose(min_level, int(min_level)) and math.isclose(max_level, int(max_level)), \
            "Featuremap stride is not power of 2!"
        self.min_level, self.max_level = int(min_level), int(max_level)
        assert len(scales) == self.max_level - self.min_level + 1, "[ROIPooler] Sizes of input featuremaps do not form a pyramid!"
        assert 0 <= self.min_level <= self.max_level
        self.canonical_level = canonical_level
        assert canonical_box_size > 0
        self.canonical_box_size = canonical_box_size

    def pool_nhwc(self, feats_nhwc, boxes, status=None):
        if torch.is_grad_enabled() and any(f.requires_grad for f in feats_nhwc):
            return _PoolAllLevels.apply(self, boxes.detach(), status, *feats_nhwc)
        levels, rois = K.assign_levels_rois(boxes, self.min_level, self.max_level, self.canonical_box_size,
                                            self.canonical_level)
        if len(feats_nhwc) == 1:
            levels = None
        return K.roi_align_fpn_nhwc(feats_nhwc, self.scales, rois, levels, self.output_size[0], self.output_size[1],
                                    self.sampling_ratio, self.aligned, status=status)

    def pool_rois_nhwc(self, feats_nhwc, rois, levels, num_valid=None, status=None):
        if torch.is_grad_enabled() and any(f.requires_grad for f in feats_nhwc):
            return _PoolRois.apply(self, rois, levels, num_valid, status, *feats_nhwc)
        return K.roi_align_fpn_nhwc(feats_nhwc, self.scales, rois, levels, self.output_size[0], self.output_size[1],
                                    self.sampling_ratio, self.aligned, status=status)

    def forward(self, x, box_lists):
        assert isinstance(x, list) and isinstance(box_lists, list), "Arguments to pooler must be lists"
        assert len(x) == len(self.scales)
        assert len(box_lists) == x[0].size(0)
        counts = [len(b) for b in box_lists]
        M = sum(counts)
        C = x[0].shape[1]
        if M == 0:
            return torch.zeros((0, C) + self.output_size, device=x[0].device, dtype=x[0].dtype)
        R = max(counts)
        boxes = torch.zeros(len(box_lists), R, 4, device=x[0].device)
        for i, b in enumerate(box_lists):
            boxes[i, : counts[i]] = b.tensor
        out = self.pool_nhwc([to_nhwc(f) for f in x], boxes)
        out = out.view(len(box_lists), R, self.output_size[0], self.output_size[1], C)
        out = torch.cat([out[i, : counts[i]] for i in range(len(box_lists))], 0)
        return out.permute(0, 3, 1, 2)
```

Before: 660.5 img/s.

## Fuse raw-image preprocessing into stem, two-source projection conv, fused ROI level assignment

The stem kernel now reads the raw per-image CHW tensors directly, normalising and padding inside the conv+pool launch, so the separate preprocessing pass and its NHWC4 buffer are no longer needed. The stride-2 bottleneck projection gets a two-source 1x1 conv that reads conv2's output and the stride-2 subsampled input in place, instead of building a concatenated tensor. ROI level assignment, rois construction and the XCD work-order sort are merged into one kernel launch. These remove launches and intermediate memory traffic, at the cost of more template variants and extra per-chunk source selection inside the pointwise kernel.

Result: no change. 657.4 img/s (-0.5%).

```diff
diff --git a/include/lvc_amd.h b/include/lvc_amd.h
--- a/include/lvc_amd.h
+++ b/include/lvc_amd.h
@@ -74,6 +74,9 @@
 int lvc_conv1x1_nhwc_f16s1_presplit(const void* x, const unsigned short* w_split, const float* scale, const float* shift,
                                     const float* residual, float* y, int N, int H, int W, int C, int K, int relu,
                                     int res_mode, int ldy, int ldr, void* workspace, void* stream);
+int lvc_conv1x1_nhwc_f16s1_src2(const float* x1, int ld1, const float* x2, int H2, int W2, int C2, const unsigned short* w_split,
+                                const float* scale, const float* shift, float* y, int N, int Ho, int Wo, int C, int K, int relu,
+                                int ldy, void* workspace, void* stream);
 int lvc_conv1x1_nhwc_f16s1_w2(const float* x, const unsigned short* w_split, const float* scale, const float* shift,
                               const float* residual, float* y, int N, int H, int W, int C, int K, int Kpad, int stride, int relu,
                               int res_mode, int ldy, int ldr, void* workspace, void* stream);
@@ -98,6 +101,10 @@
 int lvc_stem_conv_pool_nhwc4_f16x2(const float* x, const unsigned short* w_split, const float* scale, const float* shift,
                                    float* y, int N, int H, int W, int Kpad, int relu, int* d_error_word,
                                    float* y2 , int ldy2, void* stream);
+int lvc_stem_conv_pool_chw_f16x2(const void* const* images, int dtype, const int* hs, const int* ws, int B, int Hp, int Wp,
+                                 const float* mean3, const float* std3, const unsigned short* w_split, const float* scale,
+                                 const float* shift, float* y, int Kpad, int relu, int* d_error_word, float* y2, int ldy2,
+                                 void* stream);
 
 int lvc_preprocess_nhwc4(const void* image, int dtype, int h, int w, const float* mean3, const float* std3,
                          float* out, int Hp, int Wp, void* stream);
@@ -143,6 +150,8 @@
 int lvc_roi_work_order(const float* rois, const int* levels, const float* scales, int L, int K, int pooled_h, int* d_order,
                        void* stream);
 int lvc_roi_work_order_xcd(const float* rois, const int* levels, int K, int B, int* d_order, void* stream);
+int lvc_roi_levels_order_xcd(const float* boxes, int B, int R, int min_level, int max_level, int canonical_box_size,
+                             int canonical_level, int key_levels, int* levels, float* rois, int* d_order, void* stream);
 int lvc_roi_align_fpn_nhwc_ordered(const float* const* feats, const int* Hs, const int* Ws, const float* scales, int L,
                                    int B, int C, const float* rois, const int* levels, const int* d_num_valid, int K,
                                    int pooled_h, int pooled_w, int sampling_ratio, int aligned, float* output,
diff --git a/lvc_amd/csrc/conv_pw_s1.hip b/lvc_amd/csrc/conv_pw_s1.hip
--- a/lvc_amd/csrc/conv_pw_s1.hip
+++ b/lvc_amd/csrc/conv_pw_s1.hip
@@ -27,8 +27,13 @@
   float pl_qscale;
 };
 
-template <int NI, bool ONEACC, bool PLANES = false, bool PRE = false>
-__global__ __launch_bounds__(NT, 2) void conv_pw_s1_kernel(PwArgsS p) {
+struct PwArgsS2 : PwArgsS {
+  const float* x2;
+  int x2_bytes, nk1, ld1, H2, W2, C2;
+};
+
+template <int NI, bool ONEACC, bool PLANES = false, bool PRE = false, bool SRC2 = false>
+__global__ __launch_bounds__(NT, 2) void conv_pw_s1_kernel(std::conditional_t<SRC2, PwArgsS2, PwArgsS> p) {
   constexpr int HN = 64 * NI;
   constexpr int PLANE_A = PM * AROW;
   constexpr int A_BUF = 2 * PLANE_A;
@@ -62,6 +67,12 @@
   const unsigned long long xbase = (unsigned long long)p.x;
   const u32x4 xres = {(unsigned)__builtin_amdgcn_readfirstlane((unsigned)xbase), (unsigned)__builtin_amdgcn_readfirstlane((unsigned)(xbase >> 32) & 0xffffu),
                       (unsigned)p.x_bytes, 0x00020000u};
+  u32x4 x2res = xres;
+  if constexpr (SRC2) {
+    const unsigned long long x2base = (unsigned long long)p.x2;
+    x2res = u32x4{(unsigned)__builtin_amdgcn_readfirstlane((unsigned)x2base), (unsigned)__builtin_amdgcn_readfirstlane((unsigned)(x2base >> 32) & 0xffffu),
+                  (unsigned)p.x2_bytes, 0x00020000u};
+  }
   const int fx3 = (fi >> 2) & 3;
   const int a_row[2] = {(wm * 64 + fi) * AROW, (wm * 64 + 32 + fi) * AROW};
   const int b_row = (wn * 32 * NI + fi) * 64;
@@ -97,14 +108,19 @@
     const int m0 = tile_m * PM;
     const int n0 = tile_n * HN;
 
-    unsigned a_off[NJ];
+    unsigned a_off[NJ], a_off2[SRC2 ? NJ : 1];
 #pragma unroll
     for (int j = 0; j < NJ; ++j) {
       const int m = m0 + hrow + 64 * j;
       const int n = m / (p.Ho * p.Wo);
       const int rem = m - n * (p.Ho * p.Wo);
       const int ho = rem / p.Wo, wo = rem - ho * p.Wo;
-      a_off[j] = m < p.M ? (unsigned)(((n * p.H + ho * p.stride) * p.W + wo * p.stride) * p.C + q * 4) * 4u : 0x80000000u;
+      if constexpr (SRC2) {
+        a_off[j] = m < p.M ? (unsigned)(m * p.ld1 + q * 4) * 4u : 0x80000000u;
+        a_off2[j] = m < p.M ? (unsigned)(((n * p.H2 + 2 * ho) * p.W2 + 2 * wo) * p.C2 + q * 4) * 4u : 0x80000000u;
+      } else {
+        a_off[j] = m < p.M ? (unsigned)(((n * p.H + ho * p.stride) * p.W + wo * p.stride) * p.C + q * 4) * 4u : 0x80000000u;
+      }
     }
     const unsigned short* bsrc[NI];
     int bdst[NI];
@@ -123,8 +139,18 @@
     };
     f32x4 ar[3][NJ];
     auto load_A = [&](int set, int cc) {
-#pragma unroll
-      for (int j = 0; j < NJ; ++j) ar[set][j] = load_untracked(xres, a_off[j], (unsigned)cc * 128u);
+      if constexpr (SRC2) {
+        const bool first = cc < p.nk1;
+        u32x4 rs;
+#pragma unroll
+        for (int e = 0; e < 4; ++e) rs[e] = first ? xres[e] : x2res[e];
+        const unsigned soff = (unsigned)(first ? cc : cc - p.nk1) * 128u;
+#pragma unroll
+        for (int j = 0; j < NJ; ++j) ar[set][j] = load_untracked(rs, first ? a_off[j] : a_off2[j], soff);
+      } else {
+#pragma unroll
+        for (int j = 0; j < NJ; ++j) ar[set][j] = load_untracked(xres, a_off[j], (unsigned)cc * 128u);
+      }
     };
     auto store_A = [&](int set, unsigned char* dstA) {
       if (PRE) {
@@ -583,10 +609,12 @@
 }
 
 struct PwPlanes { unsigned short* planes; int* err; long long PS; int N, Npad, H; float qscale; };
+struct PwSrc2 { const float* x2; int ld1, H2, W2, C2; };
 
 static int pw_s1_launch(bool oneacc, const float* x, const unsigned short* w_split, const float* scale, const float* shift,
                         const float* residual, float* y, int N, int H, int W, int C, int K, int stride, int relu, int res_mode,
-                        int ldy, int ldr, void* workspace, void* stream, const PwPlanes* pl = nullptr, bool pre = false) {
+                        int ldy, int ldr, void* workspace, void* stream, const PwPlanes* pl = nullptr, bool pre = false,
+                        const PwSrc2* s2 = nullptr) {
   LVC_CHECK_ARG(x && w_split && y && workspace, "null pointer");
   LVC_CHECK_ARG(!oneacc || scale, "the single-accumulator form needs the row factors in `scale`");
   LVC_CHECK_ARG(N > 0 && H > 0 && W > 0 && C > 0 && K > 0 && stride >= 1, "non-positive dimension");
@@ -595,7 +623,8 @@
   LVC_CHECK_ARG(res_mode >= 0 && res_mode <= 2 && (res_mode == 0 || residual), "bad residual");
   const int Ho = (H - 1) / stride + 1, Wo = (W - 1) / stride + 1;
   if (res_mode == 2) LVC_CHECK_ARG(Ho % 2 == 0 && Wo % 2 == 0, "upsample-add needs even output size");
-  PwArgsS a;
+  PwArgsS2 a;
+  a.x2 = nullptr; a.x2_bytes = 0; a.nk1 = 0; a.ld1 = 0; a.H2 = a.W2 = a.C2 = 0;
   a.x = x; a.w = w_split; a.scale = scale; a.shift = shift; a.res = residual; a.y = y;
   a.H = H; a.W = W; a.C = C; a.K = K; a.stride = stride; a.Ho = Ho; a.Wo = Wo;
   const long long Mll = (long long)N * Ho * Wo;
@@ -606,7 +635,18 @@
   LVC_CHECK_ARG(((uintptr_t)x & 15) == 0 && ((uintptr_t)w_split & 15) == 0 && ((uintptr_t)y & 15) == 0 && ((uintptr_t)workspace & 15) == 0 &&
                     ((uintptr_t)scale & 15) == 0 && ((uintptr_t)shift & 15) == 0 && ((uintptr_t)residual & 15) == 0,
                 "pointers must be 16-byte aligned");
-  const long long xb = (long long)N * H * W * C * 4;
+  long long xb = (long long)N * H * W * C * 4;
+  if (s2) {
+    LVC_CHECK_ARG(!pl && !pre && stride == 1, "the two-source form: plain input, stride 1 over the first source");
+    LVC_CHECK_ARG(s2->x2 && ((uintptr_t)s2->x2 & 15) == 0, "second source: null or not 16-byte aligned");
+    LVC_CHECK_ARG(s2->C2 > 0 && s2->C2 % 32 == 0 && C - s2->C2 > 0 && (C - s2->C2) % 32 == 0, "both sources need a multiple of 32 channels");
+    LVC_CHECK_ARG(s2->ld1 >= C - s2->C2 && s2->ld1 % 4 == 0, "bad row stride of the first source");
+    LVC_CHECK_ARG(s2->H2 > 0 && s2->W2 > 0 && (s2->H2 - 1) / 2 + 1 == H && (s2->W2 - 1) / 2 + 1 == W, "the second source must be the stride-2 parent of the first");
+    const long long x2b = (long long)N * s2->H2 * s2->W2 * s2->C2 * 4;
+    LVC_CHECK_ARG(x2b < (1ll << 31), "second source must be smaller than 2 GiB");
+    xb = (long long)N * H * W * s2->ld1 * 4;
+    a.x2 = s2->x2; a.x2_bytes = (int)x2b; a.nk1 = (C - s2->C2) / 32; a.ld1 = s2->ld1; a.H2 = s2->H2; a.W2 = s2->W2; a.C2 = s2->C2;
+  }
   LVC_CHECK_ARG(xb < (1ll << 31), "input tensor must be smaller than 2 GiB");
   a.x_bytes = (int)xb;
   const int ni = K <= 64 ? 1 : 2;
@@ -648,6 +688,13 @@
     LVC_CHECK_LAUNCH();
     return LVC_OK;
   }
+  if (s2) {
+    LVC_CHECK_ARG(oneacc, "the two-source form exists for the single-accumulator kernel");
+    if (ni == 1) hipLaunchKernelGGL((conv_pw_s1_kernel<1, true, false, false, true>), dim3(a.nworkers), dim3(NT), 0, st, a);
+    else hipLaunchKernelGGL((conv_pw_s1_kernel<2, true, false, false, true>), dim3(a.nworkers), dim3(NT), 0, st, a);
+    LVC_CHECK_LAUNCH();
+    return LVC_OK;
+  }
   if (oneacc) {
     if (ni == 1) hipLaunchKernelGGL((conv_pw_s1_kernel<1, true>), dim3(a.nworkers), dim3(NT), 0, st, a);
     else hipLaunchKernelGGL((conv_pw_s1_kernel<2, true>), dim3(a.nworkers), dim3(NT), 0, st, a);
@@ -686,3 +733,11 @@
   pl.PS = (long long)B * H * Npad * 64;
   return pw_s1_launch(true, x, w_split, scale, shift, nullptr, (float*)planes, B * N, 1, 1, C, 3 * H * 64, 1, 0, 0, 0, 0, workspace, stream, &pl);
 }
+
+extern "C" int lvc_conv1x1_nhwc_f16s1_src2(const float* x1, int ld1, const float* x2, int H2, int W2, int C2, const unsigned short* w_split,
+                                           const float* scale, const float* shift, float* y, int N, int Ho, int Wo, int C, int K, int relu,
+                                           int ldy, void* workspace, void* stream) {
+  PwSrc2 s2;
+  s2.x2 = x2; s2.ld1 = ld1; s2.H2 = H2; s2.W2 = W2; s2.C2 = C2;
+  return pw_s1_launch(true, x1, w_split, scale, shift, nullptr, y, N, Ho, Wo, C, K, 1, relu, 0, ldy, 0, workspace, stream, nullptr, false, &s2);
+}
diff --git a/lvc_amd/csrc/roi_align.hip b/lvc_amd/csrc/roi_align.hip
--- a/lvc_amd/csrc/roi_align.hip
+++ b/lvc_amd/csrc/roi_align.hip
@@ -708,24 +708,49 @@
   const int* levels;
   int K, B;
   int* order;
+  const float* boxes;
+  int* levels_out;
+  float* rois_out;
+  int R, min_level, max_level, key_levels;
+  float canonical_box_size, canonical_level;
 };
+template <bool ASSIGN>
 __global__ __launch_bounds__(1024) void roi_work_order_xcd_kernel(RoiOrderXcdArgs p) {
   __shared__ int hist[ROI_XCD_MAX_B][256];
   __shared__ int cnt[ROI_XCD_MAX_B], tail0[ROI_XCD_MAX_B], s_min;
   const int tid = threadIdx.x;
   for (int i = tid; i < ROI_XCD_MAX_B * 256; i += 1024) (&hist[0][0])[i] = 0;
   __syncthreads();
-  auto key = [&](int k, int& b) {
-    const float* r = p.rois + (long long)k * 5;
-    const float bf = r[0];
+  auto key = [&](int k, int& b, bool write) {
+    float bf, y1, y2;
+    int lv;
+    if constexpr (ASSIGN) {
+      const float4 bx = *reinterpret_cast<const float4*>(p.boxes + (size_t)k * 4);
+      const float area = (bx.z - bx.x) * (bx.w - bx.y);
+      const float size = sqrtf(area);
+      float lvl = floorf(p.canonical_level + log2f(size / p.canonical_box_size + 1e-8f));
+      lvl = lvl < (float)p.min_level ? (float)p.min_level : lvl;
+      lvl = lvl > (float)p.max_level ? (float)p.max_level : lvl;
+      lv = (int)lvl - p.min_level;
+      bf = (float)(k / p.R); y1 = bx.y; y2 = bx.w;
+      if (write) {
+        p.levels_out[k] = lv;
+        float* r = p.rois_out + (size_t)k * 5;
+        r[0] = bf; r[1] = bx.x; r[2] = bx.y; r[3] = bx.z; r[4] = bx.w;
+      }
+      lv = p.key_levels ? (lv & 3) : 0;
+    } else {
+      const float* r = p.rois + (long long)k * 5;
+      bf = r[0]; y1 = r[2]; y2 = r[4];
+      lv = p.levels ? (p.levels[k] & 3) : 0;
+    }
     b = bf >= 0.f && bf < (float)p.B ? (int)bf : 0;
-    const int lv = p.levels ? (p.levels[k] & 3) : 0;
-    const float yc = (r[2] + r[4]) * 0.5f;
+    const float yc = (y1 + y2) * 0.5f;
     int band = yc == yc ? (int)(fminf(fmaxf(yc, 0.f), 1e6f) * (1.f / 16.f)) : 0;
     band = band > 63 ? 63 : band;
     return lv * 64 + band;
   };
-  for (int k = tid; k < p.K; k += 1024) { int b; const int ky = key(k, b); atomicAdd(&hist[b][ky], 1); }
+  for (int k = tid; k < p.K; k += 1024) { int b; const int ky = key(k, b, true); atomicAdd(&hist[b][ky], 1); }
   __syncthreads();
   if (tid < p.B) {
     int run = 0;
@@ -744,7 +769,7 @@
   const int m = s_min;
   for (int k = tid; k < p.K; k += 1024) {
     int b;
-    const int ky = key(k, b);
+    const int ky = key(k, b, false);
     const int r = atomicAdd(&hist[b][ky], 1);
     p.order[r < m ? r * p.B + b : m * p.B + tail0[b] + (r - m)] = k;
   }
@@ -755,8 +780,27 @@
   if (K == 0) return LVC_OK;
   LVC_CHECK_ARG(rois && d_order, "null pointer");
   RoiOrderXcdArgs a;
+  memset(&a, 0, sizeof a);
   a.rois = rois; a.levels = levels; a.K = K; a.B = B; a.order = d_order;
-  hipLaunchKernelGGL(roi_work_order_xcd_kernel, dim3(1), dim3(1024), 0, (hipStream_t)stream, a);
+  hipLaunchKernelGGL(roi_work_order_xcd_kernel<false>, dim3(1), dim3(1024), 0, (hipStream_t)stream, a);
+  LVC_CHECK_LAUNCH();
+  return LVC_OK;
+}
+
+extern "C" int lvc_roi_levels_order_xcd(const float* boxes, int B, int R, int min_level, int max_level, int canonical_box_size,
+                                        int canonical_level, int key_levels, int* levels, float* rois, int* d_order, void* stream) {
+  LVC_CHECK_ARG(B >= 1 && B <= ROI_XCD_MAX_B && R >= 0, "1..16 images");
+  LVC_CHECK_ARG((long long)B * R < (1ll << 28), "too many boxes");
+  if (R == 0) return LVC_OK;
+  LVC_CHECK_ARG(boxes && levels && rois && d_order, "null pointer");
+  LVC_CHECK_ARG(((uintptr_t)boxes & 15) == 0, "boxes must be 16-byte aligned");
+  RoiOrderXcdArgs a;
+  memset(&a, 0, sizeof a);
+  a.K = B * R; a.B = B; a.order = d_order;
+  a.boxes = boxes; a.levels_out = levels; a.rois_out = rois; a.R = R; a.min_level = min_level; a.max_level = max_level;
+  a.key_levels = key_levels ? 1 : 0;
+  a.canonical_box_size = (float)canonical_box_size; a.canonical_level = (float)canonical_level;
+  hipLaunchKernelGGL(roi_work_order_xcd_kernel<true>, dim3(1), dim3(1024), 0, (hipStream_t)stream, a);
   LVC_CHECK_LAUNCH();
   return LVC_OK;
 }
diff --git a/lvc_amd/csrc/stem_input.h b/lvc_amd/csrc/stem_input.h
--- /dev/null
+++ b/lvc_amd/csrc/stem_input.h
@@ -0,0 +1,32 @@
+#pragma once
+#include <stdint.h>
+
+#define STEM_MAX_IMAGES 16
+
+struct StemImages {
+  const void* img[STEM_MAX_IMAGES];
+  int h[STEM_MAX_IMAGES], w[STEM_MAX_IMAGES];
+  int bytes[STEM_MAX_IMAGES];
+};
+
+static inline const char* stem_images_fill(const void* const* images, int dtype, const int* hs, const int* ws, int B, int H, int W,
+                                           StemImages* t) {
+  if (!t) return "null table";
+  if (!images || !hs || !ws) return "null pointer";
+  if (dtype != 0 && dtype != 1) return "dtype must be 0 (f32) or 1 (u8)";
+  if (B < 1 || B > STEM_MAX_IMAGES) return "1..16 images";
+  if (H <= 0 || W <= 0) return "bad padded size";
+  const int es = dtype == 0 ? 4 : 1;
+  for (int i = 0; i < B; ++i) {
+    if (!images[i]) return "null image pointer";
+    if (hs[i] <= 0 || ws[i] <= 0 || hs[i] > H || ws[i] > W) return "an image is empty or larger than the padded size";
+    if (3ll * hs[i] * ws[i] * es >= (1ll << 31)) return "image too large";
+    if (((uintptr_t)images[i] & (uintptr_t)(es - 1)) != 0) return "image pointer not aligned to its element size";
+  }
+  for (int i = 0; i < STEM_MAX_IMAGES; ++i) {
+    const int j = i < B ? i : 0;
+    t->img[i] = images[j]; t->h[i] = hs[j]; t->w[i] = ws[j];
+    t->bytes[i] = 3 * hs[j] * ws[j] * es;
+  }
+  return nullptr;
+}
diff --git a/lvc_amd/csrc/stem_pool_h2.hip b/lvc_amd/csrc/stem_pool_h2.hip
--- a/lvc_amd/csrc/stem_pool_h2.hip
+++ b/lvc_amd/csrc/stem_pool_h2.hip
@@ -1,4 +1,5 @@
 #include "conv_common.h"
+#include "stem_input.h"
 #include <stdlib.h>
 
 #define SP_PH 3
@@ -17,6 +18,7 @@
 #define SP_NLD 3
 
 struct StemArgsH {
+  static constexpr int SRC = 0;
   const float* x;
   const unsigned short* w;
   int* err;
@@ -30,12 +32,26 @@
   int x_bytes, w_plane_bytes;
 };
 
+template <int S>
+struct StemArgsChw : StemArgsH {
+  static constexpr int SRC = S;
+  StemImages im;
+  float mean[3], std[3];
+};
+
+__device__ __forceinline__ float stem_normalise(float v, float m, float s) {
+#pragma clang fp contract(off)
+  const float d = v - m;
+  return d / s;
+}
+
 __device__ __forceinline__ void split2s(float a, f16& h, f16& m) {
   h = (f16)a;
   m = (f16)((a - (float)h) * 2048.f);
 }
 
-__global__ __launch_bounds__(SP_NT, 4) void stem_pool_h2_kernel(StemArgsH p) {
+template <class Args>
+__global__ __launch_bounds__(SP_NT, 4) void stem_pool_h2_kernel(Args p) {
   constexpr int IN_ELEMS = 2 * SP_PLANE_IN;
   constexpr int B_ELEMS = 2 * SP_PLANE_B;
   constexpr int CS_OFF = 0;
@@ -75,8 +91,11 @@
   const float sc = p.scale ? p.scale[ocol] : 1.f;
   const float sh = p.shift ? p.shift[ocol] : 0.f;
 
+  constexpr int SRC = Args::SRC;
   int range_err = 0;
   f32x4 wreg[SP_NLD];
+  unsigned wraw[SP_NLD][3];
+  unsigned wmask = 0;
   u32x4 breg[1], breg2;
   auto window_offsets = [&](int tile, unsigned* off) {
     const int tx = tile % p.tiles_x;
@@ -94,25 +113,68 @@
     }
   };
   auto load_window = [&](int tile) {
-    unsigned off[SP_NLD];
-    window_offsets(tile, off);
-#pragma unroll
-    for (int j = 0; j < SP_NLD; ++j)
-      wreg[j] = __builtin_bit_cast(f32x4, __builtin_amdgcn_raw_buffer_load_b128(xres, off[j], 0, 0));
+    if constexpr (SRC == 0) {
+      unsigned off[SP_NLD];
+      window_offsets(tile, off);
+#pragma unroll
+      for (int j = 0; j < SP_NLD; ++j)
+        wreg[j] = __builtin_bit_cast(f32x4, __builtin_amdgcn_raw_buffer_load_b128(xres, off[j], 0, 0));
+    } else {
+      constexpr int ES = SRC == 1 ? 4 : 1;
+      const int tx = tile % p.tiles_x;
+      const int t2 = tile / p.tiles_x;
+      const int ty = t2 % p.tiles_y;
+      const int img = (t2 / p.tiles_y) & (STEM_MAX_IMAGES - 1);
+      const int h = p.im.h[img], w = p.im.w[img];
+      const int plane = h * w * ES;
+      const __amdgpu_buffer_rsrc_t ires = __builtin_amdgcn_make_buffer_rsrc((void*)p.im.img[img], 0, p.im.bytes[img], 0x00020000);
+      const int iy0 = 2 * (2 * ty * SP_PH - 1) - 3, ix0 = 2 * (2 * tx * SP_PW - 1) - 3;
+      wmask = 0;
+#pragma unroll
+      for (int j = 0; j < SP_NLD; ++j) {
+        const int idx = tid + SP_NT * j;
+        const int iy = idx / SP_IW, ix = idx - iy * SP_IW;
+        const int yy = iy0 + iy, xx = ix0 + ix;
+        const bool ok = idx < SP_IH * SP_IW && yy >= 0 && yy < h && xx >= 0 && xx < w;
+        const unsigned off = ok ? (unsigned)((yy * w + xx) * ES) : 0x80000000u;
+        wmask |= ok ? 1u << j : 0u;
+#pragma unroll
+        for (int c = 0; c < 3; ++c) {
+          if constexpr (SRC == 1) wraw[j][c] = __builtin_amdgcn_raw_buffer_load_b32(ires, off, c * plane, 0);
+          else wraw[j][c] = __builtin_amdgcn_raw_buffer_load_b8(ires, off, c * plane, 0);
+        }
+      }
+    }
+  };
+  auto window_pixel = [&](int j) {
+    if constexpr (SRC == 0) {
+      return wreg[j];
+    } else {
+      f32x4 v = {0.f, 0.f, 0.f, 0.f};
+      if ((wmask >> j) & 1u) {
+#pragma unroll
+        for (int c = 0; c < 3; ++c) {
+          const float raw = SRC == 1 ? __builtin_bit_cast(float, wraw[j][c]) : (float)wraw[j][c];
+          v[c] = stem_normalise(raw, p.mean[c], p.std[c]);
+        }
+      }
+      return v;
+    }
   };
   auto store_window = [&]() {
 #pragma unroll
     for (int j = 0; j < SP_NLD; ++j) {
       const int idx = tid + SP_NT * j;
       if (idx < SP_IH * SP_IW) {
+        const f32x4 px = window_pixel(j);
         f16x4 h, m;
         float big = 0.f;
 #pragma unroll
         for (int e = 0; e < 4; ++e) {
           f16 hh, mm;
-          split2s(wreg[j][e], hh, mm);
+          split2s(px[e], hh, mm);
           h[e] = hh; m[e] = mm;
-          big = fmaxf(big, fabsf(wreg[j][e]));
+          big = fmaxf(big, fabsf(px[e]));
         }
         if (!(big <= LVC_F16_MAX)) range_err = 1;
         const int o = idx * 4;
@@ -243,6 +305,24 @@
   if (range_err && p.err) atomicOr(p.err, 2);
 }
 
+static int stem_geometry(StemArgsH& a, const unsigned short* w_split, const float* scale, const float* shift, float* y, int N, int H,
+                         int W, int Kpad, int relu, int* d_error_word, float* y2, int ldy2, const char* fn) {
+  a.w = w_split; a.scale = scale; a.shift = shift; a.y = y; a.y2 = y2; a.ldy2 = ldy2;
+  a.N = N; a.H = H; a.W = W; a.relu = relu; a.err = d_error_word;
+  a.Ho = (H + 6 - 7) / 2 + 1; a.Wo = (W + 6 - 7) / 2 + 1;
+  a.Hp = (a.Ho + 2 - 3) / 2 + 1; a.Wp = (a.Wo + 2 - 3) / 2 + 1;
+  a.tiles_x = lvc_cdiv(a.Wp, SP_PW); a.tiles_y = lvc_cdiv(a.Hp, SP_PH);
+  const long long nt = (long long)N * a.tiles_x * a.tiles_y;
+  const long long wb = (long long)Kpad * 224 * 2;
+  if (!(nt < (1ll << 31))) {
+    lvc_set_error("%s: input too large", fn);
+    return LVC_ERR_INVALID;
+  }
+  a.ntiles = (int)nt; a.w_plane_bytes = (int)wb;
+  a.nworkers = a.ntiles < 2 * lvc_cu_count() ? a.ntiles : 2 * lvc_cu_count();
+  return LVC_OK;
+}
+
 extern "C" int lvc_stem_conv_pool_nhwc4_f16x2(const float* x, const unsigned short* w_split, const float* scale,
                                               const float* shift, float* y, int N, int H, int W, int Kpad, int relu,
                                               int* d_error_word, float* y2, int ldy2, void* stream) {
@@ -252,17 +332,45 @@
   LVC_CHECK_ARG(((uintptr_t)x & 15) == 0 && ((uintptr_t)w_split & 15) == 0 && ((uintptr_t)y & 15) == 0,
                 "pointers must be 16-byte aligned");
   StemArgsH a;
-  a.x = x; a.w = w_split; a.scale = scale; a.shift = shift; a.y = y; a.y2 = y2; a.ldy2 = ldy2;
-  a.N = N; a.H = H; a.W = W; a.relu = relu; a.err = d_error_word;
-  a.Ho = (H + 6 - 7) / 2 + 1; a.Wo = (W + 6 - 7) / 2 + 1;
-  a.Hp = (a.Ho + 2 - 3) / 2 + 1; a.Wp = (a.Wo + 2 - 3) / 2 + 1;
-  a.tiles_x = lvc_cdiv(a.Wp, SP_PW); a.tiles_y = lvc_cdiv(a.Hp, SP_PH);
-  const long long nt = (long long)N * a.tiles_x * a.tiles_y;
-  const long long xb = (long long)N * H * W * 16, wb = (long long)Kpad * 224 * 2;
-  LVC_CHECK_ARG(nt < (1ll << 31) && xb < (1ll << 31), "input too large");
-  a.ntiles = (int)nt; a.x_bytes = (int)xb; a.w_plane_bytes = (int)wb;
-  a.nworkers = a.ntiles < 2 * lvc_cu_count() ? a.ntiles : 2 * lvc_cu_count();
-  hipLaunchKernelGGL(stem_pool_h2_kernel, dim3(a.nworkers), dim3(SP_NT), 0, (hipStream_t)stream, a);
+  a.x = x;
+  const long long xb = (long long)N * H * W * 16;
+  LVC_CHECK_ARG(xb < (1ll << 31), "input too large");
+  a.x_bytes = (int)xb;
+  const int rc = stem_geometry(a, w_split, scale, shift, y, N, H, W, Kpad, relu, d_error_word, y2, ldy2, __func__);
+  if (rc) return rc;
+  hipLaunchKernelGGL(stem_pool_h2_kernel<StemArgsH>, dim3(a.nworkers), dim3(SP_NT), 0, (hipStream_t)stream, a);
   LVC_CHECK_LAUNCH();
   return LVC_OK;
 }
+
+template <int S>
+static int launch_stem_chw(const StemImages& im, const float* mean3, const float* std3, const unsigned short* w_split,
+                           const float* scale, const float* shift, float* y, int B, int H, int W, int Kpad, int relu,
+                           int* d_error_word, float* y2, int ldy2, void* stream, const char* fn) {
+  StemArgsChw<S> a;
+  a.x = nullptr; a.x_bytes = 0;
+  a.im = im;
+  for (int c = 0; c < 3; ++c) { a.mean[c] = mean3[c]; a.std[c] = std3[c]; }
+  const int rc = stem_geometry(a, w_split, scale, shift, y, B, H, W, Kpad, relu, d_error_word, y2, ldy2, fn);
+  if (rc) return rc;
+  hipLaunchKernelGGL(stem_pool_h2_kernel<StemArgsChw<S>>, dim3(a.nworkers), dim3(SP_NT), 0, (hipStream_t)stream, a);
+  return LVC_OK;
+}
+
+extern "C" int lvc_stem_conv_pool_chw_f16x2(const void* const* images, int dtype, const int* hs, const int* ws, int B, int H, int W,
+                                            const float* mean3, const float* std3, const unsigned short* w_split, const float* scale,
+                                            const float* shift, float* y, int Kpad, int relu, int* d_error_word, float* y2, int ldy2,
+                                            void* stream) {
+  LVC_CHECK_ARG(mean3 && std3 && w_split && y, "null pointer");
+  LVC_CHECK_ARG(!y2 || (ldy2 >= 64 && ldy2 % 4 == 0 && ((uintptr_t)y2 & 15) == 0), "bad second output");
+  LVC_CHECK_ARG(Kpad >= 64, "bad shape");
+  LVC_CHECK_ARG(((uintptr_t)w_split & 15) == 0 && ((uintptr_t)y & 15) == 0, "pointers must be 16-byte aligned");
+  StemImages im;
+  const char* why = stem_images_fill(images, dtype, hs, ws, B, H, W, &im);
+  LVC_CHECK_ARG(!why, why);
+  const int rc = dtype == 0 ? launch_stem_chw<1>(im, mean3, std3, w_split, scale, shift, y, B, H, W, Kpad, relu, d_error_word, y2, ldy2, stream, __func__)
+                            : launch_stem_chw<2>(im, mean3, std3, w_split, scale, shift, y, B, H, W, Kpad, relu, d_error_word, y2, ldy2, stream, __func__);
+  if (rc) return rc;
+  LVC_CHECK_LAUNCH();
+  return LVC_OK;
+}
diff --git a/lvc_amd/kernels.py b/lvc_amd/kernels.py
--- a/lvc_amd/kernels.py
+++ b/lvc_amd/kernels.py
@@ -694,6 +694,42 @@
     return out
 
 
+def _two_source_shapes(z_shape, x, pc):
+    N, Ho, Wo, C1 = z_shape
+    return (x.dim() == 4 and x.shape[0] == N and pc.C == C1 + x.shape[3] and C1 % 32 == 0 and x.shape[3] % 32 == 0
+            and pc.R == 1 and pc.S == 1 and pc.stride == 1 and pc.pad == 0 and pc.mode == 0 and pc.K % 4 == 0
+            and (x.shape[1] - 1) // 2 + 1 == Ho and (x.shape[2] - 1) // 2 + 1 == Wo
+            and max(x.numel(), N * Ho * Wo * max(C1, pc.K)) < (1 << 29))
+
+
+def two_source_ok(z_shape, x, pc):
+    N, Ho, Wo, _ = z_shape
+    return _two_source_shapes(z_shape, x, pc) and conv_route(pc, N, Ho, Wo).entry == "lvc_conv1x1_nhwc_f16s1"
+
+
+def conv1x1_two_source(z, x, pc, relu=False):
+    _req_cuda(z, x)
+    assert _two_source_shapes(tuple(z.shape), x, pc), "outside the two-source kernel's range"
+    assert x.is_contiguous() and x.dtype == torch.float32 and z.dtype == torch.float32
+    N, Ho, Wo, C1 = z.shape
+    ld1 = z.stride(2)
+    assert z.stride(3) == 1 and z.stride(1) == Wo * ld1 and z.stride(0) == Ho * Wo * ld1
+    _, H, W, C2 = x.shape
+    out = torch.empty(N, Ho, Wo, pc.K, device=z.device, dtype=torch.float32)
+    pc.last_one = True
+    rows = N * Ho * Wo
+
+    def call():
+        wts, scale = pc.split2s()
+        return _lib.lib().lvc_conv1x1_nhwc_f16s1_src2(ptr(z), c_int(ld1), ptr(x), c_int(H), c_int(W), c_int(C2), ptr(wts), ptr(scale),
+                                                      ptr(pc.shift), ptr(out), c_int(N), c_int(Ho), c_int(Wo), c_int(pc.C), c_int(pc.K),
+                                                      c_int(1 if relu else 0), c_int(pc.K), ptr(conv_workspace(z.device)), _stream(z))
+
+    _launch("f16x2_pws1", 2.0 * rows * pc.K * pc.C, 4.0 * (rows * pc.C + rows * pc.K + pc.K * pc.C), pc.slot,
+            "lvc_conv1x1_nhwc_f16s1_src2", call)
+    return out
+
+
 class PackedChain:
 
     __slots__ = ("wa", "sa", "ta", "wb", "sb", "tb", "K1", "N1", "N2", "slot", "state", "__weakref__")
@@ -1056,6 +1092,55 @@
     raise RuntimeError("the fused stem exists for the fp16 split only; BasicStem runs conv + max-pool as two launches otherwise")
 
 
+class RawBatch:
+    requires_grad = False
+
+    def __init__(self, images, padded_size, mean, std):
+        self.images, self.padded_size, self.mean, self.std = list(images), (int(padded_size[0]), int(padded_size[1])), mean, std
+        self.device = self.images[0].device
+
+    @staticmethod
+    def eligible(images):
+        return (0 < len(images) <= 16 and all(im.is_cuda and im.dim() == 3 and im.shape[0] == 3 for im in images)
+                and len({im.dtype for im in images}) == 1 and images[0].dtype in (torch.float32, torch.uint8))
+
+
+def stem_fused_route():
+    return CONV_ENGINE == "bf16x3" and CONV_SPLIT == "f16x2" and STEM_FUSED
+
+
+def stem_conv_pool_chw(raw, pc, relu=True, second=None):
+    images = raw.images
+    _req_cuda(*images)
+    B = len(images)
+    if B == 0 or any(im.dtype != images[0].dtype for im in images) or images[0].dtype not in (torch.float32, torch.uint8):
+        raise RuntimeError("stem_conv_pool_chw: the images must be all float32 or all uint8")
+    if CONV_SPLIT != "f16x2":
+        raise RuntimeError("the fused stem exists for the fp16 split only")
+    assert pc.mode == 1 and pc.K == 64 and pc.R == 7 and pc.stride == 2 and pc.pad == 3
+    imgs = []
+    for im in images:
+        assert im.dim() == 3 and im.shape[0] == 3
+        imgs.append(im.contiguous())
+    H, W = raw.padded_size
+    Ho, Wo = (H - 1) // 2 + 1, (W - 1) // 2 + 1
+    Hp, Wp = (Ho - 1) // 2 + 1, (Wo - 1) // 2 + 1
+    dev = imgs[0].device
+    out = torch.empty(B, Hp, Wp, 64, device=dev, dtype=torch.float32)
+    y2 = second(out.shape) if second is not None else None
+    if y2 is not None:
+        assert y2.shape == out.shape and y2.stride(3) == 1 and y2.stride(1) == Wp * y2.stride(2) and y2.stride(0) == Hp * y2.stride(1)
+    P = (c_void_p * B)(*[im.data_ptr() for im in imgs])
+    hs = (c_int * B)(*[int(im.shape[1]) for im in imgs])
+    ws = (c_int * B)(*[int(im.shape[2]) for im in imgs])
+    st = _lib.lib().lvc_stem_conv_pool_chw_f16x2(P, c_int(1 if imgs[0].dtype == torch.uint8 else 0), hs, ws, c_int(B), c_int(H), c_int(W),
+                                                 _float3(raw.mean), _float3(raw.std), ptr(pc.split2h()), ptr(pc.scale), ptr(pc.shift),
+                                                 ptr(out), c_int(pc.w.shape[0]), c_int(1 if relu else 0), ptr(_conv_error_view(dev)),
+                                                 ptr(y2), c_int(y2.stride(2) if y2 is not None else 0), _stream(imgs[0]))
+    check(st, "lvc_stem_conv_pool_chw_f16x2")
+    return out
+
+
 def linear(x, pc, relu=False, split=None):
     M, Kin = x.shape
     y = conv2d_nhwc(x.view(M, 1, 1, Kin), pc, relu=relu, split=split)
@@ -1260,6 +1345,20 @@
                                            _stream(boxes))
     check(rc, "lvc_assign_levels_rois")
     return levels, rois
+
+
+def assign_levels_rois_order(boxes, min_level, max_level, canonical_box_size=224, canonical_level=4, key_levels=True):
+    _req_cuda(boxes)
+    B, R, _ = boxes.shape
+    boxes = boxes.contiguous()
+    levels = torch.empty(B * R, dtype=torch.int32, device=boxes.device)
+    rois = torch.empty(B * R, 5, dtype=torch.float32, device=boxes.device)
+    order = torch.empty(B * R, dtype=torch.int32, device=boxes.device)
+    rc = _lib.lib().lvc_roi_levels_order_xcd(ptr(boxes), c_int(B), c_int(R), c_int(min_level), c_int(max_level), c_int(canonical_box_size),
+                                             c_int(canonical_level), c_int(1 if key_levels else 0), ptr(levels), ptr(rois), ptr(order),
+                                             _stream(boxes))
+    check(rc, "lvc_roi_levels_order_xcd")
+    return levels, rois, order
 
 
 def fast_rcnn_inference(cls_logits, deltas, proposals, prop_count, image_sizes, num_classes, box_weights,
diff --git a/lvc_amd/modeling/backbone/resnet.py b/lvc_amd/modeling/backbone/resnet.py
--- a/lvc_amd/modeling/backbone/resnet.py
+++ b/lvc_amd/modeling/backbone/resnet.py
@@ -137,6 +137,9 @@
         if (concat is None and self.shortcut is not None and self.shortcut.stride == 2 and self.can_fuse_projection(x, t)
                 and self.chain_to(nxt, False, x, t) is None):
             cb = self.conv2.out_channels
+            pf = self._fused_projection()
+            if self.chain_to(nxt, True, x, t) is None and K.two_source_ok(tuple(t.shape[:3]) + (cb,), x, pf):
+                return K.conv1x1_two_source(K.conv2d_nhwc(t, self.conv2.packed(), relu=True), x, pf, relu=True), None
             concat = torch.empty(t.shape[0], t.shape[1], t.shape[2], cb + self.in_channels, device=t.device, dtype=torch.float32)
             K.subsample2_into(x, concat[..., cb:])
         if concat is not None:
@@ -238,10 +241,15 @@
                             norm=get_norm(norm, out_channels), activation=F.relu_)
         weight_init.c2_msra_fill(self.conv1)
 
+    def takes_raw(self):
+        return K.stem_fused_route() and self.conv1.out_channels == 64 and self.conv1._folds_norm()
+
     def forward_nhwc(self, x4, second=None):
-        if (K.CONV_ENGINE == "bf16x3" and K.CONV_SPLIT == "f16x2" and K.STEM_FUSED and self.conv1.out_channels == 64
-                and self.conv1._folds_norm()):
+        if self.takes_raw():
+            if isinstance(x4, K.RawBatch):
+                return K.stem_conv_pool_chw(x4, self.conv1.packed(), relu=True, second=second)
             return K.stem_conv_pool(x4, self.conv1.packed(), relu=True, second=second)
+        assert not isinstance(x4, K.RawBatch), "the raw batch goes to the one-launch stem only (BasicStem.takes_raw)"
         y = self.conv1.forward_nhwc(x4)
         y = K.maxpool2d_nhwc(y, 3, 2, 1)
         if second is not None:
diff --git a/lvc_amd/modeling/meta_arch/rcnn.py b/lvc_amd/modeling/meta_arch/rcnn.py
--- a/lvc_amd/modeling/meta_arch/rcnn.py
+++ b/lvc_amd/modeling/meta_arch/rcnn.py
@@ -74,6 +74,19 @@
         N, _, Hp, Wp = images.tensor.shape
         x4 = images.tensor.as_strided((N, Hp, Wp, 4), (Hp * Wp * 4, Wp * 4, 4, 1), images.tensor.storage_offset())
         return x4, images.image_sizes
+
+    def inference_input(self, batched_inputs):
+        from ..backbone.fpn import FPN
+        from ..backbone.resnet import BasicStem, ResNet
+
+        trunk = self.backbone.bottom_up if type(self.backbone) is FPN else self.backbone
+        if type(trunk) is ResNet and type(trunk.stem) is BasicStem and trunk.stem.takes_raw() and "image" in batched_inputs[0]:
+            images = [x["image"].to(self.device, non_blocking=True) for x in batched_inputs]
+            if K.RawBatch.eligible(images):
+                sizes = [(int(im.shape[-2]), int(im.shape[-1])) for im in images]
+                padded = ImageList.padded_size(sizes, self.backbone.size_divisibility)
+                return K.RawBatch(images, padded, *self._mean_std()), sizes
+        return self.preprocess_nhwc(batched_inputs)
 
     @staticmethod
     def post_rows(batched_inputs, sizes):
@@ -234,7 +247,7 @@
 
     def inference_batched(self, batched_inputs, do_postprocess=True, status=None):
         assert isinstance(self.proposal_generator, RPN) and isinstance(self.roi_heads, StandardROIHeads)
-        x4, sizes = self.preprocess_nhwc(batched_inputs)
+        x4, sizes = self.inference_input(batched_inputs)
         return self.inference_nhwc(x4, sizes, self.post_rows(batched_inputs, sizes)[0] if do_postprocess else None, status)
 
     def inference_nhwc(self, x4, sizes, post_rows=None, status=None):
@@ -267,7 +280,7 @@
         return run_with_fallbacks(self, lambda: self._inference_fast(batched_inputs, do_postprocess))
 
     def _inference_fast(self, batched_inputs, do_postprocess):
-        x4, sizes = self.preprocess_nhwc(batched_inputs)
+        x4, sizes = self.inference_input(batched_inputs)
         post_rows, out_sizes = self.post_rows(batched_inputs, sizes) if do_postprocess else (None, sizes)
         ob, osc, ocl, cnt, status = self.inference_nhwc(x4, sizes, post_rows)
         insts = instances_from_batched(ob, osc, ocl, cnt, out_sizes, status)
@@ -317,7 +330,7 @@
     mask_threshold = 0.5
 
     def _branch_device(self, batched_inputs, do_postprocess, branch):
-        x4, sizes = self.preprocess_nhwc(batched_inputs)
+        x4, sizes = self.inference_input(batched_inputs)
         dev = self.device
         sizes_dev = self._dev_const(sizes, torch.int32)
         feats = self.backbone.forward_nhwc(x4)
diff --git a/lvc_amd/modeling/poolers.py b/lvc_amd/modeling/poolers.py
--- a/lvc_amd/modeling/poolers.py
+++ b/lvc_amd/modeling/poolers.py
@@ -75,12 +75,18 @@
     def pool_nhwc(self, feats_nhwc, boxes, status=None):
         if torch.is_grad_enabled() and any(f.requires_grad for f in feats_nhwc):
             return _PoolAllLevels.apply(self, boxes.detach(), status, *feats_nhwc)
-        levels, rois = K.assign_levels_rois(boxes, self.min_level, self.max_level, self.canonical_box_size,
-                                            self.canonical_level)
+        B, R, _ = boxes.shape
+        order = None
+        if B * R >= K.ROI_ORDER_MIN and B <= 16 and B == feats_nhwc[0].shape[0]:
+            levels, rois, order = K.assign_levels_rois_order(boxes, self.min_level, self.max_level, self.canonical_box_size,
+                                                             self.canonical_level, key_levels=len(feats_nhwc) > 1)
+        else:
+            levels, rois = K.assign_levels_rois(boxes, self.min_level, self.max_level, self.canonical_box_size,
+                                                self.canonical_level)
         if len(feats_nhwc) == 1:
             levels = None
         return K.roi_align_fpn_nhwc(feats_nhwc, self.scales, rois, levels, self.output_size[0], self.output_size[1],
-                                    self.sampling_ratio, self.aligned, status=status)
+                                    self.sampling_ratio, self.aligned, status=status, order=order)
 
     def pool_rois_nhwc(self, feats_nhwc, rois, levels, num_valid=None, status=None):
         if torch.is_grad_enabled() and any(f.requires_grad for f in feats_nhwc):
```
